# adr-arroyo/PointCloudComparator

Measured on NVIDIA B200. Metric: knn_queries_per_s_k16_10M, higher is better.
Workload: dtype f32

## Files before the change

### include/pcc/search.h

```cpp
#ifndef PCC_SEARCH_H_
#define PCC_SEARCH_H_

#include <stdint.h>

#ifdef __cplusplus
extern "C" {
#endif

#define PCC_HOST 0
#define PCC_DEVICE 1

#define PCC_OK 0
#define PCC_ERR_INVALID (-1)
#define PCC_ERR_CUDA (-2)
#define PCC_ERR_STATE (-3)

#define PCC_MAX_K 512

typedef struct pcc_index pcc_index;

const char *pcc_last_error(void);
int pcc_version(void);
int64_t pcc_launch_count(void);

int pcc_create(int device, pcc_index **out);
void pcc_destroy(pcc_index *idx);

int pcc_build(pcc_index *idx, const void *pts, int64_t n, int stride_bytes, const int32_t *indices, int64_t n_idx,
              float cell_hint, int k_hint, int mem, void *stream);
int64_t pcc_size(const pcc_index *idx);
int pcc_grid_info(const pcc_index *idx, double out[5]);

int pcc_knn(pcc_index *idx, const void *q, int64_t nq, int stride_bytes, int k, int32_t *out_idx, float *out_d2,
            int *k_eff, int mem, void *stream);

int pcc_radius_count(pcc_index *idx, const void *q, int64_t nq, int stride_bytes, double radius, unsigned max_nn,
                     int64_t *offsets, int64_t *total, int mem, void *stream);
int pcc_radius_fill(pcc_index *idx, const void *q, int64_t nq, int stride_bytes, double radius, unsigned max_nn, int sorted,
                    const int64_t *offsets, int32_t *out_idx, float *out_d2, int mem, void *stream);

int pcc_knn_mean_dist(pcc_index *idx, const void *q, int64_t nq, int stride_bytes, int mean_k, float *out_mean,
                      int mem, void *stream);
int pcc_sor_threshold(pcc_index *idx, const float *distances, int64_t n, int64_t n_valid, double std_mul, double stats[3],
                      uint8_t *keep, int64_t *kept, int mem, void *stream);

int pcc_normals_knn(pcc_index *idx, const void *q, int64_t nq, int stride_bytes, int k, const float viewpoint[3], float *out,
                    int mem, void *stream);
int pcc_normals_radius(pcc_index *idx, const void *q, int64_t nq, int stride_bytes, double radius, const float viewpoint[3],
                       float *out, int mem, void *stream);

int pcc_intensity_gradient(pcc_index *idx, const void *q, int64_t nq, int stride_bytes, double radius, const float *intensity,
                           const float *normals4, float *out, int mem, void *stream);
int pcc_rift(pcc_index *idx, const void *q, int64_t nq, int stride_bytes, double radius, const float *gradient4,
             int n_distance_bins, int n_gradient_bins, float *out, int mem, void *stream);

int pcc_sift_dog(pcc_index *idx, const float *values, const float *scales, int n_scales, float *out, int mem, void *stream);
int pcc_sift_extrema(pcc_index *idx, const float *dog, int n_cols, float min_contrast, int32_t *out_row, int32_t *out_col, int64_t cap,
                     int64_t *n_found, int mem, void *stream);
int pcc_sift_keypoints(pcc_index *idx, const void *pts, int64_t n, int stride_bytes, int rgb_offset_bytes, float min_scale, int nr_octaves,
                       int nr_scales_per_octave, float min_contrast, float *out4, int64_t cap, int64_t *n_keypoints, int mem, void *stream);

int pcc_icp_step(pcc_index *idx, void *src_inout, int64_t ns, int stride_bytes, const float *T_apply, double sums[16],
                 int64_t *count, int32_t *corr_idx, float *corr_d2, int mem, void *stream);
int pcc_icp_align(pcc_index *idx, const void *src, int64_t ns, int stride_bytes, int max_iter, float T16[16], int *converged,
                  double *fitness, int *iterations, int mem, void *stream);
int pcc_umeyama_from_sums(const double sums[16], int64_t count, float T16[16]);

int pcc_euclidean_labels(pcc_index *idx, double tolerance, int64_t min_size, int64_t max_size, int32_t *labels,
                         int64_t *n_clusters, int64_t *sizes, int64_t sizes_cap, int mem, void *stream);

int pcc_ece_init(pcc_index *idx, uint32_t *parent, void *stream);
int pcc_ece_link_range(pcc_index *idx, double tolerance, int64_t begin, int64_t end, uint32_t *parent, void *stream);
int pcc_ece_absorb(pcc_index *idx, const uint32_t *other, uint32_t *parent, void *stream);
int pcc_ece_finish(pcc_index *idx, uint32_t *parent, int64_t min_size, int64_t max_size, int32_t *labels, int64_t *n_clusters, int64_t *sizes,
                   int64_t sizes_cap, void *stream);

int pcc_first_within(pcc_index *idx, const void *q, int64_t nq, int stride_bytes, double thr, int32_t *out, int mem, void *stream);

int pcc_voxel_grid(pcc_index *idx, const void *pts, int64_t n, int stride_bytes, int rgb_offset_bytes, const float leaf[3],
                   int min_points_per_voxel, void *out, int64_t *n_out, int mem, void *stream);

int pcc_region_growing(const int32_t *neighbours, int64_t n, int k, const float *normals4, float smoothness_rad, float curvature_threshold,
                       int64_t min_size, int64_t max_size, int32_t *labels, int64_t *n_clusters);

int pcc_region_growing_rgb(const int32_t *neighbours, const float *sqr_distances, int64_t n, int k, const uint32_t *rgba, int rgba_stride_bytes,
                           float distance_threshold, float point_color_threshold, float region_color_threshold, int grow_neighbours,
                           int64_t min_size, int64_t max_size, int32_t *labels, int64_t *n_clusters);

int pcc_descriptor_nn(pcc_index *workspace, const float *ref, int64_t n_ref, const float *qry, int64_t n_qry, int dim, int stride_floats,
                      int32_t *out_idx, float *out_d2, int mem, void *stream);

int pcc_export(const pcc_index *idx, double meta[16], void *ptrs[2]);
int pcc_adopt(pcc_index *idx, const double meta[16], void *stream);

int pcc_comm_init(pcc_index *idx, void *nccl_comm, int rank, int world);
int pcc_comm_info(const pcc_index *idx, int *rank, int *world);
int pcc_broadcast_index(pcc_index *idx, int root, void *stream);
int pcc_gather(pcc_index *idx, const void *local, int64_t n_local, int row_bytes, const int32_t *local_rows, void *out, int64_t n_total, void *stream);
int pcc_allreduce_f64(pcc_index *idx, double *device_buf, int n, void *stream);

int pcc_set_timing(pcc_index *idx, int enable);
double pcc_last_kernel_ms(const pcc_index *idx);

#ifdef __cplusplus
}
#endif
#endif
```

### pointcloudcomparator_b200/_lib.py

```python
from __future__ import annotations

import ctypes as C
import os

_HERE = os.path.dirname(os.path.abspath(__file__))
SO_PATH = os.path.abspath(os.environ["PCC_SO"]) if os.environ.get("PCC_SO") else os.path.join(_HERE, "libpcc_search.so")

HOST, DEVICE = 0, 1
MAX_K = 512

_lib = None

SYMBOLS = [
    "pcc_last_error", "pcc_version", "pcc_launch_count", "pcc_create", "pcc_destroy", "pcc_build", "pcc_size", "pcc_grid_info",
    "pcc_knn", "pcc_radius_count", "pcc_radius_fill", "pcc_knn_mean_dist", "pcc_sor_threshold", "pcc_normals_knn",
    "pcc_normals_radius", "pcc_icp_step", "pcc_icp_align", "pcc_umeyama_from_sums", "pcc_euclidean_labels", "pcc_first_within",
    "pcc_export", "pcc_adopt", "pcc_set_timing", "pcc_last_kernel_ms", "pcc_ece_init", "pcc_ece_link_range", "pcc_ece_absorb", "pcc_ece_finish", "pcc_voxel_grid", "pcc_descriptor_nn", "pcc_region_growing",
    "pcc_region_growing_rgb", "pcc_intensity_gradient", "pcc_rift", "pcc_sift_dog", "pcc_sift_extrema", "pcc_sift_keypoints", "pcc_comm_init", "pcc_comm_info", "pcc_broadcast_index", "pcc_gather", "pcc_allreduce_f64",
]


class PccError(RuntimeError):
    pass


def lib():
    global _lib
    if _lib is not None:
        return _lib
    if not os.path.exists(SO_PATH):
        raise PccError(f"{SO_PATH} is missing: build it with `python -c 'import __graft_entry__ as g; g.build()'` "
                       "(make -C pointcloudcomparator_b200/csrc); there is no CPU fallback")
    L = C.CDLL(SO_PATH)
    vp, i64, i32, dbl, u32 = C.c_void_p, C.c_int64, C.c_int, C.c_double, C.c_uint
    L.pcc_last_error.restype = C.c_char_p
    L.pcc_launch_count.restype = i64
    L.pcc_create.argtypes = [i32, C.POINTER(vp)]
    L.pcc_destroy.argtypes = [vp]
    L.pcc_destroy.restype = None
    L.pcc_build.argtypes = [vp, vp, i64, i32, vp, i64, C.c_float, i32, i32, vp]
    L.pcc_size.argtypes = [vp]
    L.pcc_size.restype = i64
    L.pcc_grid_info.argtypes = [vp, C.POINTER(dbl)]
    L.pcc_knn.argtypes = [vp, vp, i64, i32, i32, vp, vp, C.POINTER(i32), i32, vp]
    L.pcc_radius_count.argtypes = [vp, vp, i64, i32, dbl, u32, vp, C.POINTER(i64), i32, vp]
    L.pcc_radius_fill.argtypes = [vp, vp, i64, i32, dbl, u32, i32, vp, vp, vp, i32, vp]
    L.pcc_knn_mean_dist.argtypes = [vp, vp, i64, i32, i32, vp, i32, vp]
    L.pcc_sor_threshold.argtypes = [vp, vp, i64, i64, dbl, C.POINTER(dbl), vp, C.POINTER(i64), i32, vp]
    L.pcc_normals_knn.argtypes = [vp, vp, i64, i32, i32, C.POINTER(C.c_float), vp, i32, vp]
    L.pcc_normals_radius.argtypes = [vp, vp, i64, i32, dbl, C.POINTER(C.c_float), vp, i32, vp]
    L.pcc_intensity_gradient.argtypes = [vp, vp, i64, i32, dbl, vp, vp, vp, i32, vp]
    L.pcc_rift.argtypes = [vp, vp, i64, i32, dbl, vp, i32, i32, vp, i32, vp]
    L.pcc_sift_dog.argtypes = [vp, vp, vp, i32, vp, i32, vp]
    L.pcc_sift_extrema.argtypes = [vp, vp, i32, C.c_float, vp, vp, i64, C.POINTER(i64), i32, vp]
    L.pcc_sift_keypoints.argtypes = [vp, vp, i64, i32, i32, C.c_float, i32, i32, C.c_float, vp, i64, C.POINTER(i64), i32, vp]
    L.pcc_icp_step.argtypes = [vp, vp, i64, i32, C.POINTER(C.c_float), C.POINTER(dbl), C.POINTER(i64), vp, vp, i32, vp]
    L.pcc_icp_align.argtypes = [vp, vp, i64, i32, i32, C.POINTER(C.c_float), C.POINTER(i32), C.POINTER(dbl), C.POINTER(i32), i32, vp]
    L.pcc_umeyama_from_sums.argtypes = [C.POINTER(dbl), i64, C.POINTER(C.c_float)]
    L.pcc_euclidean_labels.argtypes = [vp, dbl, i64, i64, vp, C.POINTER(i64), vp, i64, i32, vp]
    L.pcc_first_within.argtypes = [vp, vp, i64, i32, dbl, vp, i32, vp]
    L.pcc_ece_init.argtypes = [vp, vp, vp]
    L.pcc_ece_link_range.argtypes = [vp, dbl, i64, i64, vp, vp]
    L.pcc_ece_absorb.argtypes = [vp, vp, vp, vp]
    L.pcc_ece_finish.argtypes = [vp, vp, i64, i64, vp, C.POINTER(i64), vp, i64, vp]
    L.pcc_voxel_grid.argtypes = [vp, vp, i64, i32, i32, C.POINTER(C.c_float), i32, vp, C.POINTER(i64), i32, vp]
    L.pcc_descriptor_nn.argtypes = [vp, vp, i64, vp, i64, i32, i32, vp, vp, i32, vp]
    L.pcc_region_growing.argtypes = [vp, i64, i32, vp, C.c_float, C.c_float, i64, i64, vp, C.POINTER(i64)]
    L.pcc_export.argtypes = [vp, C.POINTER(dbl), C.POINTER(vp)]
    L.pcc_adopt.argtypes = [vp, C.POINTER(dbl), vp]
    L.pcc_region_growing_rgb.argtypes = [vp, vp, i64, i32, vp, i32, C.c_float, C.c_float, C.c_float, i32, i64, i64, vp, C.POINTER(i64)]
    L.pcc_comm_init.argtypes = [vp, vp, i32, i32]
    L.pcc_comm_info.argtypes = [vp, C.POINTER(i32), C.POINTER(i32)]
    L.pcc_broadcast_index.argtypes = [vp, i32, vp]
    L.pcc_gather.argtypes = [vp, vp, i64, i32, vp, vp, i64, vp]
    L.pcc_allreduce_f64.argtypes = [vp, vp, i32, vp]
    L.pcc_set_timing.argtypes = [vp, i32]
    L.pcc_last_kernel_ms.argtypes = [vp]
    L.pcc_last_kernel_ms.restype = dbl
    _lib = L
    return L


def check(rc: int):
    if rc != 0:
        raise PccError(f"libpcc_search error {rc}: {lib().pcc_last_error().decode(errors='replace')}")
```

### pointcloudcomparator_b200/csrc/pcc_build.cu

```cuda
#include <cub/cub.cuh>
#include <stdarg.h>
#include <algorithm>
#include <cmath>
#include <cstdlib>
#include <vector>

#include <cstring>
#include "pcc_internal.h"

namespace pcc {

thread_local std::string g_error;
std::atomic<int64_t> g_launches{0};

int fail(int code, const char *fmt, ...) {
    char buf[1024];
    va_list ap; va_start(ap, fmt); vsnprintf(buf, sizeof(buf), fmt, ap); va_end(ap);
    g_error = buf;
    return code;
}

static constexpr int kMaxDim = 2048;
static constexpr int64_t kMaxCellsDefault = 1ll << 28;

__device__ __forceinline__ int f2ord(float f) { int i = __float_as_int(f); return i >= 0 ? i : i ^ 0x7FFFFFFF; }
static inline float ord2f(int i) { int j = i >= 0 ? i : i ^ 0x7FFFFFFF; float f; memcpy(&f, &j, 4); return f; }

__global__ void extract_kernel(const uint8_t *__restrict__ raw, int stride, const int32_t *__restrict__ indices, int64_t m,
                               int64_t n_rows, float4 *__restrict__ stage, int *__restrict__ bbox, unsigned long long *__restrict__ n_finite) {
    int64_t i = (int64_t)blockIdx.x * blockDim.x + threadIdx.x;
    int lo[3] = {INT_MAX, INT_MAX, INT_MAX}, hi[3] = {INT_MIN, INT_MIN, INT_MIN};
    int fin = 0;
    if (i < m) {
        int64_t row = indices ? (int64_t)indices[i] : i;
        float x = CUDART_NAN_F, y = x, z = x;
        if (row >= 0 && row < n_rows) {
            const float *p = (const float *)(raw + row * (int64_t)stride);
            x = p[0]; y = p[1]; z = p[2];
        }
        fin = finite3(x, y, z);
        stage[i] = make_float4(x, y, z, fin ? __int_as_float((int)row) : CUDART_NAN_F);
        if (fin) { lo[0] = hi[0] = f2ord(x); lo[1] = hi[1] = f2ord(y); lo[2] = hi[2] = f2ord(z); }
    }
#pragma unroll
    for (int d = 0; d < 3; ++d) { lo[d] = __reduce_min_sync(0xffffffffu, lo[d]); hi[d] = __reduce_max_sync(0xffffffffu, hi[d]); }
    unsigned nf = __reduce_add_sync(0xffffffffu, (unsigned)fin);
    if ((threadIdx.x & 31) == 0 && nf) {
#pragma unroll
        for (int d = 0; d < 3; ++d) { atomicMin(bbox + d, lo[d]); atomicMax(bbox + 3 + d, hi[d]); }
        atomicAdd(n_finite, (unsigned long long)nf);
    }
}

struct BinParams { float ox, oy, oz, inv; int nx, ny, nz; };
constexpr int64_t kFillSamples = 1 << 17;
constexpr double kFillSurface = 15.0, kFillVolume = 21.0;
__device__ __forceinline__ uint32_t cell_of(const BinParams &b, float x, float y, float z) {
    int cx = grid_c(grid_u(x, b.ox, b.inv), b.nx), cy = grid_c(grid_u(y, b.oy, b.inv), b.ny), cz = grid_c(grid_u(z, b.oz, b.inv), b.nz);
    return (uint32_t)(((size_t)cz * b.ny + cy) * b.nx + cx);
}
__global__ void bin_kernel(const float4 *__restrict__ stage, int64_t m, BinParams b, uint32_t *__restrict__ counts, uint2 *__restrict__ cellrank) {
    int64_t i = (int64_t)blockIdx.x * blockDim.x + threadIdx.x;
    if (i >= m) return;
    float4 p = stage[i];
    if (p.w != p.w) { if (cellrank) cellrank[i] = make_uint2(0xFFFFFFFFu, 0u); return; }
    uint32_t c = cell_of(b, p.x, p.y, p.z);
    uint32_t r = atomicAdd(counts + c, 1u);
    if (cellrank) cellrank[i] = make_uint2(c, r);
}
__global__ void blockfill_kernel(const float4 *__restrict__ stage, int64_t m, int64_t stride, BinParams b, const uint32_t *__restrict__ counts, unsigned long long *__restrict__ out) {
    const int64_t i = ((int64_t)blockIdx.x * blockDim.x + threadIdx.x) * stride;
    unsigned filled = 0, sample = 0;
    if (i < m) {
        const float4 p = stage[i];
        if (p.w == p.w) {
            const int cx = grid_c(grid_u(p.x, b.ox, b.inv), b.nx), cy = grid_c(grid_u(p.y, b.oy, b.inv), b.ny), cz = grid_c(grid_u(p.z, b.oz, b.inv), b.nz);
            sample = 1;
            for (int z = max(cz - 1, 0); z <= min(cz + 1, b.nz - 1); ++z)
                for (int y = max(cy - 1, 0); y <= min(cy + 1, b.ny - 1); ++y)
                    for (int x = max(cx - 1, 0); x <= min(cx + 1, b.nx - 1); ++x)
                        filled += counts[((size_t)z * b.ny + y) * b.nx + x] > 0u ? 1u : 0u;
        }
    }
    filled = __reduce_add_sync(0xffffffffu, filled); sample = __reduce_add_sync(0xffffffffu, sample);
    if ((threadIdx.x & 31) == 0 && sample) { atomicAdd(out, (unsigned long long)filled); atomicAdd(out + 1, (unsigned long long)sample); }
}
__global__ void nonzero_kernel(const uint32_t *__restrict__ counts, int64_t n, unsigned long long *__restrict__ out) {
    unsigned local = 0;
    for (int64_t i = (int64_t)blockIdx.x * blockDim.x + threadIdx.x; i < n; i += (int64_t)gridDim.x * blockDim.x) local += counts[i] != 0;
    local = __reduce_add_sync(0xffffffffu, local);
    if ((threadIdx.x & 31) == 0 && local) atomicAdd(out, (unsigned long long)local);
}
__global__ void scatter_kernel(const float4 *__restrict__ stage, const uint2 *__restrict__ cellrank, int64_t m,
                               const uint32_t *__restrict__ cell_start, float4 *__restrict__ pts) {
    int64_t i = (int64_t)blockIdx.x * blockDim.x + threadIdx.x;
    if (i >= m) return;
    uint2 cr = cellrank[i];
    if (cr.x == 0xFFFFFFFFu) return;
    pts[cell_start[cr.x] + cr.y] = stage[i];
}
__global__ void inverse_kernel(const float4 *__restrict__ pts, int64_t n, uint32_t *__restrict__ inv_pos) {
    int64_t i = (int64_t)blockIdx.x * blockDim.x + threadIdx.x;
    if (i < n) inv_pos[__float_as_int(pts[i].w)] = (uint32_t)i;
}
__global__ void occupancy_kernel(const uint32_t *__restrict__ cell_start, int64_t n_cells, uint32_t *__restrict__ occ) {
    const int64_t words = (n_cells + 31) / 32 + 1;
    for (int64_t c = (int64_t)blockIdx.x * blockDim.x + threadIdx.x; c < words * 32; c += (int64_t)gridDim.x * blockDim.x) {
        const bool full = c < n_cells && cell_start[c + 1] > cell_start[c];
        const unsigned w = __ballot_sync(0xffffffffu, full);
        if ((threadIdx.x & 31) == 0) occ[c >> 5] = w;
    }
}
struct PopcOp { __device__ __forceinline__ uint32_t operator()(uint32_t w) const { return (uint32_t)__popc(w); } };
__global__ void compact_table_kernel(const uint32_t *__restrict__ occ, const uint32_t *__restrict__ wprefix, int64_t words, const uint32_t *__restrict__ cell_start,
                                     int64_t n_cells, uint2 *__restrict__ occ2, uint32_t *__restrict__ cstart) {
    const int64_t w = (int64_t)blockIdx.x * blockDim.x + threadIdx.x;
    if (w >= words) return;
    uint32_t bits = occ[w], r = wprefix[w];
    occ2[w] = make_uint2(bits, r);
    while (bits) { const int b = __ffs(bits) - 1; bits &= bits - 1; cstart[r++] = cell_start[w * 32 + b]; }
    if (w == words - 1) cstart[r] = cell_start[n_cells];
}
int rebuild_occupancy(pcc_index *idx, cudaStream_t s) {
    const int64_t n_cells = std::max<int64_t>(idx->gh.n_cells, 1);
    const int64_t words = (n_cells + 31) / 32 + 1;
    PCC_TRY(idx->occ.reserve((size_t)words * 4));
    const int64_t threads = words * 32;
    occupancy_kernel<<<(unsigned)std::min<int64_t>((threads + 255) / 256, 148 * 32), 256, 0, s>>>(idx->cell_start.as<uint32_t>(), idx->gh.n_cells, idx->occ.as<uint32_t>());
    PCC_LAUNCHED();
    PCC_CUDA(cudaGetLastError());
#if PCC_COMPACT_TABLE
    PCC_TRY(idx->occ2.reserve((size_t)(words + 1) * sizeof(uint2)));
    PCC_TRY(idx->cstart.reserve((size_t)(std::min<int64_t>(n_cells, std::max<int64_t>(idx->n_indexed, 0)) + 2) * 4));
    PCC_TRY(idx->qkeys2.reserve((size_t)words * 4));
    size_t tmp = 0;
    cub::TransformInputIterator<uint32_t, PopcOp, const uint32_t *> pc(idx->occ.as<uint32_t>(), PopcOp());
    cub::DeviceScan::ExclusiveSum(nullptr, tmp, pc, idx->qkeys2.as<uint32_t>(), (int)words, s);
    PCC_TRY(idx->cub_tmp.reserve(tmp));
    PCC_CUDA(cub::DeviceScan::ExclusiveSum(idx->cub_tmp.p, tmp, pc, idx->qkeys2.as<uint32_t>(), (int)words, s));
    g_launches += 2;
    PCC_CUDA(cudaMemsetAsync(idx->occ2.as<uint2>() + words, 0, sizeof(uint2), s));
    compact_table_kernel<<<(unsigned)((words + 255) / 256), 256, 0, s>>>(idx->occ.as<uint32_t>(), idx->qkeys2.as<uint32_t>(), words, idx->cell_start.as<uint32_t>(), idx->gh.n_cells,
                                                                 idx->occ2.as<uint2>(), idx->cstart.as<uint32_t>());
    PCC_LAUNCHED();
    PCC_CUDA(cudaGetLastError());
#endif
    idx->occ_valid = true;
    return PCC_OK;
}
int rebuild_inverse(pcc_index *idx, cudaStream_t s) {
    PCC_TRY(idx->inv_pos.reserve((size_t)std::max<int64_t>(idx->n_input, 1) * 4));
    PCC_CUDA(cudaMemsetAsync(idx->inv_pos.p, 0xFF, (size_t)std::max<int64_t>(idx->n_input, 1) * 4, s));
    if (idx->n_indexed > 0) {
        inverse_kernel<<<(unsigned)((idx->n_indexed + 255) / 256), 256, 0, s>>>(idx->pts.as<float4>(), idx->n_indexed, idx->inv_pos.as<uint32_t>());
        PCC_LAUNCHED();
        PCC_CUDA(cudaGetLastError());
    }
    idx->inv_valid = true;
    return PCC_OK;
}

__global__ void qprep_kernel(const uint8_t *__restrict__ raw, int stride, int64_t nq, BinParams b, uint32_t bad_key,
                             float4 *__restrict__ qbuf, uint32_t *__restrict__ keys, uint32_t *__restrict__ perm) {
    int64_t i = (int64_t)blockIdx.x * blockDim.x + threadIdx.x;
    if (i >= nq) return;
    const float *p = (const float *)(raw + i * (int64_t)stride);
    float x = p[0], y = p[1], z = p[2];
    qbuf[i] = make_float4(x, y, z, 0.f);
    if (keys) { keys[i] = finite3(x, y, z) ? cell_of(b, x, y, z) : bad_key; perm[i] = (uint32_t)i; }
}

static inline unsigned blocks_for(int64_t n, int threads) { return (unsigned)std::max<int64_t>(1, (n + threads - 1) / threads); }

static double occupancy_target(int k_hint) {
    int k = k_hint > 0 ? k_hint : 16;
    if (k == 1) return 12.0;
    return std::max(8.0, 0.5 * k);
}
static double occupancy_target_volume(int k_hint) {
    int k = k_hint > 0 ? k_hint : 16;
    if (k > 32) return 0.5 * k;
    return std::max(1.9, std::min(k / 3.5, 4.0 + (k - 16) / 10.0));
}
static bool occupancy_override(double *v) {
    const char *e = getenv("PCC_OCC");
    if (e && atof(e) > 0) { *v = atof(e); return true; }
    return false;
}

static void dims_for(const double ext[3], double cell, int dims[3]) {
    for (int d = 0; d < 3; ++d) dims[d] = (int)std::min<double>(kMaxDim, std::floor(ext[d] / cell) + 1);
}
static double clamp_cell(const double ext[3], double cell, int64_t max_cells) {
    double mx = std::max(ext[0], std::max(ext[1], ext[2]));
    if (!(cell > 0) || !std::isfinite(cell)) cell = mx > 0 ? mx : 1.0;
    cell = std::max(cell, mx / (kMaxDim - 1));
    for (int it = 0; it < 64; ++it) {
        int d[3]; dims_for(ext, cell, d);
        double total = (double)d[0] * d[1] * d[2];
        if (total <= (double)max_cells) break;
        cell *= std::max(1.02, std::cbrt(total / (double)max_cells));
    }
    return cell;
}

int prepare_queries(pcc_index *idx, const void *q, int64_t nq, int stride_bytes, int mem, cudaStream_t s, Queries *out) {
    if (!idx->built) return fail(PCC_ERR_STATE, "index not built (call pcc_build first)");
    if (q == nullptr) { out->self = true; out->nq = idx->n_indexed; out->rows = idx->n_input; out->q = nullptr; out->order = nullptr; return PCC_OK; }
    if (nq < 0 || nq >= (1ll << 31) - 1 || stride_bytes < 12 || (stride_bytes & 3)) return fail(PCC_ERR_INVALID, "bad query batch (nq=%lld stride=%d; nq must be below 2^31 - 1: row counts go to CUB as 32-bit ints)", (long long)nq, stride_bytes);
    out->self = false; out->nq = nq; out->rows = nq;
    if (nq == 0) return PCC_OK;
    const uint8_t *raw = (const uint8_t *)q;
    if (mem == PCC_HOST) {
        PCC_TRY(idx->raw.reserve((size_t)nq * stride_bytes));
        PCC_CUDA(cudaMemcpyAsync(idx->raw.p, q, (size_t)nq * stride_bytes, cudaMemcpyHostToDevice, s));
        raw = idx->raw.as<uint8_t>();
    }
    PCC_TRY(idx->qbuf.reserve((size_t)nq * sizeof(float4)));
    if (idx->reuse_order_n == nq && nq > 2048) {
        BinParams b0{idx->gh.ox, idx->gh.oy, idx->gh.oz, idx->gh.inv_cell, idx->gh.nx, idx->gh.ny, idx->gh.nz};
        qprep_kernel<<<blocks_for(nq, 256), 256, 0, s>>>(raw, stride_bytes, nq, b0, (uint32_t)idx->gh.n_cells, idx->qbuf.as<float4>(), nullptr, nullptr);
        PCC_LAUNCHED();
        PCC_CUDA(cudaGetLastError());
        out->q = idx->qbuf.as<float4>();
        out->order = idx->qperm2.as<uint32_t>();
        return PCC_OK;
    }
    const bool sort = nq > 2048;
    BinParams b{idx->gh.ox, idx->gh.oy, idx->gh.oz, idx->gh.inv_cell, idx->gh.nx, idx->gh.ny, idx->gh.nz};
    if (sort) {
        PCC_TRY(idx->qkeys.reserve((size_t)nq * 4)); PCC_TRY(idx->qkeys2.reserve((size_t)nq * 4));
        PCC_TRY(idx->qperm.reserve((size_t)nq * 4)); PCC_TRY(idx->qperm2.reserve((size_t)nq * 4));
    }
    qprep_kernel<<<blocks_for(nq, 256), 256, 0, s>>>(raw, stride_bytes, nq, b, (uint32_t)idx->gh.n_cells, idx->qbuf.as<float4>(),
                                                     sort ? idx->qkeys.as<uint32_t>() : nullptr, sort ? idx->qperm.as<uint32_t>() : nullptr);
    PCC_LAUNCHED();
    PCC_CUDA(cudaGetLastError());
    out->q = idx->qbuf.as<float4>();
    out->order = nullptr;
    if (sort) {
        int bits = 1; while ((1ll << bits) <= idx->gh.n_cells && bits < 32) ++bits;
        static const int low_env = getenv("PCC_SORT_LOW_BITS") ? atoi(getenv("PCC_SORT_LOW_BITS")) : 0;
        const int low = std::max(0, std::min(low_env, bits - 8));
        size_t tmp = idx->sort_tmp_bytes;
        if (idx->sort_tmp_nq != nq || idx->sort_tmp_bits != bits) {
            cub::DeviceRadixSort::SortPairs(nullptr, tmp, idx->qkeys.as<uint32_t>(), idx->qkeys2.as<uint32_t>(), idx->qperm.as<uint32_t>(), idx->qperm2.as<uint32_t>(), (int)nq, low, bits, s);
            idx->sort_tmp_nq = nq; idx->sort_tmp_bits = bits; idx->sort_tmp_bytes = tmp;
        }
        PCC_TRY(idx->cub_tmp.reserve(tmp));
        PCC_CUDA(cub::DeviceRadixSort::SortPairs(idx->cub_tmp.p, tmp, idx->qkeys.as<uint32_t>(), idx->qkeys2.as<uint32_t>(), idx->qperm.as<uint32_t>(), idx->qperm2.as<uint32_t>(), (int)nq, low, bits, s));
        g_launches += 4;
        out->order = idx->qperm2.as<uint32_t>();
    }
    return PCC_OK;
}

int copy_out(void *dst, const void *src_dev, size_t bytes, int mem, cudaStream_t s) {
    if (!bytes || dst == src_dev) return PCC_OK;
    PCC_CUDA(cudaMemcpyAsync(dst, src_dev, bytes, mem == PCC_HOST ? cudaMemcpyDeviceToHost : cudaMemcpyDeviceToDevice, s));
    return PCC_OK;
}

}

using namespace pcc;

extern "C" {

const char *pcc_last_error(void) { return g_error.c_str(); }
int pcc_version(void) { return 100; }
int64_t pcc_launch_count(void) { return g_launches.load(); }

int pcc_create(int device, pcc_index **out) {
    if (!out) return fail(PCC_ERR_INVALID, "out is NULL");
    int n = 0;
    cudaError_t e = cudaGetDeviceCount(&n);
    if (e != cudaSuccess || n == 0) return fail(PCC_ERR_CUDA, "no usable CUDA device (%s); this library has no CPU fallback", cudaGetErrorString(e));
    if (device < 0 || device >= n) return fail(PCC_ERR_INVALID, "device %d out of range (0..%d)", device, n - 1);
    PCC_CUDA(cudaSetDevice(device));
    cudaDeviceProp prop;
    PCC_CUDA(cudaGetDeviceProperties(&prop, device));
    if (prop.major < 10) return fail(PCC_ERR_CUDA, "device %d is sm_%d%d; libpcc_search is built for sm_100a only", device, prop.major, prop.minor);
    pcc_index *idx = new pcc_index();
    idx->device = device;
    PCC_CUDA(cudaMallocHost(&idx->h_pinned, 4096));
    memset(idx->h_pinned, 0, 4096);
    PCC_CUDA(cudaEventCreate(&idx->ev0));
    PCC_CUDA(cudaEventCreate(&idx->ev1));
    *out = idx;
    return PCC_OK;
}

void pcc_destroy(pcc_index *idx) {
    if (!idx) return;
    cudaSetDevice(idx->device);
    if (idx->shadow) { pcc_index *sh = idx->shadow; idx->shadow = nullptr; pcc_destroy(sh); }
    for (int i = 0; i < 2; ++i) if (idx->pipe_stream[i]) cudaStreamDestroy(idx->pipe_stream[i]);
    Buf *bufs[] = {&idx->pts, &idx->cell_start, &idx->occ, &idx->occ2, &idx->cstart, &idx->raw, &idx->stage4, &idx->cellrank, &idx->qbuf, &idx->qkeys, &idx->qkeys2, &idx->qperm, &idx->qperm2,
                   &idx->cub_tmp, &idx->out_i, &idx->out_f, &idx->out_l, &idx->keys64, &idx->keys64b, &idx->misc, &idx->parent, &idx->inv_pos, &idx->sel_params, &idx->icp_prior, &idx->calib,
                   &idx->sift_cloud[0], &idx->sift_cloud[1], &idx->sift_val, &idx->sift_dog, &idx->sift_in, &idx->sift_nbr, &idx->sift_d2, &idx->sift_flag, &idx->sift_pos,
                   &idx->sift_row, &idx->sift_col, &idx->sift_kp};
    for (Buf *b : bufs) b->release();
    if (idx->h_pinned) cudaFreeHost(idx->h_pinned);
    if (idx->aux_stream) cudaStreamDestroy(idx->aux_stream);
    if (idx->ev_fork) cudaEventDestroy(idx->ev_fork);
    if (idx->ev_join) cudaEventDestroy(idx->ev_join);
    if (idx->ev0) cudaEventDestroy(idx->ev0);
    if (idx->ev1) cudaEventDestroy(idx->ev1);
    delete idx;
}

int64_t pcc_size(const pcc_index *idx) { return idx ? idx->n_indexed : 0; }

int pcc_grid_info(const pcc_index *idx, double out[5]) {
    if (!idx || !idx->built) return fail(PCC_ERR_STATE, "index not built");
    out[0] = idx->gh.nx; out[1] = idx->gh.ny; out[2] = idx->gh.nz; out[3] = idx->gh.cell; out[4] = idx->gh.occupancy;
    return PCC_OK;
}

int pcc_set_timing(pcc_index *idx, int enable) { if (!idx) return fail(PCC_ERR_INVALID, "idx is NULL"); idx->timing = enable != 0; idx->last_ms = -1; return PCC_OK; }
double pcc_last_kernel_ms(const pcc_index *idx) { return idx ? idx->last_ms : -1; }

int pcc_build(pcc_index *idx, const void *pts, int64_t n, int stride_bytes, const int32_t *indices, int64_t n_idx,
              float cell_hint, int k_hint, int mem, void *stream) {
    if (!idx) return fail(PCC_ERR_INVALID, "idx is NULL");
    if (n < 0 || (n > 0 && !pts) || stride_bytes < 12 || (stride_bytes & 3)) return fail(PCC_ERR_INVALID, "bad cloud (n=%lld stride=%d)", (long long)n, stride_bytes);
    if (n >= (1ll << 31) - 1) return fail(PCC_ERR_INVALID, "n=%lld exceeds int32 indices", (long long)n);
    if (indices && (n_idx < 0 || n_idx >= (1ll << 31) - 1)) return fail(PCC_ERR_INVALID, "n_idx=%lld out of range", (long long)n_idx);
    cudaStream_t s = (cudaStream_t)stream;
    PCC_CUDA(cudaSetDevice(idx->device));
    idx->built = false;
    idx->inv_valid = false;
    idx->occ_valid = false;
    idx->icp_prior_n = -1;
    ++idx->grid_gen;
    const int64_t m = indices ? n_idx : n;
    idx->n_input = n;
    idx->n_indexed = 0;
    idx->gh = GridHost();

    const uint8_t *raw = (const uint8_t *)pts;
    const int32_t *d_indices = indices;
    if (mem == PCC_HOST && m > 0) {
        PCC_TRY(idx->raw.reserve((size_t)n * stride_bytes));
        PCC_CUDA(cudaMemcpyAsync(idx->raw.p, pts, (size_t)n * stride_bytes, cudaMemcpyHostToDevice, s));
        raw = idx->raw.as<uint8_t>();
        if (indices) {
            PCC_TRY(idx->misc.reserve((size_t)n_idx * 4));
            PCC_CUDA(cudaMemcpyAsync(idx->misc.p, indices, (size_t)n_idx * 4, cudaMemcpyHostToDevice, s));
            d_indices = idx->misc.as<int32_t>();
        }
    }
    int *h = (int *)idx->h_pinned;
    PCC_TRY(idx->stage4.reserve((size_t)std::max<int64_t>(m, 1) * sizeof(float4)));
    PCC_TRY(idx->keys64.reserve(256));
    int *d_scal = idx->keys64.as<int>();
    {
        int init[12] = {INT_MAX, INT_MAX, INT_MAX, INT_MIN, INT_MIN, INT_MIN, 0, 0, 0, 0, 0, 0};
        memcpy(h, init, sizeof(init));
        PCC_CUDA(cudaMemcpyAsync(d_scal, h, sizeof(init), cudaMemcpyHostToDevice, s));
        PCC_CUDA(cudaStreamSynchronize(s));
    }
    if (m > 0) {
        extract_kernel<<<blocks_for(m, 256), 256, 0, s>>>(raw, stride_bytes, d_indices, m, n, idx->stage4.as<float4>(), d_scal, (unsigned long long *)(d_scal + 8));
        PCC_LAUNCHED();
        PCC_CUDA(cudaGetLastError());
    }
    PCC_CUDA(cudaMemcpyAsync(h, d_scal, 48, cudaMemcpyDeviceToHost, s));
    PCC_CUDA(cudaStreamSynchronize(s));
    const int64_t nfin = (int64_t)(*(unsigned long long *)(h + 8));
    idx->n_indexed = nfin;
    idx->all_rows_indexed = !indices && nfin == n;
    if (nfin == 0) {
        PCC_TRY(idx->pts.reserve(sizeof(float4)));
        PCC_TRY(idx->cell_start.reserve(2 * sizeof(uint32_t)));
        PCC_CUDA(cudaMemsetAsync(idx->cell_start.p, 0, 2 * sizeof(uint32_t), s));
        idx->gh = GridHost();
        PCC_TRY(rebuild_occupancy(idx, s));
        idx->built = true;
        return PCC_OK;
    }
    double lo[3], ext[3];
    for (int d = 0; d < 3; ++d) { lo[d] = ord2f(h[d]); ext[d] = (double)ord2f(h[3 + d]) - lo[d]; }

    int64_t max_cells = kMaxCellsDefault;
    if (const char *e = getenv("PCC_MAX_CELLS")) { long long v = atoll(e); if (v >= 1) max_cells = std::min<long long>(v, kMaxCellsDefault); }
    const double mx = std::max(ext[0], std::max(ext[1], ext[2]));
    double cell;
    const bool autotune = !(cell_hint > 0);
    double target = occupancy_target(k_hint);
    const bool target_fixed = occupancy_override(&target);
    if (!autotune) cell = cell_hint;
    else {
        int live = 0; double vol = 1;
        for (int d = 0; d < 3; ++d) if (ext[d] > 1e-6 * mx && ext[d] > 0) { ++live; vol *= ext[d]; }
        cell = live ? std::pow(vol * target / (double)nfin, 1.0 / live) : 1.0;
    }
    cell = clamp_cell(ext, cell, max_cells);

    PCC_TRY(idx->cellrank.reserve((size_t)m * sizeof(uint2)));
    BinParams b{};
    int dims[3]; int64_t n_cells = 0; double occ = 0;
    double prev_cell = 0, prev_occ = 0, dim_first = 2.0;
    for (int it = 0; it < 5; ++it) {
        dims_for(ext, cell, dims);
        n_cells = (int64_t)dims[0] * dims[1] * dims[2];
        const float cellf = (float)cell;
        b = BinParams{(float)lo[0], (float)lo[1], (float)lo[2], 1.0f / cellf, dims[0], dims[1], dims[2]};
        PCC_TRY(idx->cell_start.reserve((size_t)(n_cells + 1) * sizeof(uint32_t)));
        PCC_CUDA(cudaMemsetAsync(idx->cell_start.p, 0, (size_t)(n_cells + 1) * sizeof(uint32_t), s));
        PCC_CUDA(cudaMemsetAsync(d_scal + 10, 0, 24, s));
        bin_kernel<<<blocks_for(m, 256), 256, 0, s>>>(idx->stage4.as<float4>(), m, b, idx->cell_start.as<uint32_t>(), idx->cellrank.as<uint2>());
        PCC_LAUNCHED();
        nonzero_kernel<<<(unsigned)std::min<int64_t>(blocks_for(n_cells, 256), 148 * 16), 256, 0, s>>>(idx->cell_start.as<uint32_t>(), n_cells, (unsigned long long *)(d_scal + 10));
        PCC_LAUNCHED();
        const bool probe_fill = autotune && !target_fixed && it == 0;
        if (probe_fill) {
            const int64_t stride = std::max<int64_t>(1, m / kFillSamples);
            blockfill_kernel<<<blocks_for((m + stride - 1) / stride, 256), 256, 0, s>>>(idx->stage4.as<float4>(), m, stride, b, idx->cell_start.as<uint32_t>(), (unsigned long long *)(d_scal + 12));
            PCC_LAUNCHED();
        }
        PCC_CUDA(cudaGetLastError());
        PCC_CUDA(cudaMemcpyAsync(h + 10, d_scal + 10, 24, cudaMemcpyDeviceToHost, s));
        PCC_CUDA(cudaStreamSynchronize(s));
        const int64_t nonempty = (int64_t)(*(unsigned long long *)(h + 10));
        occ = (double)nfin / (double)std::max<int64_t>(nonempty, 1);
        if (probe_fill) {
            const unsigned long long filled = *(unsigned long long *)(h + 12), samples = *(unsigned long long *)(h + 14);
            const double nb = samples ? (double)filled / (double)samples : 0.0;
            const double w = std::min(1.0, std::max(0.0, (nb - kFillSurface) / (kFillVolume - kFillSurface)));
            target = (1.0 - w) * target + w * occupancy_target_volume(k_hint);
            dim_first = 2.0 + w;
            idx->gh.block_fill = nb;
        }
        if (!autotune || it == 4) break;
        if (occ > 0.9 * target && occ < 1.4 * target) break;
        double dim_est = dim_first;
        if (prev_cell > 0 && prev_occ > 0 && std::fabs(std::log(cell / prev_cell)) > 1e-3) {
            dim_est = std::log(occ / prev_occ) / std::log(cell / prev_cell);
            dim_est = std::min(3.0, std::max(1.0, dim_est));
        }
        prev_cell = cell; prev_occ = occ;
        double next = clamp_cell(ext, cell * std::pow(target / occ, 1.0 / dim_est), max_cells);
        if (std::fabs(next / cell - 1.0) < 0.02) break;
        cell = next;
    }
    idx->gh.ox = b.ox; idx->gh.oy = b.oy; idx->gh.oz = b.oz;
    idx->gh.cell = (float)cell; idx->gh.inv_cell = b.inv;
    idx->gh.nx = dims[0]; idx->gh.ny = dims[1]; idx->gh.nz = dims[2];
    idx->gh.n_cells = n_cells; idx->gh.occupancy = occ;

    size_t tmp = 0;
    cub::DeviceScan::ExclusiveSum(nullptr, tmp, idx->cell_start.as<uint32_t>(), idx->cell_start.as<uint32_t>(), (int)(n_cells + 1), s);
    PCC_TRY(idx->cub_tmp.reserve(tmp));
    PCC_CUDA(cub::DeviceScan::ExclusiveSum(idx->cub_tmp.p, tmp, idx->cell_start.as<uint32_t>(), idx->cell_start.as<uint32_t>(), (int)(n_cells + 1), s));
    g_launches += 2;
    PCC_TRY(idx->pts.reserve((size_t)nfin * sizeof(float4)));
    scatter_kernel<<<blocks_for(m, 256), 256, 0, s>>>(idx->stage4.as<float4>(), idx->cellrank.as<uint2>(), m, idx->cell_start.as<uint32_t>(), idx->pts.as<float4>());
    PCC_LAUNCHED();
    PCC_CUDA(cudaGetLastError());
    PCC_TRY(rebuild_occupancy(idx, s));
    if (mem == PCC_HOST) PCC_CUDA(cudaStreamSynchronize(s));
    idx->built = true;
    return PCC_OK;
}

int pcc_export(const pcc_index *idx, double meta[16], void *ptrs[2]) {
    if (!idx || !idx->built) return fail(PCC_ERR_STATE, "index not built");
    meta[0] = (double)idx->n_indexed; meta[1] = (double)idx->n_input;
    meta[2] = idx->gh.nx; meta[3] = idx->gh.ny; meta[4] = idx->gh.nz;
    meta[5] = idx->gh.ox; meta[6] = idx->gh.oy; meta[7] = idx->gh.oz;
    meta[8] = idx->gh.cell; meta[9] = idx->gh.inv_cell; meta[10] = idx->gh.occupancy; meta[11] = (double)idx->gh.n_cells;
    meta[12] = idx->all_rows_indexed ? 1.0 : 0.0; meta[13] = meta[14] = meta[15] = 0;
    ptrs[0] = idx->pts.p; ptrs[1] = idx->cell_start.p;
    return PCC_OK;
}

int pcc_adopt(pcc_index *idx, const double meta[16], void *stream) {
    if (!idx) return fail(PCC_ERR_INVALID, "idx is NULL");
    (void)stream;
    PCC_CUDA(cudaSetDevice(idx->device));
    if (!(meta[0] >= 0 && meta[1] >= 0 && meta[0] < 2147483647.0 && meta[1] < 2147483647.0 && meta[2] >= 1 && meta[3] >= 1 && meta[4] >= 1 && meta[2] <= 2048 && meta[3] <= 2048 && meta[4] <= 2048 &&
          meta[11] >= 1 && meta[11] <= (double)kMaxCellsDefault && meta[11] == meta[2] * meta[3] * meta[4] && meta[8] > 0))
        return fail(PCC_ERR_INVALID, "pcc_adopt: grid description out of range (n=%g dims=%gx%gx%g cells=%g cell=%g)", meta[0], meta[2], meta[3], meta[4], meta[11], meta[8]);
    idx->n_indexed = (int64_t)meta[0]; idx->n_input = (int64_t)meta[1]; idx->all_rows_indexed = meta[12] == 1.0;
    idx->gh.nx = (int)meta[2]; idx->gh.ny = (int)meta[3]; idx->gh.nz = (int)meta[4];
    idx->gh.ox = (float)meta[5]; idx->gh.oy = (float)meta[6]; idx->gh.oz = (float)meta[7];
    idx->gh.cell = (float)meta[8]; idx->gh.inv_cell = (float)meta[9]; idx->gh.occupancy = meta[10]; idx->gh.n_cells = (int64_t)meta[11];
    PCC_TRY(idx->pts.reserve((size_t)std::max<int64_t>(idx->n_indexed, 1) * sizeof(float4)));
    PCC_TRY(idx->cell_start.reserve((size_t)(idx->gh.n_cells + 1) * sizeof(uint32_t)));
    idx->built = true;
    idx->inv_valid = false;
    idx->icp_prior_n = -1;
    ++idx->grid_gen;
    idx->occ_valid = false;
    return PCC_OK;
}

}
```

### pointcloudcomparator_b200/csrc/pcc_device.cuh

```cuda
#pragma once
#include <type_traits>
#include <cuda_runtime.h>
#include <stdint.h>
#include <math_constants.h>

namespace pcc {

struct Grid {
    const float4 *pts;
    const uint32_t *cell_start;
    const uint32_t *occ;
    const uint2 *occ2;
    const uint32_t *cstart;
    float ox, oy, oz;
    float inv_cell, cell;
    int nx, ny, nz;
    uint32_t n;
};

#ifndef PCC_COMPACT_TABLE
#define PCC_COMPACT_TABLE 0
#endif
__device__ __forceinline__ uint32_t cell_begin(const Grid &g, size_t c) {
#if PCC_COMPACT_TABLE
    const uint2 w = __ldg(g.occ2 + (c >> 5));
    return __ldg(g.cstart + w.y + __popc(w.x & ((1u << (c & 31)) - 1u)));
#else
    return __ldg(g.cell_start + c);
#endif
}

__device__ __forceinline__ float dist2(float qx, float qy, float qz, float px, float py, float pz) {
    float dx = __fsub_rn(qx, px), dy = __fsub_rn(qy, py), dz = __fsub_rn(qz, pz);
    return __fadd_rn(__fadd_rn(__fmul_rn(dx, dx), __fmul_rn(dy, dy)), __fmul_rn(dz, dz));
}
__device__ __forceinline__ float grid_u(float x, float o, float inv) { return __fmul_rn(__fsub_rn(x, o), inv); }
__device__ __forceinline__ int grid_c(float u, int n) { return (int)fminf(fmaxf(floorf(u), 0.f), (float)(n - 1)); }
__device__ __forceinline__ bool finite3(float x, float y, float z) { return isfinite(x) && isfinite(y) && isfinite(z); }

struct QueryCell {
    float ux, uy, uz;
    int cx, cy, cz;
};
__device__ __forceinline__ QueryCell locate(const Grid &g, float x, float y, float z) {
    QueryCell c;
    c.ux = grid_u(x, g.ox, g.inv_cell); c.uy = grid_u(y, g.oy, g.inv_cell); c.uz = grid_u(z, g.oz, g.inv_cell);
    c.cx = grid_c(c.ux, g.nx); c.cy = grid_c(c.uy, g.ny); c.cz = grid_c(c.uz, g.nz);
    return c;
}
__device__ __forceinline__ float covered_d2(const Grid &g, const QueryCell &c, int R) {
    float b = CUDART_INF_F;
    if (c.cx - R > 0) b = fminf(b, c.ux - (float)(c.cx - R));
    if (c.cx + R < g.nx - 1) b = fminf(b, (float)(c.cx + R + 1) - c.ux);
    if (c.cy - R > 0) b = fminf(b, c.uy - (float)(c.cy - R));
    if (c.cy + R < g.ny - 1) b = fminf(b, (float)(c.cy + R + 1) - c.uy);
    if (c.cz - R > 0) b = fminf(b, c.uz - (float)(c.cz - R));
    if (c.cz + R < g.nz - 1) b = fminf(b, (float)(c.cz + R + 1) - c.uz);
    if (b == CUDART_INF_F) return b;
    b = (b * (1.0f - 1e-5f) - 2e-3f) * g.cell;
    return b > 0.f ? b * b : 0.f;
}

template <class F>
__device__ __forceinline__ void scan_shell(const Grid &g, const QueryCell &c, int Rin, int Rout, F &&f) {
    const int z0 = max(c.cz - Rout, 0), z1 = min(c.cz + Rout, g.nz - 1);
    const int y0 = max(c.cy - Rout, 0), y1 = min(c.cy + Rout, g.ny - 1);
    const int xa = max(c.cx - Rout, 0), xb = min(c.cx + Rout, g.nx - 1);
    for (int z = z0; z <= z1; ++z) {
        for (int y = y0; y <= y1; ++y) {
            const uint32_t *row = g.cell_start + ((size_t)z * g.ny + y) * g.nx;
            const bool outer = max(abs(z - c.cz), abs(y - c.cy)) > Rin;
            if (outer) {
                uint32_t j = __ldg(row + xa), e = __ldg(row + xb + 1);
                for (; j < e; ++j) f(j, __ldg(g.pts + j));
            } else {
                int xl = c.cx - Rin - 1;
                if (xl >= xa) { uint32_t j = __ldg(row + xa), e = __ldg(row + xl + 1); for (; j < e; ++j) f(j, __ldg(g.pts + j)); }
                int xr = c.cx + Rin + 1;
                if (xr <= xb) { uint32_t j = __ldg(row + xr), e = __ldg(row + xb + 1); for (; j < e; ++j) f(j, __ldg(g.pts + j)); }
            }
        }
    }
}

__device__ __forceinline__ float to_cell_units(const Grid &g, float d2) { return d2 == CUDART_INF_F ? d2 : d2 * g.inv_cell * g.inv_cell * (1.0f + 4e-5f); }

__device__ __forceinline__ int next_ring(const Grid &g, int R, float kth_d2) {
    const int cap = max(g.nx, max(g.ny, g.nz));
    if (kth_d2 == CUDART_INF_F) return min(2 * R + 1, max(cap, R + 1));
    const float need = sqrtf(to_cell_units(g, kth_d2)) + 0.01f;
    return max(R + 1, (int)fminf(ceilf(need), (float)cap));
}

struct group_visitor {};
template <class F>
__device__ __forceinline__ void walk_run(const Grid &g, uint32_t j, uint32_t e, F &&f) {
    for (; j + 4 <= e; j += 4) {
        const float4 p0 = __ldg(g.pts + j), p1 = __ldg(g.pts + j + 1), p2 = __ldg(g.pts + j + 2), p3 = __ldg(g.pts + j + 3);
#ifndef PCC_GROUP_VISIT
#define PCC_GROUP_VISIT 1
#endif
        if constexpr (PCC_GROUP_VISIT && std::is_base_of<group_visitor, typename std::remove_reference<F>::type>::value) f.four(j, p0, p1, p2, p3);
        else { f(j, p0); f(j + 1, p1); f(j + 2, p2); f(j + 3, p3); }
    }
    if (j < e) {
        const float4 p0 = __ldg(g.pts + j);
        const float4 p1 = __ldg(g.pts + min(j + 1, e - 1)), p2 = __ldg(g.pts + min(j + 2, e - 1));
        f(j, p0);
        if (j + 1 < e) f(j + 1, p1);
        if (j + 2 < e) f(j + 2, p2);
    }
}

__device__ __forceinline__ int centre_out(int a) { return (a & 1) ? -((a + 1) >> 1) : (a >> 1); }
struct RowRuns { uint32_t j1, e1, j2, e2; };
__device__ __forceinline__ bool row_occupied(const Grid &g, size_t base, int xa, int xb) {
    if (xb - xa >= 32) return true;
    const size_t b = base + (size_t)xa;
#if PCC_COMPACT_TABLE
    const uint32_t w0 = __ldg(&g.occ2[b >> 5].x), w1 = __ldg(&g.occ2[(b >> 5) + 1].x);
#else
    const uint32_t w0 = __ldg(g.occ + (b >> 5)), w1 = __ldg(g.occ + (b >> 5) + 1);
#endif
    const uint32_t bits = __funnelshift_r(w0, w1, (uint32_t)(b & 31));
    const int len = xb - xa + 1;
    return (bits & (len == 32 ? 0xffffffffu : ((1u << len) - 1u))) != 0u;
}
__device__ __forceinline__ RowRuns row_runs(const Grid &g, const QueryCell &c, int Rin, int Rout, float tau_u, int az, int ay) {
    RowRuns r; r.j1 = r.e1 = r.j2 = r.e2 = 0;
    const int dz = centre_out(az), z = c.cz + dz, dy = centre_out(ay), y = c.cy + dy;
    if (z < 0 || z >= g.nz || y < 0 || y >= g.ny) return r;
    const float gz = fmaxf(fmaxf((float)z - c.uz, c.uz - (float)(z + 1)) - 2e-3f, 0.f);
    const float gy = fmaxf(fmaxf((float)y - c.uy, c.uy - (float)(y + 1)) - 2e-3f, 0.f);
    const float D = gy * gy + gz * gz;
    if (D > tau_u) return r;
    int xlo = c.cx - Rout, xhi = c.cx + Rout;
    if (tau_u < CUDART_INF_F) {
        const float w = sqrtf(tau_u - D) + 2e-3f;
        xlo = max(xlo, (int)floorf(c.ux - w)); xhi = min(xhi, (int)floorf(c.ux + w));
    }
    xlo = max(xlo, 0); xhi = min(xhi, g.nx - 1);
    const size_t base = ((size_t)z * g.ny + y) * g.nx;
    const bool probe = Rin >= 0;
    if (max(abs(dz), abs(dy)) > Rin) {
        if (xlo <= xhi && (!probe || row_occupied(g, base, xlo, xhi))) { r.j1 = cell_begin(g, base + xlo); r.e1 = cell_begin(g, base + xhi + 1); }
    } else {
        const int xl = min(xhi, c.cx - Rin - 1);
        if (xlo <= xl && row_occupied(g, base, xlo, xl)) { r.j1 = cell_begin(g, base + xlo); r.e1 = cell_begin(g, base + xl + 1); }
        const int xr = max(xlo, c.cx + Rin + 1);
        if (xr <= xhi && row_occupied(g, base, xr, xhi)) { r.j2 = cell_begin(g, base + xr); r.e2 = cell_begin(g, base + xhi + 1); }
    }
    return r;
}
template <class T, class F>
__device__ __forceinline__ void scan_progressive(const Grid &g, const QueryCell &c, int Rin, int Rout, T &&tau_now, F &&f) {
    const int n1 = 2 * Rout + 1;
    int az = 0, ay = 0;
    RowRuns nxt = row_runs(g, c, Rin, Rout, tau_now(), 0, 0);
    for (;;) {
        const RowRuns cur = nxt;
        if (++ay == n1) { ay = 0; ++az; }
        const bool more = az < n1;
        if (more) nxt = row_runs(g, c, Rin, Rout, tau_now(), az, ay);
        walk_run(g, cur.j1, cur.e1, f);
        walk_run(g, cur.j2, cur.e2, f);
        if (!more) break;
    }
}
template <class F>
__device__ __forceinline__ void scan_clipped(const Grid &g, const QueryCell &c, int Rin, int Rout, float tau_u, F &&f) {
    scan_progressive(g, c, Rin, Rout, [&]() { return tau_u; }, f);
}

struct Nearest1 : group_visitor {
    float x, y, z, bd; uint32_t bidx, bpos;
    __device__ __forceinline__ void init(float qx, float qy, float qz) { x = qx; y = qy; z = qz; bd = CUDART_INF_F; bidx = 0xFFFFFFFFu; bpos = 0; }
    __device__ __forceinline__ bool found() const { return bidx != 0xFFFFFFFFu; }
    __device__ __forceinline__ void take(uint32_t pos, const float4 &r, float d2) {
        const uint32_t ri = __float_as_uint(r.w);
        if (d2 < bd || ri < bidx) { bd = d2; bidx = ri; bpos = pos; }
    }
    __device__ __forceinline__ void operator()(uint32_t pos, const float4 &r) { const float d2 = dist2(x, y, z, r.x, r.y, r.z); if (d2 <= bd) take(pos, r, d2); }
    __device__ __forceinline__ void four(uint32_t j, const float4 &p0, const float4 &p1, const float4 &p2, const float4 &p3) {
        const float d0 = dist2(x, y, z, p0.x, p0.y, p0.z), d1 = dist2(x, y, z, p1.x, p1.y, p1.z), d2 = dist2(x, y, z, p2.x, p2.y, p2.z), d3 = dist2(x, y, z, p3.x, p3.y, p3.z);
        if (fminf(fminf(d0, d1), fminf(d2, d3)) <= bd) {
            if (d0 <= bd) take(j, p0, d0);
            if (d1 <= bd) take(j + 1, p1, d1);
            if (d2 <= bd) take(j + 2, p2, d2);
            if (d3 <= bd) take(j + 3, p3, d3);
        }
    }
// ... 311 lines not shown
```

### pointcloudcomparator_b200/csrc/pcc_internal.h

```cpp
#pragma once
#include <cuda_runtime.h>
#include <stdint.h>
#include <stdio.h>
#include <atomic>
#include <string>

#include "../../include/pcc/search.h"
#include "pcc_device.cuh"

namespace pcc {

extern thread_local std::string g_error;
extern std::atomic<int64_t> g_launches;
int fail(int code, const char *fmt, ...);

#define PCC_CUDA(expr)                                                                                   \
    do {                                                                                                 \
        cudaError_t e__ = (expr);                                                                        \
        if (e__ != cudaSuccess) return pcc::fail(PCC_ERR_CUDA, "%s:%d %s -> %s", __FILE__, __LINE__, #expr, cudaGetErrorString(e__)); \
    } while (0)
#define PCC_TRY(expr)                 \
    do {                              \
        int r__ = (expr);             \
        if (r__ != PCC_OK) return r__; \
    } while (0)
#define PCC_LAUNCHED() (++pcc::g_launches)

struct Buf {
    void *p = nullptr;
    size_t cap = 0;
    int reserve(size_t bytes) {
        if (bytes <= cap) return PCC_OK;
        if (p) cudaFree(p);
        p = nullptr; cap = 0;
        size_t want = bytes + bytes / 8 + 256;
        cudaError_t e = cudaMalloc(&p, want);
        if (e != cudaSuccess) { p = nullptr; return fail(PCC_ERR_CUDA, "cudaMalloc(%zu) -> %s", want, cudaGetErrorString(e)); }
        cap = want;
        return PCC_OK;
    }
    void release() { if (p) cudaFree(p); p = nullptr; cap = 0; }
    template <class T> T *as() const { return (T *)p; }
};

struct GridHost {
    float ox = 0, oy = 0, oz = 0, cell = 1, inv_cell = 1;
    int nx = 1, ny = 1, nz = 1;
    double occupancy = 0;
    double block_fill = 0;
    int64_t n_cells = 1;
};

}

struct pcc_index {
    int device = 0;
    bool built = false;
    int64_t n_input = 0;
    int64_t n_indexed = 0;
    bool all_rows_indexed = false;
    pcc::GridHost gh;
    pcc::Buf pts;
    pcc::Buf cell_start;
    pcc::Buf occ;
    pcc::Buf occ2, cstart;
    bool occ_valid = false;
    pcc::Buf raw, stage4, cellrank, qbuf, qkeys, qkeys2, qperm, qperm2, cub_tmp, out_i, out_f, out_l, keys64, keys64b, misc, parent, inv_pos, sel_params, icp_prior, calib;
    pcc::Buf sift_cloud[2], sift_val, sift_dog, sift_in, sift_nbr, sift_d2, sift_flag, sift_pos, sift_row, sift_col, sift_kp;
    uint64_t grid_gen = 0;
    void *comm = nullptr;
    int comm_rank = 0, comm_world = 1;
    int64_t sel_tmp_nq = -1; size_t sel_tmp_bytes = 0; int64_t sort_tmp_nq = -1; int sort_tmp_bits = 0; size_t sort_tmp_bytes = 0;
    bool icp_allreduce = false;
    int calib_k = -1;
    uint64_t calib_gen = 0;
    int64_t calib_nq = 0;
    int64_t reuse_order_n = -1;
    int64_t icp_prior_n = -1;
    bool inv_valid = false;
    void *h_pinned = nullptr;
    cudaEvent_t ev0 = nullptr, ev1 = nullptr;
    bool timing = false;
    double last_ms = -1;

    pcc_index *shadow = nullptr;
    const pcc_index *grid_owner = nullptr;
    cudaStream_t pipe_stream[2] = {nullptr, nullptr};
    cudaStream_t aux_stream = nullptr;
    cudaEvent_t ev_fork = nullptr, ev_join = nullptr;

    pcc::Grid grid() const {
        const pcc_index *o = grid_owner ? grid_owner : this;
        pcc::Grid g;
        g.pts = o->pts.as<float4>(); g.cell_start = o->cell_start.as<uint32_t>(); g.occ = o->occ.as<uint32_t>(); g.occ2 = o->occ2.as<uint2>(); g.cstart = o->cstart.as<uint32_t>();
        g.ox = o->gh.ox; g.oy = o->gh.oy; g.oz = o->gh.oz; g.inv_cell = o->gh.inv_cell; g.cell = o->gh.cell;
        g.nx = o->gh.nx; g.ny = o->gh.ny; g.nz = o->gh.nz; g.n = (uint32_t)o->n_indexed;
        return g;
    }
};

namespace pcc {
struct Queries {
    const float4 *q = nullptr;
    const uint32_t *order = nullptr;
    int64_t nq = 0;
    bool self = false;
    int64_t rows = 0;
};
int prepare_queries(pcc_index *idx, const void *q, int64_t nq, int stride_bytes, int mem, cudaStream_t s, Queries *out);
int copy_out(void *dst, const void *src_dev, size_t bytes, int mem, cudaStream_t s);
int rebuild_inverse(pcc_index *idx, cudaStream_t s);
int rebuild_occupancy(pcc_index *idx, cudaStream_t s);
int comm_allreduce_f64(pcc_index *idx, double *d_buf, int n, cudaStream_t s);
int knn_select(pcc_index *idx, const Queries &qs, int k, int32_t *oi, float *od, cudaStream_t s);
struct KernelTimer {
    pcc_index *idx; cudaStream_t s;
    KernelTimer(pcc_index *i, cudaStream_t st) : idx(i), s(st) { if (idx->timing) cudaEventRecord(idx->ev0, s); }
    void stop() { if (idx->timing) { cudaEventRecord(idx->ev1, s); cudaEventSynchronize(idx->ev1); float ms = 0; cudaEventElapsedTime(&ms, idx->ev0, idx->ev1); idx->last_ms = ms; } }
};
}
```

### pointcloudcomparator_b200/csrc/pcc_knn.cu

```cuda
#include <algorithm>
#include <cmath>
#include <cstring>

#include <cub/device/device_select.cuh>
#include <cub/iterator/counting_input_iterator.cuh>

#include "pcc_internal.h"
#include "pcc_fastknn.cuh"

namespace pcc {

struct QueryView {
    const float4 *q; const uint32_t *order; int64_t nq; bool self;
};
__device__ __forceinline__ bool load_query(const Grid &g, const QueryView &v, int64_t t, float &x, float &y, float &z, int64_t &row, bool &write_empty) {
    write_empty = false;
    if (t >= v.nq) return false;
    if (v.self) { float4 p = __ldg(g.pts + t); x = p.x; y = p.y; z = p.z; row = __float_as_int(p.w); return true; }
    uint32_t qi = v.order ? __ldg(v.order + t) : (uint32_t)t;
    float4 p = __ldg(v.q + qi); x = p.x; y = p.y; z = p.z; row = qi;
#ifdef PCC_EXP_SEQROWS
    row = t;
#endif
#ifdef PCC_EXP_SEQQ
    p = __ldg(v.q + t); x = p.x; y = p.y; z = p.z;
#endif
    if (!finite3(x, y, z) || g.n == 0) { write_empty = true; return false; }
    return true;
}

template <class List>
__device__ __forceinline__ void knn_search(const Grid &g, float x, float y, float z, int k, List &list) {
    const QueryCell c = locate(g, x, y, z);
    int Rin = -1, R = 1;
    for (;;) {
        scan_progressive(g, c, Rin, R, [&]() { return to_cell_units(g, key_d2(list.at(k - 1))); },
                         [&](uint32_t, float4 p) { list.offer(make_key(dist2(x, y, z, p.x, p.y, p.z), __float_as_uint(p.w))); });
        const float cov = covered_d2(g, c, R);
        if (cov == CUDART_INF_F) break;
        const nkey_t kth = list.at(k - 1);
        if (kth != PCC_EMPTY_KEY && key_d2(kth) < cov) break;
        Rin = R; R = next_ring(g, R, key_d2(kth));
    }
}

template <int K>
__device__ __forceinline__ void write_row(const nkey_t (&key)[K], int k, int32_t *__restrict__ oi, float *__restrict__ od, int vec4) {
    if (vec4 && K >= 4 && k == K) {
#pragma unroll
        for (int j = 0; j + 3 < K; j += 4) {
            reinterpret_cast<int4 *>(oi)[j >> 2] = make_int4(key_idx(key[j]), key_idx(key[j + 1]), key_idx(key[j + 2]), key_idx(key[j + 3]));
            reinterpret_cast<float4 *>(od)[j >> 2] = make_float4(key_d2(key[j]), key_d2(key[j + 1]), key_d2(key[j + 2]), key_d2(key[j + 3]));
        }
    } else {
#pragma unroll
        for (int j = 0; j < K; ++j) if (j < k) { oi[j] = key_idx(key[j]); od[j] = key_d2(key[j]); }
    }
}
template <int K>
__device__ __forceinline__ void knn_reg_body(const Grid &g, const QueryView &v, int64_t t, int k, int32_t *__restrict__ out_idx, float *__restrict__ out_d2, int vec4) {
    float x, y, z; int64_t row; bool empty;
    RegList<K> list; list.init();
    const bool live = load_query(g, v, t, x, y, z, row, empty);
    if (!live && !empty) return;
    if (live) knn_search(g, x, y, z, k, list);
    write_row<K>(list.key, k, out_idx + row * k, out_d2 + row * k, vec4);
}
template <int K>
__global__ void __launch_bounds__(128) knn_reg_kernel(Grid g, QueryView v, int k, int32_t *__restrict__ out_idx, float *__restrict__ out_d2, int vec4) {
    knn_reg_body<K>(g, v, (int64_t)blockIdx.x * blockDim.x + threadIdx.x, k, out_idx, out_d2, vec4);
}
constexpr unsigned kTiedToWide = 4096;
struct FixList { uint32_t *list; unsigned *count; unsigned long long *stats; uint32_t *ring_list; unsigned *ring_count; uint8_t *ring_flag; uint32_t *wide_list; unsigned *wide_count; uint32_t *late_list; unsigned *late_count; uint32_t *retry_list; unsigned *retry_count; };
__device__ __forceinline__ void push_list(uint32_t *list, unsigned *count, uint32_t value) {
    const unsigned mask = __activemask();
    const int leader = __ffs(mask) - 1, lane = threadIdx.x & 31;
    unsigned base = 0;
    if (lane == leader) base = atomicAdd(count, (unsigned)__popc(mask));
    base = __shfl_sync(mask, base, leader);
    list[base + __popc(mask & ((1u << lane) - 1))] = value;
}
template <int K>
__global__ void __launch_bounds__(128) knn_fixup_kernel(Grid g, QueryView v, int k, int32_t *__restrict__ out_idx, float *__restrict__ out_d2, int vec4, FixList fix) {
    const unsigned n = *fix.count;
    if (fix.wide_list && n <= kTiedToWide) return;
    for (unsigned i = blockIdx.x * blockDim.x + threadIdx.x; i < n; i += gridDim.x * blockDim.x) knn_reg_body<K>(g, v, (int64_t)fix.list[i], k, out_idx, out_d2, vec4);
}

#ifndef PCC_LOG16
#define PCC_LOG16 48
#endif
#ifndef PCC_MB16
#define PCC_MB16 9
#endif
#ifndef PCC_LOG32
#define PCC_LOG32 80
#endif
#ifndef PCC_MB32
#define PCC_MB32 5
#endif
constexpr int64_t kSmallBatch = 1024, kSmallBatchBigK = 64;
constexpr int kRingMaxR = 3;
template <int K> struct FastCfg { static constexpr int threads = 128, log_slots = K <= 16 ? PCC_LOG16 : PCC_LOG32, min_blocks = K <= 16 ? PCC_MB16 : PCC_MB32; };
}
#include "pcc_knn_thr.cuh"
namespace pcc {
template <int K>
__device__ __forceinline__ float kth_distance(const Grid &g, const QueryCell &c, float x, float y, float z, int k, RegDist<K> &list, bool &proved,
                                              uint32_t *__restrict__ slog, int &nlog, const int R0) {
    scan_progressive(g, c, -1, R0, [&]() { return to_cell_units(g, (k == K) ? list.d[K - 1] : list.at(k - 1)); }, [&](uint32_t pos, float4 p) {
        const float d2 = dist2(x, y, z, p.x, p.y, p.z);
        if (d2 <= list.d[K - 1]) {
            if (nlog < FastCfg<K>::log_slots) slog[nlog * FastCfg<K>::threads] = pos;
            ++nlog;
            list.insert(d2);
        }
    });
    const float kth = (k == K) ? list.d[K - 1] : list.at(k - 1);
    const float cov = covered_d2(g, c, R0);
    proved = cov == CUDART_INF_F || kth < cov;
    return kth;
}
template <int K>
__device__ __forceinline__ void knn_fast_body(const Grid &g, const QueryView &v, const int64_t t, int k, int32_t *__restrict__ out_idx, float *__restrict__ out_d2, int vec4,
                                              const FixList &fix, uint32_t *__restrict__ slog, const int R0) {
    constexpr int kFastThreads = FastCfg<K>::threads, kLogSlots = FastCfg<K>::log_slots;
    float x, y, z; int64_t row; bool empty;
    const bool live = load_query(g, v, t, x, y, z, row, empty);
    if (!live) {
        if (R0 == 1 && t < v.nq) fix.ring_flag[t] = 0;
        if (empty) { nkey_t e[K];
#pragma unroll
            for (int j = 0; j < K; ++j) e[j] = PCC_EMPTY_KEY;
            write_row<K>(e, k, out_idx + row * k, out_d2 + row * k, vec4); }
        return;
    }
    const QueryCell c = locate(g, x, y, z);
    RegDist<K> list; list.init();
    int nlog = 0; bool proved;
    const float tau = kth_distance<K>(g, c, x, y, z, k, list, proved, slog, nlog, R0);
    int m = 0;
    if (nlog <= kLogSlots) {
        for (int i = 0; i < nlog; ++i) {
            const uint32_t pos = slog[i * kFastThreads];
            const float4 p = __ldg(g.pts + pos);
            if (dist2(x, y, z, p.x, p.y, p.z) <= tau) { slog[m * kFastThreads] = pos; ++m; }
        }
    } else {
        scan_clipped(g, c, -1, R0, to_cell_units(g, tau), [&](uint32_t pos, float4 p) {
            if (dist2(x, y, z, p.x, p.y, p.z) <= tau) { if (m < kLogSlots) slog[m * kFastThreads] = pos; ++m; }
        });
    }
    if (fix.stats && R0 == 1) { atomicAdd(fix.stats + 0, 1ull); atomicAdd(fix.stats + 1, (unsigned long long)nlog); atomicAdd(fix.stats + 4, proved ? 0ull : 1ull); atomicAdd(fix.stats + 5, m > K ? 1ull : 0ull); atomicAdd(fix.stats + 6, (unsigned long long)m); atomicAdd(fix.stats + 3, nlog > kLogSlots ? 1ull : 0ull); }
    const bool tied = m > K;
    const bool wide = !tied && !proved && (tau == CUDART_INF_F || next_ring(g, 1, tau) > kRingMaxR);
    if (R0 == 1) fix.ring_flag[t] = (!tied && !proved && !wide) ? 1 : 0;
    if (tied) { push_list(fix.list, fix.count, (uint32_t)t); return; }
    if (wide) { push_list(fix.wide_list, fix.wide_count, (uint32_t)t); return; }
    nkey_t e[K];
#pragma unroll
    for (int j = 0; j < K; ++j) {
        e[j] = PCC_EMPTY_KEY;
        if (j < m) { const float4 p = __ldg(g.pts + slog[j * kFastThreads]); e[j] = make_key(dist2(x, y, z, p.x, p.y, p.z), __float_as_uint(p.w)); }
    }
    bitonic_sort_key<K>(e);
    write_row<K>(e, k, out_idx + row * k, out_d2 + row * k, vec4);
}
template <int K>
__global__ void __launch_bounds__(FastCfg<K>::threads, FastCfg<K>::min_blocks) knn_fast_kernel(Grid g, QueryView v, int k, int32_t *__restrict__ out_idx, float *__restrict__ out_d2, int vec4, FixList fix) {
    __shared__ uint32_t slog_all[FastCfg<K>::log_slots * FastCfg<K>::threads];
    knn_fast_body<K>(g, v, (int64_t)blockIdx.x * blockDim.x + threadIdx.x, k, out_idx, out_d2, vec4, fix, slog_all + threadIdx.x, 1);
}
__device__ __forceinline__ nkey_t warp_sort_keys(nkey_t v, int lane) {
#pragma unroll
    for (int size = 2; size <= 32; size <<= 1) {
#pragma unroll
        for (int j = size >> 1; j > 0; j >>= 1) {
            const nkey_t o = __shfl_xor_sync(0xffffffffu, v, j);
// ... 410 lines not shown
__global__ void mean_dist_heap_kernel(Grid g, QueryView v, int mean_k, float *__restrict__ out) {
    extern __shared__ nkey_t smem_keys[];
    const int64_t t = (int64_t)blockIdx.x * blockDim.x + threadIdx.x;
    float x, y, z; int64_t row; bool empty;
    const bool live = load_query(g, v, t, x, y, z, row, empty);
    if (!live) { if (empty) out[row] = 0.f; return; }
    HeapList list; list.init(smem_keys + threadIdx.x, blockDim.x, mean_k + 1);
    const QueryCell c = locate(g, x, y, z);
    int Rin = -1, R = 1;
    for (;;) {
        scan_progressive(g, c, Rin, R, [&]() { return list.full() ? to_cell_units(g, key_d2(list.worst())) : CUDART_INF_F; },
                             [&](uint32_t, float4 p) { list.offer(make_key(dist2(x, y, z, p.x, p.y, p.z), __float_as_uint(p.w))); });
        const float cov = covered_d2(g, c, R);
        if (cov == CUDART_INF_F) break;
        if (list.full() && key_d2(list.worst()) < cov) break;
        Rin = R; R = next_ring(g, R, list.full() ? key_d2(list.worst()) : CUDART_INF_F);
    }
    list.finish();
    double s = 0.0;
    for (int j = 1; j <= mean_k; ++j) s += sqrt((double)key_d2(list.at(j)));
    out[row] = (float)(s / (double)mean_k);
}

template <int K>
__global__ void __launch_bounds__(128) normals_knn_reg_kernel(Grid g, QueryView v, int k, const uint32_t *__restrict__ inv_pos, float vx, float vy, float vz, float4 *__restrict__ out) {
    const int64_t t = (int64_t)blockIdx.x * blockDim.x + threadIdx.x;
    float x, y, z; int64_t row; bool empty;
    const bool live = load_query(g, v, t, x, y, z, row, empty);
    if (!live) { if (empty) out[row] = make_float4(CUDART_NAN_F, CUDART_NAN_F, CUDART_NAN_F, CUDART_NAN_F); return; }
    RegList<K> list; list.init();
    knn_search(g, x, y, z, k, list);
    float a[9] = {0, 0, 0, 0, 0, 0, 0, 0, 0}; int cnt = 0;
#pragma unroll
    for (int j = 0; j < K; ++j) if (j < k && list.key[j] != PCC_EMPTY_KEY) { float4 p = __ldg(g.pts + __ldg(inv_pos + (uint32_t)list.key[j])); accu_add(a, p.x, p.y, p.z); ++cnt; }
    out[row] = normal_from_accu(a, cnt, x, y, z, vx, vy, vz);
}
__global__ void normals_knn_heap_kernel(Grid g, QueryView v, int k, const uint32_t *__restrict__ inv_pos, float vx, float vy, float vz, float4 *__restrict__ out) {
    extern __shared__ nkey_t smem_keys[];
    const int64_t t = (int64_t)blockIdx.x * blockDim.x + threadIdx.x;
    float x, y, z; int64_t row; bool empty;
    const bool live = load_query(g, v, t, x, y, z, row, empty);
    if (!live) { if (empty) out[row] = make_float4(CUDART_NAN_F, CUDART_NAN_F, CUDART_NAN_F, CUDART_NAN_F); return; }
    HeapList list; list.init(smem_keys + threadIdx.x, blockDim.x, k);
    const QueryCell c = locate(g, x, y, z);
    int Rin = -1, R = 1;
    for (;;) {
        scan_progressive(g, c, Rin, R, [&]() { return list.full() ? to_cell_units(g, key_d2(list.worst())) : CUDART_INF_F; },
                             [&](uint32_t, float4 p) { list.offer(make_key(dist2(x, y, z, p.x, p.y, p.z), __float_as_uint(p.w))); });
        const float cov = covered_d2(g, c, R);
        if (cov == CUDART_INF_F) break;
        if (list.full() && key_d2(list.worst()) < cov) break;
        Rin = R; R = next_ring(g, R, list.full() ? key_d2(list.worst()) : CUDART_INF_F);
    }
    list.finish();
    float a[9] = {0, 0, 0, 0, 0, 0, 0, 0, 0}; int cnt = 0;
    for (int j = 0; j < list.cnt; ++j) { float4 p = __ldg(g.pts + __ldg(inv_pos + (uint32_t)list.at(j))); accu_add(a, p.x, p.y, p.z); ++cnt; }
    out[row] = normal_from_accu(a, cnt, x, y, z, vx, vy, vz);
}

struct Mat34 { float m[12]; };
static constexpr int kIcpThreads = 128, kIcpMaxPriorR = 16;
__global__ void __launch_bounds__(kIcpThreads) icp_step_kernel(Grid g, float4 *__restrict__ src, const uint32_t *__restrict__ order, int64_t ns, Mat34 T, int apply,
                                                               double *__restrict__ partials, int32_t *__restrict__ corr_idx, float *__restrict__ corr_d2,
                                                               uint32_t *__restrict__ prior) {
    const int64_t t = (int64_t)blockIdx.x * blockDim.x + threadIdx.x;
    double acc[17];
#pragma unroll
    for (int i = 0; i < 17; ++i) acc[i] = 0.0;
    if (t < ns) {
        const uint32_t qi = order ? __ldg(order + t) : (uint32_t)t;
        float4 p = src[qi];
        int32_t bi = -1; float bd = CUDART_INF_F;
        uint32_t acc_pos = 0xFFFFFFFFu;
        if (finite3(p.x, p.y, p.z)) {
            if (apply) {
                float nx = ((T.m[0] * p.x + T.m[1] * p.y) + T.m[2] * p.z) + T.m[3];
                float ny = ((T.m[4] * p.x + T.m[5] * p.y) + T.m[6] * p.z) + T.m[7];
                float nz = ((T.m[8] * p.x + T.m[9] * p.y) + T.m[10] * p.z) + T.m[11];
                p.x = nx; p.y = ny; p.z = nz;
                src[qi] = p;
            }
            if (g.n > 0 && finite3(p.x, p.y, p.z)) {
                Nearest1 nn; nn.init(p.x, p.y, p.z);
                const QueryCell c = locate(g, p.x, p.y, p.z);
                int R = 1;
                const uint32_t pv = prior ? prior[qi] : 0xFFFFFFFFu;
                if (pv < g.n) {
                    const float4 m = __ldg(g.pts + pv);
                    nn.bd = dist2(p.x, p.y, p.z, m.x, m.y, m.z); nn.bidx = __float_as_uint(m.w); nn.bpos = pv;
                    R = next_ring(g, 0, nn.bd);
                    if (R > kIcpMaxPriorR) { nn.init(p.x, p.y, p.z); R = 1; }
                }
                nearest1_search(g, c, R, nn);
                bi = nn.found() ? (int32_t)nn.bidx : -1; bd = nn.bd;
                const uint32_t bpos = nn.bpos;
                if (bi >= 0) {
                    acc_pos = bpos;
                    const float4 m = __ldg(g.pts + bpos);
                    const double sx = p.x, sy = p.y, sz = p.z, tx = m.x, ty = m.y, tz = m.z;
                    acc[0] = sx; acc[1] = sy; acc[2] = sz; acc[3] = tx; acc[4] = ty; acc[5] = tz;
                    acc[6] = tx * sx; acc[7] = tx * sy; acc[8] = tx * sz;
                    acc[9] = ty * sx; acc[10] = ty * sy; acc[11] = ty * sz;
                    acc[12] = tz * sx; acc[13] = tz * sy; acc[14] = tz * sz;
                    acc[15] = (double)bd; acc[16] = 1.0;
                }
            }
        }
        if (corr_idx) corr_idx[qi] = bi;
        if (corr_d2) corr_d2[qi] = bd;
        if (prior) prior[qi] = bi >= 0 ? acc_pos : 0xFFFFFFFFu;
    }
    __shared__ double red[kIcpThreads / 32][17];
#pragma unroll
    for (int i = 0; i < 17; ++i) {
        double v = acc[i];
#pragma unroll
        for (int o = 16; o > 0; o >>= 1) v += __shfl_xor_sync(0xffffffffu, v, o);
        if ((threadIdx.x & 31) == 0) red[threadIdx.x >> 5][i] = v;
    }
    __syncthreads();
    if (threadIdx.x < 17) {
        double v = 0.0;
#pragma unroll
        for (int w = 0; w < kIcpThreads / 32; ++w) v += red[w][threadIdx.x];
        partials[(size_t)blockIdx.x * 17 + threadIdx.x] = v;
    }
}
__global__ void icp_reduce_kernel(const double *__restrict__ partials, int64_t n_blocks, double *__restrict__ out) {
    __shared__ double red[256];
    const int comp = blockIdx.x;
    double v = 0.0;
    for (int64_t b = threadIdx.x; b < n_blocks; b += blockDim.x) v += partials[(size_t)b * 17 + comp];
    red[threadIdx.x] = v;
    __syncthreads();
    for (int o = 128; o > 0; o >>= 1) { if ((int)threadIdx.x < o) red[threadIdx.x] += red[threadIdx.x + o]; __syncthreads(); }
    if (threadIdx.x == 0) out[comp] = red[0];
}
__global__ void icp_load_kernel(const uint8_t *__restrict__ raw, int stride, int64_t ns, float4 *__restrict__ dst) {
    int64_t i = (int64_t)blockIdx.x * blockDim.x + threadIdx.x;
    if (i >= ns) return;
    const float *p = (const float *)(raw + i * (int64_t)stride);
    dst[i] = make_float4(p[0], p[1], p[2], 1.0f);
}
__global__ void icp_store_kernel(const float4 *__restrict__ srcw, int64_t ns, uint8_t *__restrict__ raw, int stride) {
    int64_t i = (int64_t)blockIdx.x * blockDim.x + threadIdx.x;
    if (i >= ns) return;
    float *p = (float *)(raw + i * (int64_t)stride);
    float4 v = srcw[i];
    p[0] = v.x; p[1] = v.y; p[2] = v.z;
}

__global__ void fill_f32_kernel(float *p, int64_t n, float v) { int64_t i = (int64_t)blockIdx.x * blockDim.x + threadIdx.x; if (i < n) p[i] = v; }
static inline unsigned nblocks(int64_t n, int threads) { return (unsigned)std::max<int64_t>(1, (n + threads - 1) / threads); }
static inline QueryView view_of(const Queries &q) { return QueryView{q.q, q.order, q.nq, q.self}; }
static int heap_threads(int k) {
    int t = (int)((96 * 1024) / ((size_t)k * sizeof(nkey_t)));
    t = std::min(128, (t / 32) * 32);
    return std::max(32, t);
}
template <class Kern>
static int set_heap_smem(Kern kern) {
    PCC_CUDA(cudaFuncSetAttribute(kern, cudaFuncAttributeMaxDynamicSharedMemorySize, 160 * 1024));
    return PCC_OK;
}

template <int K>
static void launch_knn_reg(const Grid &g, const QueryView &v, int k, int32_t *oi, float *od, int vec4, cudaStream_t s) {
    knn_reg_kernel<K><<<nblocks(v.nq, 128), 128, 0, s>>>(g, v, k, oi, od, vec4);
    PCC_LAUNCHED();
}
template <int K>
static void launch_knn_cell(const Grid &g, const QueryView &v, int k, int32_t *oi, float *od, int vec4, FixList fix, cudaStream_t s) {
    fix.wide_list = nullptr;
    cudaMemsetAsync(fix.count, 0, sizeof(unsigned), s);
    knn_cell_kernel<K><<<nblocks(v.nq, kCellWarps * 32), kCellWarps * 32, 0, s>>>(g, v, k, oi, od, vec4, fix);
    PCC_LAUNCHED();
    knn_fixup_kernel<K><<<148 * 4, 128, 0, s>>>(g, v, k, oi, od, vec4, fix);
    PCC_LAUNCHED();
}
constexpr int64_t kCalibSample = 1 << 15;
constexpr float kCalibQuantile = 0.99f;
template <int K>
static int calibrate_thr(pcc_index *idx, const Grid &g, const QueryView &v, int k, cudaStream_t s) {
    PCC_TRY(idx->calib.reserve((size_t)kCalibBuckets * kCalibBins * 4 + kCalibBuckets * 4));
    unsigned *hist = idx->calib.as<unsigned>();
    float *ratio = (float *)(hist + kCalibBuckets * kCalibBins);
    PCC_CUDA(cudaMemsetAsync(hist, 0, (size_t)kCalibBuckets * kCalibBins * 4, s));
    const int64_t stride = std::max<int64_t>(1, v.nq / kCalibSample), ns = (v.nq + stride - 1) / stride;
    knn_calib_kernel<K><<<nblocks(ns, 128), 128, 0, s>>>(g, v, k, stride, hist);
    PCC_LAUNCHED();
    static const float quantile = getenv("PCC_THR_QUANTILE") ? (float)atof(getenv("PCC_THR_QUANTILE")) : kCalibQuantile;
    knn_calib_finish_kernel<<<1, kCalibBuckets, 0, s>>>(hist, ratio, quantile);
    PCC_LAUNCHED();
    return PCC_OK;
}
template <int K>
static int launch_knn_fast(pcc_index *idx, const Grid &g, const QueryView &v, int k, int32_t *oi, float *od, int vec4, FixList fix, cudaStream_t s) {
    size_t tmp = idx->sel_tmp_bytes;
    if (idx->sel_tmp_nq != v.nq) {
        cub::DeviceSelect::Flagged(nullptr, tmp, cub::CountingInputIterator<uint32_t>(0), fix.ring_flag, fix.ring_list, fix.ring_count, (int)v.nq, s);
        idx->sel_tmp_nq = v.nq; idx->sel_tmp_bytes = tmp;
    }
    PCC_TRY(idx->cub_tmp.reserve(tmp));
    if (!idx->aux_stream) {
        PCC_CUDA(cudaStreamCreateWithFlags(&idx->aux_stream, cudaStreamNonBlocking));
        PCC_CUDA(cudaEventCreateWithFlags(&idx->ev_fork, cudaEventDisableTiming));
        PCC_CUDA(cudaEventCreateWithFlags(&idx->ev_join, cudaEventDisableTiming));
    }
    if (fix.stats) { cudaMemsetAsync(fix.count, 0, sizeof(unsigned), s); cudaMemsetAsync(fix.wide_count, 0, 3 * sizeof(unsigned), s); }
    else cudaMemsetAsync(fix.count, 0, 33 * sizeof(unsigned), s);
    static const bool old_fast_env = getenv("PCC_OLD_FAST") != nullptr;
    static const bool thr_all = getenv("PCC_THR_ALL") != nullptr;
    const bool old_fast = old_fast_env || (K != 16 && !thr_all) || v.nq >= (1ll << 31);
    if (old_fast) {
        knn_fast_kernel<K><<<nblocks(v.nq, FastCfg<K>::threads), FastCfg<K>::threads, 0, s>>>(g, v, k, oi, od, vec4, fix);
        PCC_LAUNCHED();
    } else {
        const pcc_index *owner = idx->grid_owner ? idx->grid_owner : idx;
        unsigned *h_fb = (unsigned *)((char *)idx->h_pinned + 2048);
        if (idx->calib_k == k && idx->calib_gen == owner->grid_gen && idx->calib_nq > 0 && (double)h_fb[0] > 0.04 * (double)idx->calib_nq) idx->calib_k = -1;
        if (idx->calib_k != k || idx->calib_gen != owner->grid_gen) {
            PCC_TRY(calibrate_thr<K>(idx, g, v, k, s));
            idx->calib_k = k; idx->calib_gen = owner->grid_gen;
        }
        const float *ratio = (const float *)(idx->calib.as<unsigned>() + kCalibBuckets * kCalibBins);
        static std::atomic<unsigned long long> attr_done{0};
        if (!((attr_done.load() >> (idx->device & 63)) & 1ull)) {
            PCC_CUDA(cudaFuncSetAttribute(knn_thr_kernel<K, true>, cudaFuncAttributeMaxDynamicSharedMemorySize, (int)ThrCfg<K>::smem));
            PCC_CUDA(cudaFuncSetAttribute(knn_thr_kernel<K, false>, cudaFuncAttributeMaxDynamicSharedMemorySize, (int)ThrCfg<K>::smem));
            PCC_CUDA(cudaFuncSetAttribute(knn_thr_retry_kernel<K, true>, cudaFuncAttributeMaxDynamicSharedMemorySize, (int)ThrCfg<K>::smem));
            PCC_CUDA(cudaFuncSetAttribute(knn_thr_retry_kernel<K, false>, cudaFuncAttributeMaxDynamicSharedMemorySize, (int)ThrCfg<K>::smem));
            attr_done.fetch_or(1ull << (idx->device & 63));
        }
        const char *staged_env = getenv("PCC_THR_STAGED");
        const bool staged = staged_env && atoi(staged_env) != 0;
        if (staged && k == K) {
            static std::atomic<unsigned long long> sattr_done{0};
            if (!((sattr_done.load() >> (idx->device & 63)) & 1ull)) {
                PCC_CUDA(cudaFuncSetAttribute(knn_thr_staged_kernel<K, true>, cudaFuncAttributeMaxDynamicSharedMemorySize, (int)ThrStagedCfg<K>::smem));
                sattr_done.fetch_or(1ull << (idx->device & 63));
            }
            knn_thr_staged_kernel<K, true><<<nblocks(v.nq, ThrCfg<K>::threads), ThrCfg<K>::threads, ThrStagedCfg<K>::smem, s>>>(g, v, k, oi, od, vec4, fix, ratio);
            PCC_LAUNCHED();
            knn_thr_retry_kernel<K, true><<<148 * 4, ThrCfg<K>::threads, ThrCfg<K>::smem, s>>>(g, v, k, oi, od, vec4, fix, ratio);
            PCC_LAUNCHED();
        } else if (k == K) {
            knn_thr_kernel<K, true><<<nblocks(v.nq, ThrCfg<K>::threads), ThrCfg<K>::threads, ThrCfg<K>::smem, s>>>(g, v, k, oi, od, vec4, fix, ratio);
            PCC_LAUNCHED();
            knn_thr_retry_kernel<K, true><<<148 * 4, ThrCfg<K>::threads, ThrCfg<K>::smem, s>>>(g, v, k, oi, od, vec4, fix, ratio);
            PCC_LAUNCHED();
        } else {
            knn_thr_kernel<K, false><<<nblocks(v.nq, ThrCfg<K>::threads), ThrCfg<K>::threads, ThrCfg<K>::smem, s>>>(g, v, k, oi, od, vec4, fix, ratio);
            PCC_LAUNCHED();
            knn_thr_retry_kernel<K, false><<<148 * 4, ThrCfg<K>::threads, ThrCfg<K>::smem, s>>>(g, v, k, oi, od, vec4, fix, ratio);
            PCC_LAUNCHED();
        }
        h_fb[0] = 0; idx->calib_nq = v.nq;
        PCC_CUDA(cudaMemcpyAsync(h_fb, fix.retry_count, sizeof(unsigned), cudaMemcpyDeviceToHost, s));
    }
    PCC_CUDA(cudaEventRecord(idx->ev_fork, s));
    PCC_CUDA(cudaStreamWaitEvent(idx->aux_stream, idx->ev_fork, 0));
    knn_wide_kernel<<<148 * 6, 128, 0, idx->aux_stream>>>(g, v, k, oi, od, fix, fix.wide_list, fix.wide_count, old_fast ? 1 : 0);
    PCC_LAUNCHED();
    PCC_CUDA(cudaEventRecord(idx->ev_join, idx->aux_stream));
    PCC_CUDA(cub::DeviceSelect::Flagged(idx->cub_tmp.p, tmp, cub::CountingInputIterator<uint32_t>(0), fix.ring_flag, fix.ring_list, fix.ring_count, (int)v.nq, s));
    PCC_LAUNCHED();
    knn_rings_kernel<K><<<148 * 16, 128, 0, s>>>(g, v, k, oi, od, vec4, fix);
    PCC_LAUNCHED();
    PCC_CUDA(cudaStreamWaitEvent(s, idx->ev_join, 0));
    knn_wide_kernel<<<148 * 2, 128, 0, s>>>(g, v, k, oi, od, fix, fix.late_list, fix.late_count, 0);
    PCC_LAUNCHED();
    if (old_fast) {
        knn_fixup_kernel<K><<<148 * 4, 128, 0, s>>>(g, v, k, oi, od, vec4, fix);
        PCC_LAUNCHED();
    }
    return PCC_OK;
}

}

using namespace pcc;

static int check_common(pcc_index *idx, void *stream) {
    if (!idx) return fail(PCC_ERR_INVALID, "idx is NULL");
    if (!idx->built) return fail(PCC_ERR_STATE, "index not built (call pcc_build first)");
    PCC_CUDA(cudaSetDevice(idx->device));
    if (!idx->occ_valid) PCC_TRY(rebuild_occupancy(idx, (cudaStream_t)stream));
    return PCC_OK;
}

extern "C" {

}

static int knn_impl(pcc_index *idx, const void *q, int64_t nq, int stride_bytes, int k, int32_t *out_idx, float *out_d2, int *k_eff, int mem, cudaStream_t s, bool sync) {
    Queries qs;
    PCC_TRY(prepare_queries(idx, q, nq, stride_bytes, mem, s, &qs));
    if (k_eff) *k_eff = (int)std::min<int64_t>(k, idx->n_indexed);
    if (qs.rows == 0) return PCC_OK;
    if (!out_idx || !out_d2) return fail(PCC_ERR_INVALID, "output pointers are NULL");
    int32_t *oi = out_idx; float *od = out_d2;
    const size_t cells = (size_t)qs.rows * k;
    if (mem == PCC_HOST) {
        PCC_TRY(idx->out_i.reserve(cells * 4)); PCC_TRY(idx->out_f.reserve(cells * 4));
        oi = idx->out_i.as<int32_t>(); od = idx->out_f.as<float>();
    }
    if (qs.self && !idx->all_rows_indexed) {
// ... 24 lines not shown
        else if (exact_only && k <= 8) launch_knn_reg<8>(g, v, k, oi, od, vec4, s);
        else if (exact_only && k <= 16) launch_knn_reg<16>(g, v, k, oi, od, vec4, s);
        else if (exact_only && k <= 32) launch_knn_reg<32>(g, v, k, oi, od, vec4, s);
        else if (use_cell && k <= 8) launch_knn_cell<8>(g, v, k, oi, od, vec4, fix, s);
        else if (use_cell && k <= 16) launch_knn_cell<16>(g, v, k, oi, od, vec4, fix, s);
        else if (use_cell && k <= 32) launch_knn_cell<32>(g, v, k, oi, od, vec4, fix, s);
        else if (k <= 4) PCC_TRY(launch_knn_fast<4>(idx, g, v, k, oi, od, vec4, fix, s));
        else if (k <= 8) PCC_TRY(launch_knn_fast<8>(idx, g, v, k, oi, od, vec4, fix, s));
        else if (k <= 16) PCC_TRY(launch_knn_fast<16>(idx, g, v, k, oi, od, vec4, fix, s));
        else if (k <= 32) PCC_TRY(launch_knn_fast<32>(idx, g, v, k, oi, od, vec4, fix, s));
        else if (!exact_only) PCC_TRY(knn_select(idx, qs, k, oi, od, s));
        else {
            const int th = heap_threads(k);
            PCC_TRY(set_heap_smem(knn_heap_kernel));
            knn_heap_kernel<<<nblocks(v.nq, th), th, (size_t)k * th * sizeof(nkey_t), s>>>(g, v, k, oi, od);
            PCC_LAUNCHED();
        }
        PCC_CUDA(cudaGetLastError());
    }
    timer.stop();
    if (getenv("PCC_STATS") && k > 1 && k <= 32) {
        unsigned long long h[14];
        cudaMemcpyAsync(h, idx->misc.as<uint32_t>() + 2, 112, cudaMemcpyDeviceToHost, s); cudaStreamSynchronize(s);
        const double q = (double)std::max<unsigned long long>(h[0], 1);
        fprintf(stderr, "[pcc stats] queries=%llu logged/q=%.1f log_overflow=%.5f need_ring2=%.3f fixup=%.5f members/q=%.2f\n",
                h[0], h[1] / q, h[3] / q, h[4] / q, h[5] / q, h[6] / q);
        fprintf(stderr, "[pcc stats] wide queries=%llu steps/q=%.1f final R: <=1 %llu, 2 %llu, 3 %llu, 4-7 %llu, 8-15 %llu, 16+ %llu\n", h[2], h[7] / (double)std::max<unsigned long long>(h[2], 1), h[8], h[9], h[10], h[11], h[12], h[13]);
    }
    if (mem == PCC_HOST) {
        PCC_TRY(copy_out(out_idx, oi, cells * 4, mem, s));
        PCC_TRY(copy_out(out_d2, od, cells * 4, mem, s));
        if (sync) PCC_CUDA(cudaStreamSynchronize(s));
    }
    return PCC_OK;
}

extern "C" {

int pcc_knn(pcc_index *idx, const void *q, int64_t nq, int stride_bytes, int k, int32_t *out_idx, float *out_d2, int *k_eff, int mem, void *stream) {
    PCC_TRY(check_common(idx, stream));
    if (k < 1 || k > PCC_MAX_K) return fail(PCC_ERR_INVALID, "k=%d outside 1..%d", k, PCC_MAX_K);
    cudaStream_t s = (cudaStream_t)stream;
    static const int64_t kChunk = getenv("PCC_PIPE_CHUNK_LOG2") ? (1ll << std::max(16, std::min(24, atoi(getenv("PCC_PIPE_CHUNK_LOG2"))))) : (1ll << 20);
    if (mem == PCC_HOST && q && nq >= 2 * kChunk && !idx->timing && stride_bytes >= 12 && !(stride_bytes & 3)) {
        if (!out_idx || !out_d2) return fail(PCC_ERR_INVALID, "output pointers are NULL");
        if (!idx->shadow) {
            idx->shadow = new pcc_index();
            idx->shadow->device = idx->device;
            idx->shadow->grid_owner = idx;
            PCC_CUDA(cudaMallocHost(&idx->shadow->h_pinned, 4096));
            for (int i = 0; i < 2; ++i) PCC_CUDA(cudaStreamCreateWithFlags(&idx->pipe_stream[i], cudaStreamNonBlocking));
        }
        pcc_index *sh = idx->shadow;
        sh->built = true; sh->n_input = idx->n_input; sh->n_indexed = idx->n_indexed; sh->gh = idx->gh;
        PCC_CUDA(cudaStreamSynchronize(s));
        int rc = PCC_OK;
        int64_t c0 = 0;
        for (int i = 0; c0 < nq && rc == PCC_OK; ++i, c0 += kChunk) {
            const int64_t n = std::min(kChunk, nq - c0);
            rc = knn_impl((i & 1) ? sh : idx, (const uint8_t *)q + c0 * stride_bytes, n, stride_bytes, k, out_idx + c0 * k, out_d2 + c0 * k, k_eff, PCC_HOST, idx->pipe_stream[i & 1], false);
        }
        cudaStreamSynchronize(idx->pipe_stream[0]);
        cudaStreamSynchronize(idx->pipe_stream[1]);
        return rc;
    }
    return knn_impl(idx, q, nq, stride_bytes, k, out_idx, out_d2, k_eff, mem, s, true);
}

int pcc_knn_mean_dist(pcc_index *idx, const void *q, int64_t nq, int stride_bytes, int mean_k, float *out_mean, int mem, void *stream) {
    PCC_TRY(check_common(idx, stream));
    if (mean_k < 1 || mean_k + 1 > PCC_MAX_K) return fail(PCC_ERR_INVALID, "mean_k=%d outside 1..%d", mean_k, PCC_MAX_K - 1);
    cudaStream_t s = (cudaStream_t)stream;
    Queries qs;
    PCC_TRY(prepare_queries(idx, q, nq, stride_bytes, mem, s, &qs));
    if (qs.rows == 0) return PCC_OK;
    if (!out_mean) return fail(PCC_ERR_INVALID, "output pointer is NULL");
    float *od = out_mean;
    if (mem == PCC_HOST) { PCC_TRY(idx->out_f.reserve((size_t)qs.rows * 4)); od = idx->out_f.as<float>(); }
    if (qs.self && !idx->all_rows_indexed) PCC_CUDA(cudaMemsetAsync(od, 0, (size_t)qs.rows * 4, s));
    const Grid g = idx->grid();
    const QueryView v = view_of(qs);
    const int need = mean_k + 1;
    KernelTimer timer(idx, s);
    if (qs.nq > 0) {
        const unsigned nb = nblocks(v.nq, 128);
#define PCC_MD(KK)                                                                            \
    if (need == KK) mean_dist_reg_kernel<KK, true><<<nb, 128, 0, s>>>(g, v, mean_k, od);          \
    else mean_dist_reg_kernel<KK, false><<<nb, 128, 0, s>>>(g, v, mean_k, od)
        if (need <= 2) { PCC_MD(2); }
        else if (need <= 5) { PCC_MD(5); }
        else if (need <= 9) { PCC_MD(9); }
        else if (need <= 17) { PCC_MD(17); }
        else if (need <= 33) { PCC_MD(33); }
        else if (need <= 51) { PCC_MD(51); }
#undef PCC_MD
        else {
            const int th = heap_threads(need);
            PCC_TRY(set_heap_smem(mean_dist_heap_kernel));
            mean_dist_heap_kernel<<<nblocks(v.nq, th), th, (size_t)need * th * sizeof(nkey_t), s>>>(g, v, mean_k, od);
        }
        PCC_LAUNCHED();
        PCC_CUDA(cudaGetLastError());
    }
    timer.stop();
    if (mem == PCC_HOST) { PCC_TRY(copy_out(out_mean, od, (size_t)qs.rows * 4, mem, s)); PCC_CUDA(cudaStreamSynchronize(s)); }
    return PCC_OK;
}

int pcc_normals_knn(pcc_index *idx, const void *q, int64_t nq, int stride_bytes, int k, const float viewpoint[3], float *out, int mem, void *stream) {
    PCC_TRY(check_common(idx, stream));
    if (k < 1 || k > PCC_MAX_K) return fail(PCC_ERR_INVALID, "k=%d outside 1..%d", k, PCC_MAX_K);
    cudaStream_t s = (cudaStream_t)stream;
    Queries qs;
    PCC_TRY(prepare_queries(idx, q, nq, stride_bytes, mem, s, &qs));
    if (qs.rows == 0) return PCC_OK;
    if (!out) return fail(PCC_ERR_INVALID, "output pointer is NULL");
    if (!idx->inv_valid) PCC_TRY(rebuild_inverse(idx, s));
    float4 *od = (float4 *)out;
    if (mem == PCC_HOST) { PCC_TRY(idx->out_f.reserve((size_t)qs.rows * 16)); od = idx->out_f.as<float4>(); }
    if (qs.self && !idx->all_rows_indexed) PCC_CUDA(cudaMemsetAsync(od, 0xFF, (size_t)qs.rows * 16, s));
    const float vx = viewpoint ? viewpoint[0] : 0.f, vy = viewpoint ? viewpoint[1] : 0.f, vz = viewpoint ? viewpoint[2] : 0.f;
    const Grid g = idx->grid();
    const QueryView v = view_of(qs);
    const uint32_t *inv = idx->inv_pos.as<uint32_t>();
    KernelTimer timer(idx, s);
    if (qs.nq > 0) {
        const unsigned nb = nblocks(v.nq, 128);
        if (k <= 8) normals_knn_reg_kernel<8><<<nb, 128, 0, s>>>(g, v, k, inv, vx, vy, vz, od);
        else if (k <= 16) normals_knn_reg_kernel<16><<<nb, 128, 0, s>>>(g, v, k, inv, vx, vy, vz, od);
        else if (k <= 32) normals_knn_reg_kernel<32><<<nb, 128, 0, s>>>(g, v, k, inv, vx, vy, vz, od);
        else {
            const int th = heap_threads(k);
            PCC_TRY(set_heap_smem(normals_knn_heap_kernel));
            normals_knn_heap_kernel<<<nblocks(v.nq, th), th, (size_t)k * th * sizeof(nkey_t), s>>>(g, v, k, inv, vx, vy, vz, od);
        }
        PCC_LAUNCHED();
        PCC_CUDA(cudaGetLastError());
    }
    timer.stop();
    if (mem == PCC_HOST) { PCC_TRY(copy_out(out, od, (size_t)qs.rows * 16, mem, s)); PCC_CUDA(cudaStreamSynchronize(s)); }
    return PCC_OK;
}

int pcc_icp_step(pcc_index *idx, void *src_inout, int64_t ns, int stride_bytes, const float *T_apply, double sums[16], int64_t *count,
                 int32_t *corr_idx, float *corr_d2, int mem, void *stream) {
    PCC_TRY(check_common(idx, stream));
    if (ns < 0 || stride_bytes < 12 || (stride_bytes & 3)) return fail(PCC_ERR_INVALID, "bad source cloud (ns=%lld stride=%d)", (long long)ns, stride_bytes);
    if (!sums || !count) return fail(PCC_ERR_INVALID, "sums / count are NULL");
    cudaStream_t s = (cudaStream_t)stream;
    for (int i = 0; i < 16; ++i) sums[i] = 0;
    *count = 0;
    if (ns == 0) return PCC_OK;
    Queries qs;
    PCC_TRY(prepare_queries(idx, src_inout, ns, stride_bytes, mem, s, &qs));
    float4 *work = idx->qbuf.as<float4>();
    Mat34 T; int apply = 0;
    if (T_apply) { memcpy(T.m, T_apply, sizeof(T.m)); apply = 1; } else memset(&T, 0, sizeof(T));
    const unsigned nb = nblocks(ns, kIcpThreads);
    PCC_TRY(idx->keys64b.reserve(((size_t)nb * 17 + 32) * sizeof(double)));
    double *partials = idx->keys64b.as<double>();
    double *d_out = partials + (size_t)nb * 17;
    int32_t *ci = corr_idx; float *cd = corr_d2;
    if (mem == PCC_HOST) {
        if (corr_idx) { PCC_TRY(idx->out_i.reserve((size_t)ns * 4)); ci = idx->out_i.as<int32_t>(); }
        if (corr_d2) { PCC_TRY(idx->out_f.reserve((size_t)ns * 4)); cd = idx->out_f.as<float>(); }
    }
    KernelTimer timer(idx, s);
    static const bool no_prior = getenv("PCC_ICP_NO_PRIOR") != nullptr;
    uint32_t *prior = nullptr;
    if (!no_prior) {
        const bool fresh = idx->icp_prior_n != ns;
        if (fresh) {
            PCC_TRY(idx->icp_prior.reserve((size_t)std::max<int64_t>(ns, 1) * 4));
            PCC_CUDA(cudaMemsetAsync(idx->icp_prior.p, 0xFF, (size_t)std::max<int64_t>(ns, 1) * 4, s));
            idx->icp_prior_n = ns;
        }
        prior = idx->icp_prior.as<uint32_t>();
    }
    icp_step_kernel<<<nb, kIcpThreads, 0, s>>>(idx->grid(), work, qs.order, ns, T, apply, partials, ci, cd, prior);
    PCC_LAUNCHED();
    icp_reduce_kernel<<<17, 256, 0, s>>>(partials, nb, d_out);
    PCC_LAUNCHED();
    if (idx->icp_allreduce) PCC_TRY(comm_allreduce_f64(idx, d_out, 17, s));
    PCC_CUDA(cudaGetLastError());
    timer.stop();
    double *h = (double *)idx->h_pinned;
    PCC_CUDA(cudaMemcpyAsync(h, d_out, 17 * sizeof(double), cudaMemcpyDeviceToHost, s));
    if (apply) {
        if (mem == PCC_DEVICE) {
            icp_store_kernel<<<nblocks(ns, 256), 256, 0, s>>>(work, ns, (uint8_t *)src_inout, stride_bytes);
            PCC_LAUNCHED();
        } else {
            icp_store_kernel<<<nblocks(ns, 256), 256, 0, s>>>(work, ns, idx->raw.as<uint8_t>(), stride_bytes);
            PCC_LAUNCHED();
            PCC_CUDA(cudaMemcpyAsync(src_inout, idx->raw.p, (size_t)ns * stride_bytes, cudaMemcpyDeviceToHost, s));
        }
    }
    if (mem == PCC_HOST) {
        if (corr_idx) PCC_TRY(copy_out(corr_idx, ci, (size_t)ns * 4, mem, s));
        if (corr_d2) PCC_TRY(copy_out(corr_d2, cd, (size_t)ns * 4, mem, s));
    }
    PCC_CUDA(cudaStreamSynchronize(s));
    for (int i = 0; i < 16; ++i) sums[i] = h[i];
    *count = (int64_t)llround(h[16]);
    return PCC_OK;
}

}
```

### pointcloudcomparator_b200/csrc/pcc_knn_thr.cuh

```cuda
#pragma once
#include <utility>

#include "pcc_device.cuh"

namespace pcc {

#ifndef PCC_THR_QAHEAD
#define PCC_THR_QAHEAD 0
#endif
#ifndef PCC_THR_EARLY
#define PCC_THR_EARLY 16
#endif
#ifndef PCC_THR_JOINT
#define PCC_THR_JOINT 1
#endif
#ifndef PCC_THR_SLOTS8
#define PCC_THR_SLOTS8 36
#endif
#ifndef PCC_THR_SLOTS16
#define PCC_THR_SLOTS16 48
#endif
#ifndef PCC_THR_SLOTS32
#define PCC_THR_SLOTS32 100
#endif
#ifndef PCC_THR_MB8
#define PCC_THR_MB8 6
#endif
#ifndef PCC_THR_MB16
#define PCC_THR_MB16 4
#endif
#ifndef PCC_THR_MB32
#define PCC_THR_MB32 4
#endif
template <int K> struct ThrCfg {
    static constexpr int B = K <= 16 ? 16 : 32;
    static constexpr int slots = K <= 8 ? PCC_THR_SLOTS8 : (K <= 16 ? PCC_THR_SLOTS16 : PCC_THR_SLOTS32);
    static constexpr int slot_bits = slots <= 64 ? 6 : 7;
    static constexpr int threads = K <= 16 ? 128 : 64;
    static constexpr int min_blocks = K <= 8 ? PCC_THR_MB8 : (K <= 16 ? PCC_THR_MB16 : PCC_THR_MB32);
    static constexpr size_t smem = (size_t)slots * threads * sizeof(uint2);
    static_assert(slots <= (1 << slot_bits) && slots % 4 == 0, "log slots must fit the key's slot field");
};
constexpr int kCalibBuckets = 64, kCalibBins = 64;
constexpr float kCalibBinsPerOctave = 8.f;

template <class F, int... I> __device__ __forceinline__ void static_for_impl(F &&f, std::integer_sequence<int, I...>) { (f(std::integral_constant<int, I>{}), ...); }
template <int N, class F> __device__ __forceinline__ void static_for(F &&f) { static_for_impl(f, std::make_integer_sequence<int, N>{}); }
__device__ __forceinline__ void ce_u32(uint32_t &a, uint32_t &b) { const uint32_t lo = min(a, b), hi = max(a, b); a = lo; b = hi; }
template <int N> struct OemNet {
    int a[N * 8], b[N * 8], n;
    constexpr OemNet() : a(), b(), n(0) {
        for (int p = 1; p < N; p <<= 1)
            for (int k = p; k >= 1; k >>= 1)
                for (int j = k % p; j <= N - 1 - k; j += 2 * k)
                    for (int i = 0; i < k; ++i)
                        if (i + j + k < N && (i + j) / (2 * p) == (i + j + k) / (2 * p)) { a[n] = i + j; b[n] = i + j + k; ++n; }
    }
};
template <int N, int... I>
__device__ __forceinline__ void oem_apply_u32(uint32_t (&v)[N], std::integer_sequence<int, I...>) {
    constexpr OemNet<N> net{};
    (ce_u32(v[net.a[I]], v[net.b[I]]), ...);
}
template <int N>
__device__ __forceinline__ void oem_sort_u32(uint32_t (&v)[N]) {
    constexpr OemNet<N> net{};
    oem_apply_u32<N>(v, std::make_integer_sequence<int, net.n>{});
}
template <int N> struct BitonicMergeNet {
    int a[N * 8], b[N * 8], n;
    constexpr BitonicMergeNet() : a(), b(), n(0) {
        for (int j = N >> 1; j > 0; j >>= 1)
            for (int i = 0; i < N; ++i)
                if ((i ^ j) > i) { a[n] = i; b[n] = i ^ j; ++n; }
    }
};
template <int N, int... I>
__device__ __forceinline__ void bitonic_merge_apply_u32(uint32_t (&v)[N], std::integer_sequence<int, I...>) {
    constexpr BitonicMergeNet<N> net{};
    (ce_u32(v[net.a[I]], v[net.b[I]]), ...);
}
template <int N>
__device__ __forceinline__ void merge_prune_u32(uint32_t (&best)[N], const uint32_t (&blk)[N], uint32_t &dropmin) {
    static_for<N>([&](auto I) {
        constexpr int i = decltype(I)::value;
        const uint32_t a = best[i], b = blk[N - 1 - i];
        best[i] = min(a, b);
        dropmin = min(dropmin, max(a, b));
    });
    constexpr BitonicMergeNet<N> net{};
    bitonic_merge_apply_u32<N>(best, std::make_integer_sequence<int, net.n>{});
}

template <int K>
__global__ void __launch_bounds__(128) knn_calib_kernel(Grid g, QueryView v, int k, int64_t stride, unsigned *__restrict__ hist) {
    const int64_t t = ((int64_t)blockIdx.x * blockDim.x + threadIdx.x) * stride;
    float x, y, z; int64_t row; bool empty;
    if (!load_query(g, v, t, x, y, z, row, empty)) return;
    const QueryCell c = locate(g, x, y, z);
    RegDist<K> list; list.init();
    uint32_t M = 0;
    scan_shell(g, c, -1, 1, [&](uint32_t, float4 p) { list.offer(dist2(x, y, z, p.x, p.y, p.z)); ++M; });
    const float kth = (k == K) ? list.d[K - 1] : list.at(k - 1);
    if (kth == CUDART_INF_F) return;
    const float ratio = (kth - list.d[0]) * g.inv_cell * g.inv_cell * (float)M / (float)k;
    const int bin = min(max((int)floorf(log2f(fmaxf(ratio, 1e-6f)) * kCalibBinsPerOctave) + kCalibBins / 2, 0), kCalibBins - 1);
    atomicAdd(hist + min(M >> 2, (uint32_t)kCalibBuckets - 1u) * kCalibBins + bin, 1u);
}
__global__ void knn_calib_finish_kernel(const unsigned *__restrict__ hist, float *__restrict__ ratio, float quant) {
    __shared__ unsigned all[kCalibBins];
    __shared__ float all_r;
    const int b = threadIdx.x;
    unsigned s = 0;
    for (int i = 0; i < kCalibBuckets; ++i) s += hist[i * kCalibBins + b];
    all[b] = s;
    __syncthreads();
    if (b == 0) {
        unsigned tot = 0; for (int j = 0; j < kCalibBins; ++j) tot += all[j];
        float r = 8.f;
        if (tot) { unsigned cum = 0; int j = 0; for (; j < kCalibBins; ++j) { cum += all[j]; if ((float)cum >= quant * (float)tot) break; } r = exp2f((float)(min(j, kCalibBins - 1) + 1 - kCalibBins / 2) / kCalibBinsPerOctave); }
        all_r = r;
    }
    __syncthreads();
    unsigned tot = 0; for (int j = 0; j < kCalibBins; ++j) tot += hist[b * kCalibBins + j];
    float r = all_r;
    if (tot >= 64) { unsigned cum = 0; int j = 0; for (; j < kCalibBins; ++j) { cum += hist[b * kCalibBins + j]; if ((float)cum >= quant * (float)tot) break; } r = exp2f((float)(min(j, kCalibBins - 1) + 1 - kCalibBins / 2) / kCalibBinsPerOctave); }
    ratio[b] = r;
}

__device__ __forceinline__ void sts_v2(uint32_t addr, uint32_t a, uint32_t b) { asm volatile("st.shared.v2.u32 [%0], {%1, %2};" ::"r"(addr), "r"(a), "r"(b) : "memory"); }
template <uint32_t STRIDE> __device__ __forceinline__ void advance_if_le(uint32_t &wa, float d, float tau) {
    asm("{\n\t.reg .pred p;\n\tsetp.le.f32 p, %1, %2;\n\t@p add.u32 %0, %0, %3;\n\t}" : "+r"(wa) : "f"(d), "f"(tau), "n"(STRIDE));
}
template <uint32_t STRIDE> __device__ __forceinline__ void advance_if_le_and(uint32_t &wa, float d, float tau, bool ok) {
    asm("{\n\t.reg .pred p, q;\n\tsetp.ne.u32 q, %4, 0;\n\tsetp.le.and.f32 p, %1, %2, q;\n\t@p add.u32 %0, %0, %3;\n\t}" : "+r"(wa) : "f"(d), "f"(tau), "n"(STRIDE), "r"((uint32_t)ok));
}
#ifndef PCC_THR_PREFETCH
#define PCC_THR_PREFETCH 3
#endif
__device__ __forceinline__ void prefetch_l2(const void *p) { asm volatile("prefetch.global.L2 [%0];" ::"l"(p)); }
__device__ __forceinline__ void prefetch_l1(const void *p) { asm volatile("prefetch.global.L1 [%0];" ::"l"(p)); }
template <int LINES, bool L1>
__device__ __forceinline__ void prefetch_run(const float4 *pts, uint32_t j, uint32_t e) {
    if (j >= e) return;
    const char *a = (const char *)(pts + j), *last = (const char *)(pts + (e - 1));
#pragma unroll
    for (int i = 0; i < LINES; ++i) {
        const char *q = a + 128 * i;
        if (q <= last || i == 0) { if (L1) prefetch_l1(q); else prefetch_l2(q); }
    }
    if (L1) prefetch_l1(last); else prefetch_l2(last);
}
#ifndef PCC_THR_PIPE
#define PCC_THR_PIPE 0
#endif
struct Quad { float4 p0, p1, p2, p3; };
template <bool GEN> __device__ __forceinline__ float4 load_pt(const float4 *pts, uint32_t j) { if (GEN) return pts[j]; return __ldg(pts + j); }
template <bool GEN> __device__ __forceinline__ Quad load_quad(const float4 *pts, uint32_t j) { Quad q; q.p0 = load_pt<GEN>(pts, j); q.p1 = load_pt<GEN>(pts, j + 1); q.p2 = load_pt<GEN>(pts, j + 2); q.p3 = load_pt<GEN>(pts, j + 3); return q; }
template <uint32_t STRIDE, bool COMPRESS, class F>
__device__ __forceinline__ void thr_quad(const Quad &q, const uint32_t j, const float x, const float y, const float z, float &T, float &dmin, float &tau, uint32_t &wa, const uint32_t cap, F &&on_full) {
    const float d0 = dist2(x, y, z, q.p0.x, q.p0.y, q.p0.z), d1 = dist2(x, y, z, q.p1.x, q.p1.y, q.p1.z), d2 = dist2(x, y, z, q.p2.x, q.p2.y, q.p2.z), d3 = dist2(x, y, z, q.p3.x, q.p3.y, q.p3.z);
    sts_v2(wa, __float_as_uint(d0), j); advance_if_le<STRIDE>(wa, d0, tau);
    sts_v2(wa, __float_as_uint(d1), j + 1); advance_if_le<STRIDE>(wa, d1, tau);
    sts_v2(wa, __float_as_uint(d2), j + 2); advance_if_le<STRIDE>(wa, d2, tau);
    sts_v2(wa, __float_as_uint(d3), j + 3); advance_if_le<STRIDE>(wa, d3, tau);
    dmin = fminf(fminf(dmin, fminf(d0, d1)), fminf(d2, d3)); tau = dmin + T;
    if (!COMPRESS) wa = min(wa, cap);
    else if (PCC_THR_JOINT ? __any_sync(__activemask(), wa >= cap) : (wa >= cap)) on_full();
}
template <uint32_t STRIDE, bool COMPRESS, bool GEN, class F>
__device__ __forceinline__ void thr_walk_run(const float4 *pts, uint32_t j, const uint32_t e, const float x, const float y, const float z, float &T,
                                             float &dmin, float &tau, uint32_t &wa, const uint32_t cap, F &&on_full) {
#if PCC_THR_PIPE
    bool have_a = j + 4 <= e;
    Quad a, b;
    if (have_a) a = load_quad<GEN>(pts, j);
    while (have_a) {
        const bool have_b = j + 8 <= e;
        if (have_b) b = load_quad<GEN>(pts, j + 4);
        thr_quad<STRIDE, COMPRESS>(a, j, x, y, z, T, dmin, tau, wa, cap, on_full);
        j += 4;
        if (!have_b) break;
        have_a = j + 8 <= e;
        if (have_a) a = load_quad<GEN>(pts, j + 4);
        thr_quad<STRIDE, COMPRESS>(b, j, x, y, z, T, dmin, tau, wa, cap, on_full);
        j += 4;
    }
#else
#ifndef PCC_THR_EXP
#define PCC_THR_EXP 0
#endif
    const uint32_t j0 = j;
    for (; j + 4 <= e; j += 4) {
        const Quad a = load_quad<GEN>(pts, PCC_THR_EXP == 1 ? j0 : (PCC_THR_EXP == 2 ? 0u : j));
        thr_quad<STRIDE, COMPRESS>(a, j, x, y, z, T, dmin, tau, wa, cap, on_full);
    }
#endif
    if (j < e) {
        const float4 p0 = load_pt<GEN>(pts, j), p1 = load_pt<GEN>(pts, min(j + 1, e - 1)), p2 = load_pt<GEN>(pts, min(j + 2, e - 1));
        const float d0 = dist2(x, y, z, p0.x, p0.y, p0.z), d1 = dist2(x, y, z, p1.x, p1.y, p1.z), d2 = dist2(x, y, z, p2.x, p2.y, p2.z);
        sts_v2(wa, __float_as_uint(d0), j); advance_if_le<STRIDE>(wa, d0, tau);
        sts_v2(wa, __float_as_uint(d1), j + 1); advance_if_le_and<STRIDE>(wa, d1, tau, j + 1 < e);
        sts_v2(wa, __float_as_uint(d2), j + 2); advance_if_le_and<STRIDE>(wa, d2, tau, j + 2 < e);
        dmin = fminf(fminf(dmin, d0), fminf(d1, d2)); tau = dmin + T;
        if (!COMPRESS) wa = min(wa, cap);
        else if (PCC_THR_JOINT ? __any_sync(__activemask(), wa >= cap) : (wa >= cap)) on_full();
    }
}

constexpr float kRetryScale = 4.f;
#ifndef PCC_THR_TILE
#define PCC_THR_TILE 384
#endif
namespace thr_tma {
__device__ __forceinline__ uint32_t smem_u32(const void *p) { return (uint32_t)__cvta_generic_to_shared(p); }
__device__ __forceinline__ void mbar_init(unsigned long long *bar, unsigned count) {
    asm volatile("mbarrier.init.shared::cta.b64 [%0], %1;" ::"r"(smem_u32(bar)), "r"(count) : "memory");
    asm volatile("fence.mbarrier_init.release.cluster;" ::: "memory");
}
__device__ __forceinline__ void mbar_expect_tx(unsigned long long *bar, unsigned bytes) {
    asm volatile("mbarrier.arrive.expect_tx.shared::cta.b64 _, [%0], %1;" ::"r"(smem_u32(bar)), "r"(bytes) : "memory");
}
__device__ __forceinline__ void bulk_g2s(void *dst, const void *src, unsigned bytes, unsigned long long *bar) {
    asm volatile("cp.async.bulk.shared::cluster.global.mbarrier::complete_tx::bytes [%0], [%1], %2, [%3];"
                 ::"r"(smem_u32(dst)), "l"(src), "r"(bytes), "r"(smem_u32(bar)) : "memory");
}
__device__ __forceinline__ void mbar_wait(unsigned long long *bar, unsigned parity) {
    asm volatile("{\n\t.reg .pred p;\n\tWAIT_%=:\n\tmbarrier.try_wait.parity.shared::cta.b64 p, [%0], %1;\n\t@p bra DONE_%=;\n\tbra WAIT_%=;\n\tDONE_%=:\n\t}"
                 ::"r"(smem_u32(bar)), "r"(parity) : "memory");
}
}
#ifndef PCC_THR_MAIN_COMPRESS
#define PCC_THR_MAIN_COMPRESS 0
#endif
template <int K, bool FULLK, bool RETRY, bool STAGED = false, bool COMPRESS = RETRY>
__device__ __forceinline__ void knn_thr_body(const Grid &g, const QueryView &v, const int64_t t, const int k_rt, int32_t *__restrict__ out_idx, float *__restrict__ out_d2, int vec4,
                                             const FixList &fix, const float *__restrict__ ratio, uint2 *__restrict__ slog, const bool loose = false,
                                             float4 *tile = nullptr, unsigned long long *bar = nullptr) {
    constexpr int TH = ThrCfg<K>::threads, SLOTS = ThrCfg<K>::slots, B = ThrCfg<K>::B;
    constexpr uint32_t SMASK = (1u << ThrCfg<K>::slot_bits) - 1u;
    const int k = FULLK ? K : k_rt;
    float x = 0.f, y = 0.f, z = 0.f; int64_t row = 0; bool empty = false;
#if PCC_THR_QAHEAD
    uint32_t qi_ahead = 0xFFFFFFFFu;
    if (!RETRY && !STAGED && v.order) {
        constexpr int64_t AHEAD = (int64_t)PCC_THR_QAHEAD * ThrCfg<K>::threads;
        if ((threadIdx.x & 31) == 0 && t + 2 * AHEAD < v.nq) prefetch_l2(v.order + t + 2 * AHEAD);
        if (t + AHEAD < v.nq) qi_ahead = __ldg(v.order + t + AHEAD);
    }
#endif
    const bool live = load_query(g, v, t, x, y, z, row, empty);
    auto leave_dead = [&]() {
        if (t < v.nq) fix.ring_flag[t] = 0;
        if (empty) { nkey_t e[K];
#pragma unroll
            for (int j = 0; j < K; ++j) e[j] = PCC_EMPTY_KEY;
            write_row<K>(e, k, out_idx + row * k, out_d2 + row * k, vec4); }
    };
    if (!STAGED && !live) { leave_dead(); return; }
    QueryCell c; c.cx = c.cy = c.cz = 0; c.ux = c.uy = c.uz = 0.f;
    if (live) c = locate(g, x, y, z);
    uint32_t M = 0, s0 = 0, e0 = 0, rowmask = 0;
    if (live) {
        const int xa = max(c.cx - 1, 0), xb = min(c.cx + 1, g.nx - 1);
        uint32_t rs[9], re[9];
#pragma unroll
        for (int r = 0; r < 9; ++r) {
            const int zz = c.cz + centre_out(r / 3), yy = c.cy + centre_out(r % 3);
            rs[r] = re[r] = 0;
            if (zz >= 0 && zz < g.nz && yy >= 0 && yy < g.ny) {
                const size_t rowb = ((size_t)zz * g.ny + yy) * g.nx;
                rs[r] = cell_begin(g, rowb + xa); re[r] = cell_begin(g, rowb + xb + 1);
            }
        }
#pragma unroll
        for (int r = 0; r < 9; ++r) { M += re[r] - rs[r]; rowmask |= (re[r] > rs[r] ? 1u : 0u) << r; if (!STAGED && (PCC_THR_PREFETCH & 1)) prefetch_run<3, false>(g.pts, rs[r], re[r]); }
        s0 = rs[0]; e0 = re[0];
    }
#if PCC_THR_QAHEAD
    if (!RETRY && !STAGED && qi_ahead != 0xFFFFFFFFu) prefetch_l2(v.q + qi_ahead);
#endif
    auto leave_wide = [&]() {
        fix.ring_flag[t] = 0;
        if (fix.stats) { atomicAdd(fix.stats + 0, 1ull); atomicAdd(fix.stats + 4, 1ull); }
        push_list(fix.wide_list, fix.wide_count, (uint32_t)t);
    };
    const bool walker = live && M >= (uint32_t)k;
    if (!STAGED && !walker) { leave_wide(); return; }
    bool lane_staged = false;
    uint32_t my_start = 0, my_off = 0;
    if (STAGED) {
        const unsigned full = 0xffffffffu;
        const int lane = threadIdx.x & 31;
        const unsigned wmask = __ballot_sync(full, walker);
        if (wmask) {
            const int leader = __ffs(wmask) - 1;
            const int lcy = __shfl_sync(full, c.cy, leader), lcz = __shfl_sync(full, c.cz, leader);
            bool inrow = walker && c.cy == lcy && c.cz == lcz;
            const int xmin = __reduce_min_sync(full, inrow ? c.cx : 0x7fffffff);
            inrow = inrow && c.cx <= xmin + 9;
            const int xmax = __reduce_max_sync(full, inrow ? c.cx : xmin);
            uint32_t len = 0;
            if (lane < 9) {
                const int zz = lcz + centre_out(lane / 3), yy = lcy + centre_out(lane % 3);
                if (zz >= 0 && zz < g.nz && yy >= 0 && yy < g.ny) {
                    const uint32_t *rowp = g.cell_start + ((size_t)zz * g.ny + yy) * g.nx;
                    my_start = __ldg(rowp + max(xmin - 1, 0)); len = __ldg(rowp + min(xmax + 1, g.nx - 1) + 1) - my_start;
                }
            }
            uint32_t inc = len;
#pragma unroll
            for (int o = 1; o < 16; o <<= 1) { const uint32_t w = __shfl_up_sync(full, inc, o); if (lane >= o) inc += w; }
            my_off = inc - len;
            const uint32_t total = __shfl_sync(full, inc, 8);
            if (total <= (uint32_t)PCC_THR_TILE && total > 0) {
                if (lane == 0) thr_tma::mbar_expect_tx(bar, total * 16u);
                __syncwarp();
                if (lane < 9 && len) thr_tma::bulk_g2s(tile + my_off, g.pts + my_start, len * 16u, bar);
                lane_staged = inrow;
                thr_tma::mbar_wait(bar, 0);
            }
        }
    }
    float T = __ldg(ratio + min(M >> 2, (uint32_t)kCalibBuckets - 1u)) * (float)k / (float)max(M, 1u) * (g.cell * g.cell) * ((RETRY && loose) ? kRetryScale : 1.f);
    float dmin = CUDART_INF_F;
    if (walker && e0 > s0) { const float4 p = __ldg(g.pts + ((s0 + e0) >> 1)); dmin = dist2(x, y, z, p.x, p.y, p.z); }
    float tau = dmin + T;
    constexpr uint32_t STRIDE = (uint32_t)TH * (uint32_t)sizeof(uint2);
    constexpr int LOGCAP = SLOTS - 4;
    const uint32_t wa0 = (uint32_t)__cvta_generic_to_shared(slog), cap = wa0 + (uint32_t)LOGCAP * STRIDE;
    uint32_t wa = wa0;
    uint32_t best[B], dropmin;
    auto select_log = [&](const int n) {
        auto load_keys = [&](uint32_t (&key)[B], const int b0) {
            static_for<B>([&](auto I) {
                constexpr int i = decltype(I)::value;
                key[i] = b0 + i < n ? (((slog[(b0 + i) * TH].x << 1) & ~SMASK) | (uint32_t)(b0 + i)) : 0xFFFFFFFFu;
            });
        };
        dropmin = 0xFFFFFFFFu;
        load_keys(best, 0);
        oem_sort_u32<B>(best);
        for (int b0 = B; b0 < n; b0 += B) {
            uint32_t blk[B];
            load_keys(blk, b0);
            oem_sort_u32<B>(blk);
            merge_prune_u32<B>(best, blk, dropmin);
        }
    };
    auto kth_key = [&]() {
        uint32_t kth = best[K - 1];
        if (!FULLK) {
            kth = 0u;
            static_for<K - 1>([&](auto I) { constexpr int i = decltype(I)::value; kth = max(kth, i < k ? best[i] : 0u); });
        }
        return kth;
    };
    bool give_up = false;
    auto compress_if = [&](const int min_n) {
        const int nf = (int)((wa - wa0) / STRIDE);
        if (nf < min_n) return;
        select_log(nf);
        const float tau_new = __uint_as_float(slog[(kth_key() & SMASK) * TH].x) * (1.f + 1.f / 32768.f);
        if (tau_new < tau) { dmin = 0.f; T = tau_new; tau = tau_new; }
        int m = 0;
        for (int i = 0; i < nf; ++i) { const uint2 e = slog[i * TH]; if (__uint_as_float(e.x) <= tau) { slog[m * TH] = e; ++m; } }
        if (m >= LOGCAP - 4) { give_up = true; m = 0; }
        wa = wa0 + (uint32_t)m * STRIDE;
    };
    auto on_full = [&]() { compress_if(wa >= cap ? 0 : K + 13); };
    {
        const RowRuns none = {0u, 0u, 0u, 0u};
        int az = 0, ay = 0;
        if (!walker) rowmask = 0;
        RowRuns nxt = (rowmask & 1u) ? row_runs(g, c, -1, 1, to_cell_units(g, tau), 0, 0) : none;
        for (;;) {
            const RowRuns cur = nxt;
            const int r = az * 3 + ay;
            if (++ay == 3) { ay = 0; ++az; }
            const bool more = az < 3;
            nxt = none;
            if (more && ((rowmask >> (az * 3 + ay)) & 1u)) { nxt = row_runs(g, c, -1, 1, to_cell_units(g, tau), az, ay); if (!STAGED && (PCC_THR_PREFETCH & 2)) prefetch_run<3, true>(g.pts, nxt.j1, nxt.e1); }
            if (STAGED) {
                const uint32_t st = __shfl_sync(0xffffffffu, my_start, r), of = __shfl_sync(0xffffffffu, my_off, r);
                const float4 *src = lane_staged ? (const float4 *)tile + of - st : g.pts;
                thr_walk_run<STRIDE, COMPRESS, true>(src, cur.j1, cur.e1, x, y, z, T, dmin, tau, wa, cap, on_full);
            } else thr_walk_run<STRIDE, COMPRESS, false>(g.pts, cur.j1, cur.e1, x, y, z, T, dmin, tau, wa, cap, on_full);
            (void)r;
            if (!more) break;
            if (COMPRESS && PCC_THR_EARLY > 0) {
                const int nl = (int)((wa - wa0) / STRIDE);
                if (__any_sync(__activemask(), nl >= LOGCAP - PCC_THR_EARLY)) compress_if(K + 5);
            }
        }
    }
    if (STAGED && !live) { leave_dead(); return; }
    if (STAGED && !walker) { leave_wide(); return; }
    if (RETRY && give_up) { fix.ring_flag[t] = 0; knn_reg_body<K>(g, v, t, k, out_idx, out_d2, vec4); return; }
    if (!RETRY && COMPRESS && give_up) { fix.ring_flag[t] = 0; push_list(fix.retry_list, fix.retry_count, (uint32_t)t); return; }
    const int n = (int)((wa - wa0) / STRIDE);
    select_log(n);
    const uint32_t kth = kth_key();
    uint32_t gap = 0xFFFFFFFFu;
    static_for<K>([&](auto I) {
        constexpr int i = decltype(I)::value;
        const uint32_t nxt = i + 1 < B ? best[i + 1] : dropmin;
        const uint32_t d = nxt - best[i];
        gap = min(gap, (FULLK || i < k) ? d : 0xFFFFFFFFu);
    });
    const bool overflow = n >= LOGCAP;
    const bool tie = kth == 0xFFFFFFFFu || gap <= SMASK;
    float tau_k = CUDART_INF_F;
    if (kth != 0xFFFFFFFFu) tau_k = __uint_as_float(slog[(kth & SMASK) * TH].x);
    const bool under = !(tau_k <= tau);
    if (fix.stats && !RETRY) { atomicAdd(fix.stats + 0, 1ull); atomicAdd(fix.stats + 1, (unsigned long long)n); atomicAdd(fix.stats + 3, overflow ? 1ull : 0ull); atomicAdd(fix.stats + 5, (overflow || tie || under) ? 1ull : 0ull); atomicAdd(fix.stats + 6, (unsigned long long)M); }
    if (!RETRY && (overflow || tie || under)) {
        fix.ring_flag[t] = 0;
        push_list(fix.retry_list, fix.retry_count, (uint32_t)t | ((under && !overflow) ? 0x80000000u : 0u));
        return;
    }
    int32_t *oi = out_idx + row * k; float *od = out_d2 + row * k;
    if (RETRY && (overflow || tie || under)) {
        RegList<K> list; list.init();
        if (!overflow) for (int i = 0; i < n; ++i) { const uint2 e = slog[i * TH]; list.offer(((nkey_t)e.x << 32) | __float_as_uint(__ldg(&g.pts[e.y].w))); }
        const nkey_t kk = FULLK ? list.key[K - 1] : list.at(k - 1);
        tau_k = key_d2(kk);
        if (overflow || kk == PCC_EMPTY_KEY || !(tau_k <= tau)) { fix.ring_flag[t] = 0; knn_reg_body<K>(g, v, t, k, out_idx, out_d2, vec4); return; }
        const float cov = covered_d2(g, c, 1);
        const bool proved = cov == CUDART_INF_F || tau_k < cov;
        const bool wide = !proved && next_ring(g, 1, tau_k) > kRingMaxR;
        fix.ring_flag[t] = (!proved && !wide) ? 1 : 0;
        if (wide) { push_list(fix.wide_list, fix.wide_count, (uint32_t)t); return; }
        write_row<K>(list.key, k, oi, od, vec4);
        return;
// ... 57 lines not shown
```

### pointcloudcomparator_b200/csrc/pcc_radius.cu

```cuda
#include <cub/cub.cuh>
#include <algorithm>
#include <cmath>
#include <cstring>

#include "pcc_internal.h"

namespace pcc {

struct QueryView { const float4 *q; const uint32_t *order; int64_t nq; bool self; };
static inline QueryView view_of(const Queries &q) { return QueryView{q.q, q.order, q.nq, q.self}; }
static inline unsigned nblocks(int64_t n, int threads) { return (unsigned)std::max<int64_t>(1, (n + threads - 1) / threads); }

__device__ __forceinline__ bool load_query(const Grid &g, const QueryView &v, int64_t t, float &x, float &y, float &z, int64_t &row) {
    if (t >= v.nq) return false;
    if (v.self) { float4 p = __ldg(g.pts + t); x = p.x; y = p.y; z = p.z; row = __float_as_int(p.w); return true; }
    uint32_t qi = v.order ? __ldg(v.order + t) : (uint32_t)t;
    float4 p = __ldg(v.q + qi); x = p.x; y = p.y; z = p.z; row = qi;
    return finite3(x, y, z) && g.n > 0;
}

template <class F>
__device__ __forceinline__ void radius_visit(const Grid &g, float x, float y, float z, float r2, int R0, F &&f) {
    const QueryCell c = locate(g, x, y, z);
    int Rin = -1, R = R0;
    for (;;) {
        scan_shell(g, c, Rin, R, [&](uint32_t pos, float4 p) { const float d2 = dist2(x, y, z, p.x, p.y, p.z); if (d2 < r2) f(pos, p, d2); });
        if (covered_d2(g, c, R) >= r2) break;
        Rin = R; ++R;
    }
}

__global__ void __launch_bounds__(128) radius_count_kernel(Grid g, QueryView v, float r2, int R0, unsigned max_nn, int64_t *__restrict__ counts) {
    const int64_t t = (int64_t)blockIdx.x * blockDim.x + threadIdx.x;
    float x, y, z; int64_t row;
    if (!load_query(g, v, t, x, y, z, row)) return;
    unsigned n = 0;
    radius_visit(g, x, y, z, r2, R0, [&](uint32_t, float4, float) { ++n; });
    if (max_nn && n > max_nn) n = max_nn;
    counts[row] = n;
}
__global__ void __launch_bounds__(128) radius_fill_kernel(Grid g, QueryView v, float r2, int R0, const int64_t *__restrict__ offsets, nkey_t *__restrict__ keys) {
    const int64_t t = (int64_t)blockIdx.x * blockDim.x + threadIdx.x;
    float x, y, z; int64_t row;
    if (!load_query(g, v, t, x, y, z, row)) return;
    nkey_t *o = keys + offsets[row];
    int lead = (int)((4u - (unsigned)(((uintptr_t)o >> 3) & 3u)) & 3u);
    nkey_t p0 = 0, p1 = 0, p2 = 0, p3 = 0;
    int n = 0;
    radius_visit(g, x, y, z, r2, R0, [&](uint32_t, float4 p, float d2) {
        const nkey_t key = make_key(d2, __float_as_uint(p.w));
        if (lead > 0) { *o++ = key; --lead; return; }
        const int slot = n & 3;
        if (slot == 0) p0 = key; else if (slot == 1) p1 = key; else if (slot == 2) p2 = key; else p3 = key;
        ++n;
        if (slot == 3) { reinterpret_cast<ulonglong2 *>(o)[0] = make_ulonglong2(p0, p1); reinterpret_cast<ulonglong2 *>(o)[1] = make_ulonglong2(p2, p3); o += 4; }
    });
    const int rest = n & 3;
    if (rest > 0) o[0] = p0;
    if (rest > 1) o[1] = p1;
    if (rest > 2) o[2] = p2;
}
__global__ void radius_capped_kernel(Grid g, QueryView v, float r2, int R0, int max_nn, const int64_t *__restrict__ offsets, nkey_t *__restrict__ keys) {
    extern __shared__ nkey_t smem_keys[];
    const int64_t t = (int64_t)blockIdx.x * blockDim.x + threadIdx.x;
    float x, y, z; int64_t row;
    if (!load_query(g, v, t, x, y, z, row)) return;
    HeapList list; list.init(smem_keys + threadIdx.x, blockDim.x, max_nn);
    radius_visit(g, x, y, z, r2, R0, [&](uint32_t, float4 p, float d2) { list.offer(make_key(d2, __float_as_uint(p.w))); });
    list.finish();
    nkey_t *o = keys + offsets[row];
    for (int j = 0; j < list.cnt; ++j) o[j] = list.at(j);
}
template <int KPL>
__device__ __forceinline__ void warp_sort_regs(nkey_t (&v)[KPL], int lane) {
    constexpr int N = 32 * KPL;
#pragma unroll
    for (int kk = 2; kk <= N; kk <<= 1) {
#pragma unroll
        for (int j = kk >> 1; j > 0; j >>= 1) {
            if (j >= 32) {
                const int jj = j >> 5;
#pragma unroll
                for (int r = 0; r < KPL; ++r) {
                    if ((r & jj) == 0) {
                        const nkey_t a = v[r], b = v[r | jj];
                        const bool up = (((r << 5) | lane) & kk) == 0;
                        const bool sw = (b < a) == up;
                        v[r] = sw ? b : a; v[r | jj] = sw ? a : b;
                    }
                }
            } else {
#pragma unroll
                for (int r = 0; r < KPL; ++r) {
                    const nkey_t o = __shfl_xor_sync(0xffffffffu, v[r], j);
                    const bool up = (((r << 5) | lane) & kk) == 0, lower = (lane & j) == 0;
                    v[r] = ((lower == up) == (o < v[r])) ? o : v[r];
                }
            }
        }
    }
}
template <int KPL>
__device__ __forceinline__ void sort_row_in_place(nkey_t *__restrict__ k, int n, int lane) {
    nkey_t v[KPL];
#pragma unroll
    for (int r = 0; r < KPL; ++r) v[r] = (r * 32 + lane) < n ? k[r * 32 + lane] : PCC_EMPTY_KEY;
    warp_sort_regs<KPL>(v, lane);
#pragma unroll
    for (int r = 0; r < KPL; ++r) if ((r * 32 + lane) < n) k[r * 32 + lane] = v[r];
}
static constexpr int kRowSortWarps = 4, kRowSortCap = 1024;
__global__ void __launch_bounds__(kRowSortWarps * 32) sort_rows_kernel(const int64_t *__restrict__ offsets, int64_t rows, nkey_t *__restrict__ keys,
                                                                       uint32_t *__restrict__ big_rows, unsigned *__restrict__ n_big) {
    __shared__ nkey_t sm_all[kRowSortWarps][kRowSortCap];
    const int warp = threadIdx.x >> 5, lane = threadIdx.x & 31;
    const int64_t row = (int64_t)blockIdx.x * kRowSortWarps + warp;
    if (row >= rows) return;
    const int64_t b = offsets[row];
    const int64_t n64 = offsets[row + 1] - b;
    if (n64 <= 1) return;
    if (n64 > kRowSortCap) { if (lane == 0) big_rows[atomicAdd(n_big, 1u)] = (uint32_t)row; return; }
    const int n = (int)n64;
    nkey_t *k = keys + b;
    if (n <= 32) {
        nkey_t v = lane < n ? k[lane] : PCC_EMPTY_KEY;
#pragma unroll
        for (int kk = 2; kk <= 32; kk <<= 1) {
#pragma unroll
            for (int j = kk >> 1; j > 0; j >>= 1) {
                const nkey_t o = __shfl_xor_sync(0xffffffffu, v, j);
                const bool up = (lane & kk) == 0, lower = (lane & j) == 0;
                const nkey_t mn = v < o ? v : o, mx = v < o ? o : v;
                v = (lower == up) ? mn : mx;
            }
        }
        if (lane < n) k[lane] = v;
        return;
    }
    if (n <= 64) { sort_row_in_place<2>(k, n, lane); return; }
    if (n <= 128) { sort_row_in_place<4>(k, n, lane); return; }
    if (n <= 256) { sort_row_in_place<8>(k, n, lane); return; }
    nkey_t *sm = sm_all[warp];
    int P = 64; while (P < n) P <<= 1;
    for (int i = lane; i < P; i += 32) sm[i] = i < n ? k[i] : PCC_EMPTY_KEY;
    __syncwarp();
    for (int kk = 2; kk <= P; kk <<= 1) {
        for (int j = kk >> 1; j > 0; j >>= 1) {
            for (int t = lane; t < (P >> 1); t += 32) {
                const int i = ((t & ~(j - 1)) << 1) | (t & (j - 1));
                const nkey_t a = sm[i], c = sm[i + j];
                const bool up = (i & kk) == 0;
                if ((c < a) == up) { sm[i] = c; sm[i + j] = a; }
            }
            __syncwarp();
        }
    }
    for (int i = lane; i < n; i += 32) k[i] = sm[i];
}
constexpr int kSelBuckets = 64;
struct SelParam { float scale; int bucket; int R; int pad; };
#ifndef PCC_SELB
#define PCC_SELB 6
#endif
__global__ void __launch_bounds__(128, PCC_SELB) select_bound_kernel(Grid g, QueryView v, int k, int64_t *__restrict__ counts, SelParam *__restrict__ params) {
    __shared__ uint32_t hist_all[kSelBuckets * 128];
    uint32_t *hist = hist_all + threadIdx.x;
    const int64_t t = (int64_t)blockIdx.x * blockDim.x + threadIdx.x;
    float x, y, z; int64_t row;
    if (!load_query(g, v, t, x, y, z, row)) return;
    const QueryCell c = locate(g, x, y, z);
    int R = 1, B = -1;
    unsigned m = 0;
    float scale = 0.f;
    for (;;) {
        const float cov = covered_d2(g, c, R);
        float hi = cov;
        if (cov == CUDART_INF_F) {
            float mx = 0.f;
            scan_shell(g, c, -1, R, [&](uint32_t, float4 p) { mx = fmaxf(mx, dist2(x, y, z, p.x, p.y, p.z)); });
            hi = fmaxf(mx * 1.0001f, 1e-30f);
            if (!(hi < CUDART_INF_F)) hi = 3.0e38f;
        }
        unsigned seen = 0;
        if (hi > 0.f) {
            scale = (float)kSelBuckets / hi;
#pragma unroll 8
            for (int b = 0; b < kSelBuckets; ++b) hist[b * 128] = 0u;
            scan_shell(g, c, -1, R, [&](uint32_t, float4 p) {
                const float fb = __fmul_rn(dist2(x, y, z, p.x, p.y, p.z), scale);
                if (fb < (float)kSelBuckets) hist[(int)fb * 128] += 1u;
            });
            for (int b = 0; b < kSelBuckets; ++b) { seen += hist[b * 128]; if (seen >= (unsigned)k) { B = b; break; } }
        }
        if (B >= 0) { m = seen; break; }
        if (cov == CUDART_INF_F) { B = kSelBuckets - 1; m = seen; break; }
        R = seen > 0 ? R + 1 : next_ring(g, R, CUDART_INF_F);
    }
    counts[row] = (m + 3u) & ~3u;
    SelParam sp; sp.scale = scale; sp.bucket = B; sp.R = R; sp.pad = 0;
    params[row] = sp;
}
__global__ void __launch_bounds__(128) select_fill_kernel(Grid g, QueryView v, const int64_t *__restrict__ offsets, const SelParam *__restrict__ params, nkey_t *__restrict__ keys) {
    const int64_t t = (int64_t)blockIdx.x * blockDim.x + threadIdx.x;
    float x, y, z; int64_t row;
    if (!load_query(g, v, t, x, y, z, row)) return;
    if (offsets[row + 1] == offsets[row]) return;
    const SelParam sp = params[row];
    const QueryCell c = locate(g, x, y, z);
    ulonglong2 *o = reinterpret_cast<ulonglong2 *>(keys + offsets[row]);
    const float edge = (float)(sp.bucket + 1) / sp.scale;
    const float limit = (float)(sp.bucket + 1);
    nkey_t p0 = PCC_EMPTY_KEY, p1 = PCC_EMPTY_KEY, p2 = PCC_EMPTY_KEY, p3 = PCC_EMPTY_KEY;
    int n = 0;
    scan_clipped(g, c, -1, sp.R, to_cell_units(g, edge * 1.00001f), [&](uint32_t, float4 p) {
        const float d2 = dist2(x, y, z, p.x, p.y, p.z);
        const float fb = __fmul_rn(d2, sp.scale);
        if (fb < (float)kSelBuckets && (float)(int)fb < limit) {
            const nkey_t key = make_key(d2, __float_as_uint(p.w));
            const int slot = n & 3;
            if (slot == 0) p0 = key; else if (slot == 1) p1 = key; else if (slot == 2) p2 = key; else p3 = key;
            ++n;
            if (slot == 3) { o[0] = make_ulonglong2(p0, p1); o[1] = make_ulonglong2(p2, p3); o += 2; p0 = p1 = p2 = p3 = PCC_EMPTY_KEY; }
        }
    });
    if (n & 3) { o[0] = make_ulonglong2(p0, p1); o[1] = make_ulonglong2(p2, p3); }
}
__global__ void select_unpack_kernel(const int64_t *__restrict__ offsets, const nkey_t *__restrict__ keys, int64_t rows, int k, int32_t *__restrict__ idx, float *__restrict__ d2) {
    const int64_t i = (int64_t)blockIdx.x * blockDim.x + threadIdx.x;
    if (i >= rows * k) return;
    const int64_t row = i / k; const int j = (int)(i - row * k);
    const int64_t b = offsets[row], e = offsets[row + 1];
    const nkey_t key = b + j < e ? keys[b + j] : PCC_EMPTY_KEY;
    idx[i] = key_idx(key); d2[i] = key_d2(key);
}
template <int KPL>
__device__ __forceinline__ void sort_unpack_row(const nkey_t *__restrict__ k_in, int n, int k, int lane, int32_t *__restrict__ oi, float *__restrict__ od) {
    nkey_t v[KPL];
#pragma unroll
    for (int r = 0; r < KPL; ++r) v[r] = (r * 32 + lane) < n ? k_in[r * 32 + lane] : PCC_EMPTY_KEY;
    warp_sort_regs<KPL>(v, lane);
#pragma unroll
    for (int r = 0; r < KPL; ++r) { const int e = r * 32 + lane; if (e < k) { oi[e] = key_idx(v[r]); od[e] = key_d2(v[r]); } }
}
__global__ void __launch_bounds__(128) select_sort_unpack_kernel(const int64_t *__restrict__ offsets, const nkey_t *__restrict__ keys, int64_t rows, int k,
                                                                 int32_t *__restrict__ idx, float *__restrict__ d2, unsigned *__restrict__ n_long) {
    const int lane = threadIdx.x & 31;
    const int64_t row = (int64_t)blockIdx.x * 4 + (threadIdx.x >> 5);
    if (row >= rows) return;
    const int64_t b = offsets[row], n64 = offsets[row + 1] - b;
    int32_t *oi = idx + row * k; float *od = d2 + row * k;
    if (n64 > 256) { if (lane == 0) atomicAdd(n_long, 1u); return; }
    const int n = (int)n64;
    if (n <= 32) {
        nkey_t v[1] = {lane < n ? keys[b + lane] : PCC_EMPTY_KEY};
        warp_sort_regs<1>(v, lane);
        for (int e = lane; e < k; e += 32) { oi[e] = e < 32 ? key_idx(v[0]) : -1; od[e] = e < 32 ? key_d2(v[0]) : CUDART_INF_F; }
    } else if (n <= 64) {
        sort_unpack_row<2>(keys + b, n, k, lane, oi, od);
        for (int e = 64 + lane; e < k; e += 32) { oi[e] = -1; od[e] = CUDART_INF_F; }
    } else if (n <= 128) {
        sort_unpack_row<4>(keys + b, n, k, lane, oi, od);
        for (int e = 128 + lane; e < k; e += 32) { oi[e] = -1; od[e] = CUDART_INF_F; }
    } else {
        sort_unpack_row<8>(keys + b, n, k, lane, oi, od);
        for (int e = 256 + lane; e < k; e += 32) { oi[e] = -1; od[e] = CUDART_INF_F; }
    }
}
__global__ void big_row_bounds_kernel(const int64_t *__restrict__ offsets, const uint32_t *__restrict__ big_rows, unsigned n_big, int64_t *__restrict__ begin, int64_t *__restrict__ end) {
    const unsigned i = blockIdx.x * blockDim.x + threadIdx.x;
    if (i < n_big) { begin[i] = offsets[big_rows[i]]; end[i] = offsets[big_rows[i] + 1]; }
}
__global__ void big_row_copy_kernel(const int64_t *__restrict__ begin, const int64_t *__restrict__ end, const nkey_t *__restrict__ src, nkey_t *__restrict__ dst) {
    for (int64_t i = begin[blockIdx.x] + threadIdx.x; i < end[blockIdx.x]; i += blockDim.x) dst[i] = src[i];
}
__global__ void unpack_kernel(const nkey_t *__restrict__ keys, int64_t n, int32_t *__restrict__ idx, float *__restrict__ d2) {
    int64_t i = (int64_t)blockIdx.x * blockDim.x + threadIdx.x;
    if (i >= n) return;
    nkey_t k = keys[i];
    idx[i] = (int32_t)(uint32_t)k; d2[i] = __uint_as_float((uint32_t)(k >> 32));
}

__global__ void __launch_bounds__(128) normals_rows_kernel(Grid g, QueryView v, const int64_t *__restrict__ offsets, const nkey_t *__restrict__ keys,
                                                           const uint32_t *__restrict__ inv_pos, float vx, float vy, float vz, float4 *__restrict__ out) {
    const int64_t t = (int64_t)blockIdx.x * blockDim.x + threadIdx.x;
    if (t >= v.nq) return;
    float x, y, z; int64_t row;
    if (v.self) { float4 p = __ldg(g.pts + t); x = p.x; y = p.y; z = p.z; row = __float_as_int(p.w); }
    else { uint32_t qi = v.order ? __ldg(v.order + t) : (uint32_t)t; float4 p = __ldg(v.q + qi); x = p.x; y = p.y; z = p.z; row = qi; }
    const int64_t b = offsets[row], e = offsets[row + 1];
    float a[9] = {0, 0, 0, 0, 0, 0, 0, 0, 0};
    for (int64_t j = b; j < e; ++j) { float4 p = __ldg(g.pts + __ldg(inv_pos + (uint32_t)keys[j])); accu_add(a, p.x, p.y, p.z); }
    out[row] = normal_from_accu(a, (int)min((int64_t)INT_MAX, e - b), x, y, z, vx, vy, vz);
}

__device__ __forceinline__ int64_t rows_query(const Grid &g, const QueryView &v, int64_t t, float &x, float &y, float &z) {
    if (v.self) { float4 p = __ldg(g.pts + t); x = p.x; y = p.y; z = p.z; return __float_as_int(p.w); }
    uint32_t qi = v.order ? __ldg(v.order + t) : (uint32_t)t; float4 p = __ldg(v.q + qi); x = p.x; y = p.y; z = p.z; return qi;
}

__global__ void __launch_bounds__(128) gradient_rows_kernel(Grid g, QueryView v, const int64_t *__restrict__ offsets, const nkey_t *__restrict__ keys,
                                                            const uint32_t *__restrict__ inv_pos, const float *__restrict__ intensity,
                                                            const float4 *__restrict__ normals, float4 *__restrict__ out) {
    const int64_t t = (int64_t)blockIdx.x * blockDim.x + threadIdx.x;
    if (t >= v.nq) return;
    float qx, qy, qz;
    const int64_t row = rows_query(g, v, t, qx, qy, qz);
    const int64_t b = offsets[row], e = offsets[row + 1];
    const float qnan = CUDART_NAN_F;
    if (e - b < 3) { out[row] = make_float4(qnan, qnan, qnan, 0.f); return; }
    float cx = 0.f, cy = 0.f, cz = 0.f, mi = 0.f;
    for (int64_t j = b; j < e; ++j) {
        const uint32_t id = (uint32_t)keys[j];
        const float4 p = __ldg(g.pts + __ldg(inv_pos + id));
        cx += p.x; cy += p.y; cz += p.z;
        mi += __ldg(intensity + id);
    }
    const float fn = (float)(e - b);
    cx = __fdiv_rn(cx, fn); cy = __fdiv_rn(cy, fn); cz = __fdiv_rn(cz, fn); mi = __fdiv_rn(mi, fn);
    float a00 = 0.f, a01 = 0.f, a02 = 0.f, a11 = 0.f, a12 = 0.f, a22 = 0.f, b0 = 0.f, b1 = 0.f, b2 = 0.f;
    for (int64_t j = b; j < e; ++j) {
        const uint32_t id = (uint32_t)keys[j];
        const float4 p = __ldg(g.pts + __ldg(inv_pos + id));
        const float in = __ldg(intensity + id);
        if (!isfinite(in)) continue;
        const float x = p.x - cx, y = p.y - cy, z = p.z - cz, w = in - mi;
        a00 += x * x; a01 += x * y; a02 += x * z;
        a11 += y * y; a12 += y * z;
        a22 += z * z;
        b0 += x * w; b1 += y * w; b2 += z * w;
    }
    float A[9] = {a00, a01, a02, a01, a11, a12, a02, a12, a22};
    const float rhs[3] = {b0, b1, b2};
    float xs[3];
    colpiv_qr_solve(A, rhs, xs);
    const float4 n = __ldg(normals + row);
    const float nn[3] = {n.x, n.y, n.z};
    float gr[3];
#pragma unroll
    for (int r = 0; r < 3; ++r) {
        const float m0 = (r == 0 ? 1.f : 0.f) - nn[r] * nn[0];
        const float m1 = (r == 1 ? 1.f : 0.f) - nn[r] * nn[1];
        const float m2 = (r == 2 ? 1.f : 0.f) - nn[r] * nn[2];
        gr[r] = sum3(m0 * xs[0], m1 * xs[1], m2 * xs[2]);
    }
    out[row] = make_float4(gr[0], gr[1], gr[2], 0.f);
}

__device__ __forceinline__ float rift_sq_norm(const float (&h)[32], int nb) {
    if (nb < 4) {
        float s = h[0] * h[0];
#pragma unroll
        for (int i = 1; i < 3; ++i) if (i < nb) s = s + h[i] * h[i];
        return s;
    }
    const int aligned = nb & ~3, aligned2 = nb & ~7;
    float r0[4], r1[4];
#pragma unroll
    for (int l = 0; l < 4; ++l) r0[l] = h[l] * h[l];
    if (aligned > 4) {
#pragma unroll
        for (int l = 0; l < 4; ++l) r1[l] = h[4 + l] * h[4 + l];
#pragma unroll
        for (int idx = 8; idx < 32; idx += 8) {
            if (idx < aligned2) {
#pragma unroll
                for (int l = 0; l < 4; ++l) { r0[l] = r0[l] + h[idx + l] * h[idx + l]; r1[l] = r1[l] + h[idx + 4 + l] * h[idx + 4 + l]; }
            }
        }
#pragma unroll
        for (int l = 0; l < 4; ++l) r0[l] = r0[l] + r1[l];
        if (aligned > aligned2) {
#pragma unroll
            for (int idx = 0; idx < 32; idx += 8) {
                if (idx == aligned2) {
#pragma unroll
                    for (int l = 0; l < 4; ++l) r0[l] = r0[l] + h[idx + l] * h[idx + l];
                }
            }
        }
    }
    float s = (r0[0] + r0[2]) + (r0[1] + r0[3]);
#pragma unroll
    for (int i = 4; i < 32; ++i) if (i >= aligned && i < nb) s = s + h[i] * h[i];
    return s;
}

__global__ void __launch_bounds__(128) rift_rows_kernel(Grid g, QueryView v, const int64_t *__restrict__ offsets, const nkey_t *__restrict__ keys,
                                                        const uint32_t *__restrict__ inv_pos, const float4 *__restrict__ gradient, float radius,
                                                        int nd, int ng, float *__restrict__ out) {
    const int64_t t = (int64_t)blockIdx.x * blockDim.x + threadIdx.x;
    if (t >= v.nq) return;
    float qx, qy, qz;
    const int64_t row = rows_query(g, v, t, qx, qy, qz);
    const int nb = nd * ng;
    float *o = out + row * nb;
    const int64_t b = offsets[row], e = offsets[row + 1];
    if (e == b) { for (int k = 0; k < nb; ++k) o[k] = CUDART_NAN_F; return; }
    float h[32];
#pragma unroll
    for (int k = 0; k < 32; ++k) h[k] = 0.f;
    const float rden = radius + 1.1920929e-07f, gden = 3.14159274f + 1.1920929e-07f;
    const float fnd = (float)nd, fng = (float)ng;
    for (int64_t j = b; j < e; ++j) {
        const nkey_t key = keys[j];
        const uint32_t id = (uint32_t)key;
        const float4 p = __ldg(g.pts + __ldg(inv_pos + id));
        const float4 gv = __ldg(gradient + id);
        const float mag = sqrtf(sum3(gv.x * gv.x, gv.y * gv.y, gv.z * gv.z));
        float ux = p.x - qx, uy = p.y - qy, uz = p.z - qz;
        const float z = sum3(ux * ux, uy * uy, uz * uz);
        if (z > 0.f) { const float s = sqrtf(z); ux = __fdiv_rn(ux, s); uy = __fdiv_rn(uy, s); uz = __fdiv_rn(uz, s); }
        float ang = acosf(__fdiv_rn(sum3(gv.x * ux, gv.y * uy, gv.z * uz), mag));
        if (!isfinite(ang)) ang = 0.f;
        const float dist = __fdiv_rn(fnd * sqrtf(__uint_as_float((uint32_t)(key >> 32))), rden);
        const float grad = __fdiv_rn(fng * ang, gden);
        const int dmin = max((int)ceilf(dist - 1.f), 0), dmax = min((int)floorf(dist + 1.f), nd - 1);
        const int gmin = (int)ceilf(grad - 1.f), gmax = (int)floorf(grad + 1.f);
        for (int gi = gmin; gi <= gmax; ++gi) {
            const int gw = (gi + ng) % ng;
            const float wg = 1.0f - fabsf(grad - (float)gi);
            for (int di = dmin; di <= dmax; ++di) {
                const float w = (1.0f - fabsf(dist - (float)di)) * wg;
                const float add = w * mag;
                const int bin = gw * nd + di;
#pragma unroll
                for (int k = 0; k < 32; ++k) if (k == bin) h[k] += add;
            }
        }
    }
    const float z = rift_sq_norm(h, nb);
    if (z > 0.f) {
        const float s = sqrtf(z);
#pragma unroll
        for (int k = 0; k < 32; ++k) h[k] = __fdiv_rn(h[k], s);
    }
#pragma unroll
    for (int k = 0; k < 32; ++k) if (k < nb) o[k] = h[k];
}

struct SiftScales { float sigma_sqr[16]; float cutoff[16]; };

__global__ void __launch_bounds__(128) sift_dog_rows_kernel(Grid g, QueryView v, const int64_t *__restrict__ offsets, const nkey_t *__restrict__ keys,
                                                            const float *__restrict__ values, SiftScales sc, int ns, float *__restrict__ out) {
    const int64_t t = (int64_t)blockIdx.x * blockDim.x + threadIdx.x;
    if (t >= v.nq) return;
    float qx, qy, qz;
    const int64_t row = rows_query(g, v, t, qx, qy, qz);
    const int64_t b = offsets[row], e = offsets[row + 1];
    float num[16], den[16];
#pragma unroll
    for (int s = 0; s < 16; ++s) { num[s] = 0.f; den[s] = 0.f; }
    for (int64_t j = b; j < e; ++j) {
        const nkey_t key = keys[j];
        const float d2 = __uint_as_float((uint32_t)(key >> 32));
        const float val = __ldg(values + (uint32_t)key);
#pragma unroll
        for (int s = 0; s < 16; ++s) {
            if (s < ns && d2 <= sc.cutoff[s]) {
                const float w = sift_expf(__fdiv_rn(__fmul_rn(-0.5f, d2), sc.sigma_sqr[s]));
                num[s] = __fadd_rn(num[s], __fmul_rn(val, w));
                den[s] = __fadd_rn(den[s], w);
            }
        }
    }
    float *o = out + row * (ns - 1);
    float prev = 0.f;
#pragma unroll
    for (int s = 0; s < 16; ++s) {
        if (s < ns) {
            const float resp = __fdiv_rn(num[s], den[s]);
            if (s > 0) o[s - 1] = __fsub_rn(resp, prev);
            prev = resp;
        }
    }
}

__global__ void __launch_bounds__(128) first_within_kernel(Grid g, QueryView v, double thr, float r2_cover, int R0, int32_t *__restrict__ out) {
    const int64_t t = (int64_t)blockIdx.x * blockDim.x + threadIdx.x;
    if (t >= v.nq) return;
    const uint32_t qi = v.order ? __ldg(v.order + t) : (uint32_t)t;
    const float4 q = __ldg(v.q + qi);
    int32_t best = INT_MAX;
    if (finite3(q.x, q.y, q.z) && g.n > 0) {
        const QueryCell c = locate(g, q.x, q.y, q.z);
        int Rin = -1, R = R0;
        for (;;) {
            scan_shell(g, c, Rin, R, [&](uint32_t, float4 p) {
                const double dx = (double)(q.x - p.x), dy = (double)(q.y - p.y), dz = (double)(q.z - p.z);
                if (sqrt(dx * dx + dy * dy + dz * dz) < thr) best = min(best, __float_as_int(p.w));
            });
            if (covered_d2(g, c, R) >= r2_cover) break;
            Rin = R; ++R;
        }
    }
    out[qi] = best == INT_MAX ? -1 : best;
}

__device__ __forceinline__ uint32_t uf_find(uint32_t *parent, uint32_t x) {
    uint32_t p = __ldcg(parent + x);
    while (p != x) { uint32_t gp = __ldcg(parent + p); if (gp != p) parent[x] = gp; x = p; p = gp; }
    return x;
}
__device__ __forceinline__ void uf_union(uint32_t *parent, uint32_t a, uint32_t b) {
    for (;;) {
        a = uf_find(parent, a); b = uf_find(parent, b);
        if (a == b) return;
        if (a < b) { uint32_t t = a; a = b; b = t; }
        const uint32_t old = atomicCAS(parent + a, a, b);
        if (old == a) return;
        a = old;
    }
}
__global__ void iota_kernel(uint32_t *p, int64_t n) { int64_t i = (int64_t)blockIdx.x * blockDim.x + threadIdx.x; if (i < n) p[i] = (uint32_t)i; }
__global__ void __launch_bounds__(128) ece_link_kernel(Grid g, float r2, int R0, uint32_t *__restrict__ parent) {
    const int64_t t = (int64_t)blockIdx.x * blockDim.x + threadIdx.x;
    if (t >= g.n) return;
    const float4 q = __ldg(g.pts + t);
    uint32_t ra = uf_find(parent, (uint32_t)t);
    radius_visit(g, q.x, q.y, q.z, r2, R0, [&](uint32_t pos, float4, float) {
        if (pos >= (uint32_t)t) return;
        if (pos == ra || __ldcg(parent + pos) == ra) return;
        uf_union(parent, ra, pos);
        ra = uf_find(parent, ra);
    });
}
__global__ void __launch_bounds__(128) ece_link_range_kernel(Grid g, float r2, int R0, uint32_t begin, uint32_t end, uint32_t *__restrict__ parent) {
    const int64_t t = (int64_t)begin + (int64_t)blockIdx.x * blockDim.x + threadIdx.x;
    if (t >= end) return;
    const float4 q = __ldg(g.pts + t);
    uint32_t ra = uf_find(parent, (uint32_t)t);
    radius_visit(g, q.x, q.y, q.z, r2, R0, [&](uint32_t pos, float4, float) {
        if (pos == (uint32_t)t || pos == ra || __ldcg(parent + pos) == ra) return;
        uf_union(parent, ra, pos);
        ra = uf_find(parent, ra);
    });
}
__global__ void ece_absorb_kernel(uint32_t n, const uint32_t *__restrict__ other, uint32_t *__restrict__ parent) {
    const int64_t t = (int64_t)blockIdx.x * blockDim.x + threadIdx.x;
    if (t >= n) return;
    const uint32_t o = other[t];
    if (o != (uint32_t)t && o < n) uf_union(parent, (uint32_t)t, o);
}
__global__ void ece_compress_kernel(uint32_t n, uint32_t *__restrict__ parent) {
    const int64_t t = (int64_t)blockIdx.x * blockDim.x + threadIdx.x;
    if (t < n) parent[t] = uf_find(parent, (uint32_t)t);
}
__global__ void ece_flatten_kernel(Grid g, uint32_t *__restrict__ parent, uint32_t *__restrict__ size, uint32_t *__restrict__ min_orig) {
    const int64_t t = (int64_t)blockIdx.x * blockDim.x + threadIdx.x;
    if (t >= g.n) return;
    const uint32_t r = uf_find(parent, (uint32_t)t);
    parent[t] = r;
    atomicAdd(size + r, 1u);
    atomicMin(min_orig + r, (uint32_t)__float_as_int(__ldg(g.pts + t).w));
}
__global__ void ece_select_kernel(uint32_t n, const uint32_t *__restrict__ parent, const uint32_t *__restrict__ size, const uint32_t *__restrict__ min_orig,
                                  uint32_t min_size, uint32_t max_size, nkey_t *__restrict__ keys, uint32_t *__restrict__ roots, unsigned long long *__restrict__ n_kept) {
    const int64_t t = (int64_t)blockIdx.x * blockDim.x + threadIdx.x;
    if (t >= n || parent[t] != (uint32_t)t) return;
    const uint32_t s = size[t];
    if (s < min_size || s > max_size) return;
    const unsigned long long slot = atomicAdd(n_kept, 1ull);
    keys[slot] = ((nkey_t)(0xFFFFFFFFu - s) << 32) | min_orig[t];
    roots[slot] = (uint32_t)t;
}
__global__ void ece_rank_kernel(const nkey_t *__restrict__ keys_sorted, const uint32_t *__restrict__ roots_sorted, int64_t n_kept, uint32_t *__restrict__ rank_of_root, int64_t *__restrict__ sizes, int64_t sizes_cap) {
    const int64_t i = (int64_t)blockIdx.x * blockDim.x + threadIdx.x;
    if (i >= n_kept) return;
    rank_of_root[roots_sorted[i]] = (uint32_t)i;
    if (sizes && i < sizes_cap) sizes[i] = (int64_t)(0xFFFFFFFFu - (uint32_t)(keys_sorted[i] >> 32));
}
__global__ void ece_label_kernel(Grid g, const uint32_t *__restrict__ parent, const uint32_t *__restrict__ rank_of_root, int32_t *__restrict__ labels) {
    const int64_t t = (int64_t)blockIdx.x * blockDim.x + threadIdx.x;
    if (t >= g.n) return;
    labels[__float_as_int(__ldg(g.pts + t).w)] = (int32_t)rank_of_root[parent[t]];
}
__global__ void fill_u32_kernel(uint32_t *p, int64_t n, uint32_t v) { int64_t i = (int64_t)blockIdx.x * blockDim.x + threadIdx.x; if (i < n) p[i] = v; }
__global__ void fill_f4_kernel(float4 *p, int64_t n, float4 v) { int64_t i = (int64_t)blockIdx.x * blockDim.x + threadIdx.x; if (i < n) p[i] = v; }

static int heap_threads(int k) {
    int t = (int)((96 * 1024) / ((size_t)k * sizeof(nkey_t)));
    t = std::min(128, (t / 32) * 32);
    return std::max(32, t);
}
static inline int ring0(const pcc_index *idx, double radius) { return std::max(1, (int)std::ceil(radius / (double)idx->gh.cell)); }

static int radius_offsets(pcc_index *idx, const Queries &qs, double radius, unsigned max_nn, int64_t *d_offsets, cudaStream_t s) {
    const float r2 = (float)(radius * radius);
    PCC_CUDA(cudaMemsetAsync(d_offsets, 0, (size_t)(qs.rows + 1) * sizeof(int64_t), s));
    if (qs.nq > 0) {
        radius_count_kernel<<<nblocks(qs.nq, 128), 128, 0, s>>>(idx->grid(), view_of(qs), r2, ring0(idx, radius), max_nn, d_offsets);
        PCC_LAUNCHED();
        PCC_CUDA(cudaGetLastError());
    }
    size_t tmp = 0;
    cub::DeviceScan::ExclusiveSum(nullptr, tmp, d_offsets, d_offsets, (int)(qs.rows + 1), s);
    PCC_TRY(idx->cub_tmp.reserve(tmp));
    PCC_CUDA(cub::DeviceScan::ExclusiveSum(idx->cub_tmp.p, tmp, d_offsets, d_offsets, (int)(qs.rows + 1), s));
    g_launches += 2;
    return PCC_OK;
}
static int sort_csr_rows(pcc_index *idx, int64_t rows, const int64_t *d_offsets, int64_t total, nkey_t *keys, cudaStream_t s) {
    Queries qs; qs.rows = rows;
    {
        PCC_TRY(idx->misc.reserve((size_t)qs.rows * 4 + 64));
        unsigned *n_big = idx->misc.as<unsigned>();
        uint32_t *big_rows = idx->misc.as<uint32_t>() + 16;
        PCC_CUDA(cudaMemsetAsync(n_big, 0, 4, s));
        sort_rows_kernel<<<nblocks(qs.rows, kRowSortWarps), kRowSortWarps * 32, 0, s>>>(d_offsets, qs.rows, keys, big_rows, n_big);
        PCC_LAUNCHED();
        PCC_CUDA(cudaGetLastError());
        unsigned *h = (unsigned *)idx->h_pinned;
        PCC_CUDA(cudaMemcpyAsync(h, n_big, 4, cudaMemcpyDeviceToHost, s));
        PCC_CUDA(cudaStreamSynchronize(s));
        const unsigned nb = h[0];
        if (nb > 0) {
            if (total >= (1ll << 31)) return fail(PCC_ERR_INVALID, "radius result of %lld neighbours exceeds the segmented-sort limit", (long long)total);
            PCC_TRY(idx->keys64b.reserve((size_t)total * sizeof(nkey_t)));
            PCC_TRY(idx->parent.reserve((size_t)nb * 16));
            int64_t *bb = idx->parent.as<int64_t>(), *be = bb + nb;
            big_row_bounds_kernel<<<nblocks(nb, 256), 256, 0, s>>>(d_offsets, big_rows, nb, bb, be); PCC_LAUNCHED();
            size_t tmp = 0;
            cub::DeviceSegmentedSort::SortKeys(nullptr, tmp, keys, idx->keys64b.as<nkey_t>(), (int)total, (int)nb, bb, be, s);
            PCC_TRY(idx->cub_tmp.reserve(tmp));
            PCC_CUDA(cub::DeviceSegmentedSort::SortKeys(idx->cub_tmp.p, tmp, keys, idx->keys64b.as<nkey_t>(), (int)total, (int)nb, bb, be, s));
            g_launches += 3;
            big_row_copy_kernel<<<nb, 256, 0, s>>>(bb, be, idx->keys64b.as<nkey_t>(), keys); PCC_LAUNCHED();
            PCC_CUDA(cudaGetLastError());
        }
    }
    return PCC_OK;
}
static int radius_rows(pcc_index *idx, const Queries &qs, double radius, unsigned max_nn, int sorted, const int64_t *d_offsets, int64_t total, nkey_t **keys_out, cudaStream_t s) {
    const float r2 = (float)(radius * radius);
    PCC_TRY(idx->keys64.reserve((size_t)std::max<int64_t>(total, 1) * sizeof(nkey_t)));
// ... 416 lines not shown
```

Before: 2.650 billion.

## Sort queries by cell and scatter them into a sorted buffer

Replaces the full CUB radix sort over all key bits with a CUB sort on the low bits plus a custom top-digit count/scan/scatter pass. The scatter writes both the order and a query array already in sorted order, so search kernels read queries contiguously instead of gathering through the permutation. It also adds a pcc_query_order API and drops an experimental query-prefetch path. The cost is more kernels and extra buffers, and the scatter writes memory in a strided pattern.

```diff
diff --git a/include/pcc/search.h b/include/pcc/search.h
--- a/include/pcc/search.h
+++ b/include/pcc/search.h
@@ -33,6 +33,8 @@
 
 int pcc_knn(pcc_index *idx, const void *q, int64_t nq, int stride_bytes, int k, int32_t *out_idx, float *out_d2,
             int *k_eff, int mem, void *stream);
+
+int pcc_query_order(pcc_index *idx, const void *q, int64_t nq, int stride_bytes, int mem, uint32_t *out_order, uint32_t *out_keys, void *stream);
 
 int pcc_radius_count(pcc_index *idx, const void *q, int64_t nq, int stride_bytes, double radius, unsigned max_nn,
                      int64_t *offsets, int64_t *total, int mem, void *stream);
diff --git a/pointcloudcomparator_b200/_lib.py b/pointcloudcomparator_b200/_lib.py
--- a/pointcloudcomparator_b200/_lib.py
+++ b/pointcloudcomparator_b200/_lib.py
@@ -13,7 +13,7 @@
 
 SYMBOLS = [
     "pcc_last_error", "pcc_version", "pcc_launch_count", "pcc_create", "pcc_destroy", "pcc_build", "pcc_size", "pcc_grid_info",
-    "pcc_knn", "pcc_radius_count", "pcc_radius_fill", "pcc_knn_mean_dist", "pcc_sor_threshold", "pcc_normals_knn",
+    "pcc_knn", "pcc_query_order", "pcc_radius_count", "pcc_radius_fill", "pcc_knn_mean_dist", "pcc_sor_threshold", "pcc_normals_knn",
     "pcc_normals_radius", "pcc_icp_step", "pcc_icp_align", "pcc_umeyama_from_sums", "pcc_euclidean_labels", "pcc_first_within",
     "pcc_export", "pcc_adopt", "pcc_set_timing", "pcc_last_kernel_ms", "pcc_ece_init", "pcc_ece_link_range", "pcc_ece_absorb", "pcc_ece_finish", "pcc_voxel_grid", "pcc_descriptor_nn", "pcc_region_growing",
     "pcc_region_growing_rgb", "pcc_intensity_gradient", "pcc_rift", "pcc_sift_dog", "pcc_sift_extrema", "pcc_sift_keypoints", "pcc_comm_init", "pcc_comm_info", "pcc_broadcast_index", "pcc_gather", "pcc_allreduce_f64",
@@ -43,6 +43,7 @@
     L.pcc_size.restype = i64
     L.pcc_grid_info.argtypes = [vp, C.POINTER(dbl)]
     L.pcc_knn.argtypes = [vp, vp, i64, i32, i32, vp, vp, C.POINTER(i32), i32, vp]
+    L.pcc_query_order.argtypes = [vp, vp, i64, i32, i32, vp, vp, vp]
     L.pcc_radius_count.argtypes = [vp, vp, i64, i32, dbl, u32, vp, C.POINTER(i64), i32, vp]
     L.pcc_radius_fill.argtypes = [vp, vp, i64, i32, dbl, u32, i32, vp, vp, vp, i32, vp]
     L.pcc_knn_mean_dist.argtypes = [vp, vp, i64, i32, i32, vp, i32, vp]
diff --git a/pointcloudcomparator_b200/csrc/pcc_build.cu b/pointcloudcomparator_b200/csrc/pcc_build.cu
--- a/pointcloudcomparator_b200/csrc/pcc_build.cu
+++ b/pointcloudcomparator_b200/csrc/pcc_build.cu
@@ -160,14 +160,76 @@
     return PCC_OK;
 }
 
+__device__ __forceinline__ uint32_t query_key(const BinParams &b, uint32_t bad_key, float x, float y, float z) {
+    return finite3(x, y, z) ? cell_of(b, x, y, z) : bad_key;
+}
 __global__ void qprep_kernel(const uint8_t *__restrict__ raw, int stride, int64_t nq, BinParams b, uint32_t bad_key,
                              float4 *__restrict__ qbuf, uint32_t *__restrict__ keys, uint32_t *__restrict__ perm) {
     int64_t i = (int64_t)blockIdx.x * blockDim.x + threadIdx.x;
     if (i >= nq) return;
     const float *p = (const float *)(raw + i * (int64_t)stride);
     float x = p[0], y = p[1], z = p[2];
-    qbuf[i] = make_float4(x, y, z, 0.f);
-    if (keys) { keys[i] = finite3(x, y, z) ? cell_of(b, x, y, z) : bad_key; perm[i] = (uint32_t)i; }
+    if (qbuf) qbuf[i] = make_float4(x, y, z, 0.f);
+    if (keys) { keys[i] = query_key(b, bad_key, x, y, z); perm[i] = (uint32_t)i; }
+}
+constexpr int kTopBits = 5, kTopBins = 1 << kTopBits, kTopThreads = 256, kTopRounds = 16, kTopTile = kTopThreads * kTopRounds;
+__global__ void __launch_bounds__(kTopThreads) topdigit_count_kernel(const uint32_t *__restrict__ keys, int64_t nq, int low, uint32_t *__restrict__ tile_counts, int64_t ntiles) {
+    __shared__ uint32_t h[kTopBins];
+    if (threadIdx.x < kTopBins) h[threadIdx.x] = 0;
+    __syncthreads();
+    const int64_t base = (int64_t)blockIdx.x * kTopTile;
+    for (int r = 0; r < kTopRounds; ++r) {
+        const int64_t i = base + r * kTopThreads + threadIdx.x;
+        if (i < nq) atomicAdd(h + (__ldg(keys + i) >> low), 1u);
+    }
+    __syncthreads();
+    if (threadIdx.x < kTopBins) tile_counts[threadIdx.x * ntiles + blockIdx.x] = h[threadIdx.x];
+}
+__global__ void __launch_bounds__(kTopThreads) topdigit_scatter_kernel(const uint32_t *__restrict__ keys, const uint32_t *__restrict__ perm, int64_t nq, int low,
+                                                                       const uint32_t *__restrict__ tile_offsets, int64_t ntiles, const uint8_t *__restrict__ raw, int stride,
+                                                                       uint32_t *__restrict__ order, float4 *__restrict__ qsorted) {
+    constexpr int W = kTopThreads / 32;
+    __shared__ uint32_t next[kTopBins];
+    __shared__ uint32_t wpos[W][kTopBins];
+    const int lane = threadIdx.x & 31, warp = threadIdx.x >> 5;
+    if (threadIdx.x < kTopBins) next[threadIdx.x] = tile_offsets[threadIdx.x * ntiles + blockIdx.x];
+    const int64_t base = (int64_t)blockIdx.x * kTopTile;
+    for (int r = 0; r < kTopRounds; ++r) {
+        const int64_t i = base + r * kTopThreads + threadIdx.x;
+        const bool valid = i < nq;
+        const uint32_t d = valid ? __ldg(keys + i) >> low : kTopBins;
+        const uint32_t peers = __match_any_sync(0xffffffffu, d);
+        const int rank = __popc(peers & ((1u << lane) - 1u));
+        wpos[warp][lane] = 0;
+        __syncwarp();
+        if (valid && rank == 0) wpos[warp][d] = __popc(peers);
+        __syncthreads();
+        if (threadIdx.x < kTopBins) {
+            uint32_t run = next[threadIdx.x];
+#pragma unroll
+            for (int w = 0; w < W; ++w) { const uint32_t c = wpos[w][threadIdx.x]; wpos[w][threadIdx.x] = run; run += c; }
+            next[threadIdx.x] = run;
+        }
+        __syncthreads();
+        if (valid) {
+            const uint32_t pos = wpos[warp][d] + rank, row = __ldg(perm + i);
+            const float *p = (const float *)(raw + (int64_t)row * stride);
+            order[pos] = row;
+            qsorted[pos] = make_float4(p[0], p[1], p[2], 0.f);
+        }
+        __syncthreads();
+    }
+}
+__global__ void qgather_kernel(const float4 *__restrict__ qbuf, const uint32_t *__restrict__ order, int64_t nq, float4 *__restrict__ qsorted) {
+    int64_t t = (int64_t)blockIdx.x * blockDim.x + threadIdx.x;
+    if (t < nq) qsorted[t] = qbuf[order[t]];
+}
+__global__ void qkeys_identity_kernel(const float4 *__restrict__ q, int64_t nq, BinParams b, uint32_t bad_key, uint32_t *__restrict__ keys, uint32_t *__restrict__ order) {
+    int64_t i = (int64_t)blockIdx.x * blockDim.x + threadIdx.x;
+    if (i >= nq) return;
+    const float4 p = q[i];
+    keys[i] = query_key(b, bad_key, p.x, p.y, p.z);
+    order[i] = (uint32_t)i;
 }
 
 static inline unsigned blocks_for(int64_t n, int threads) { return (unsigned)std::max<int64_t>(1, (n + threads - 1) / threads); }
@@ -204,9 +266,11 @@
     return cell;
 }
 
-int prepare_queries(pcc_index *idx, const void *q, int64_t nq, int stride_bytes, int mem, cudaStream_t s, Queries *out) {
+constexpr int64_t kSortMinQueries = 2048;
+
+int prepare_queries(pcc_index *idx, const void *q, int64_t nq, int stride_bytes, int mem, cudaStream_t s, Queries *out, bool row_copy) {
     if (!idx->built) return fail(PCC_ERR_STATE, "index not built (call pcc_build first)");
-    if (q == nullptr) { out->self = true; out->nq = idx->n_indexed; out->rows = idx->n_input; out->q = nullptr; out->order = nullptr; return PCC_OK; }
+    if (q == nullptr) { out->self = true; out->nq = idx->n_indexed; out->rows = idx->n_input; out->qsorted = nullptr; out->order = nullptr; return PCC_OK; }
     if (nq < 0 || nq >= (1ll << 31) - 1 || stride_bytes < 12 || (stride_bytes & 3)) return fail(PCC_ERR_INVALID, "bad query batch (nq=%lld stride=%d; nq must be below 2^31 - 1: row counts go to CUB as 32-bit ints)", (long long)nq, stride_bytes);
     out->self = false; out->nq = nq; out->rows = nq;
     if (nq == 0) return PCC_OK;
@@ -216,42 +280,58 @@
         PCC_CUDA(cudaMemcpyAsync(idx->raw.p, q, (size_t)nq * stride_bytes, cudaMemcpyHostToDevice, s));
         raw = idx->raw.as<uint8_t>();
     }
-    PCC_TRY(idx->qbuf.reserve((size_t)nq * sizeof(float4)));
-    if (idx->reuse_order_n == nq && nq > 2048) {
-        BinParams b0{idx->gh.ox, idx->gh.oy, idx->gh.oz, idx->gh.inv_cell, idx->gh.nx, idx->gh.ny, idx->gh.nz};
-        qprep_kernel<<<blocks_for(nq, 256), 256, 0, s>>>(raw, stride_bytes, nq, b0, (uint32_t)idx->gh.n_cells, idx->qbuf.as<float4>(), nullptr, nullptr);
-        PCC_LAUNCHED();
-        PCC_CUDA(cudaGetLastError());
-        out->q = idx->qbuf.as<float4>();
-        out->order = idx->qperm2.as<uint32_t>();
-        return PCC_OK;
-    }
-    const bool sort = nq > 2048;
-    BinParams b{idx->gh.ox, idx->gh.oy, idx->gh.oz, idx->gh.inv_cell, idx->gh.nx, idx->gh.ny, idx->gh.nz};
+    const BinParams b{idx->gh.ox, idx->gh.oy, idx->gh.oz, idx->gh.inv_cell, idx->gh.nx, idx->gh.ny, idx->gh.nz};
+    const bool reuse = idx->reuse_order_n == nq && nq > kSortMinQueries;
+    const bool sort = nq > kSortMinQueries && !reuse;
+    const bool rows = !sort || row_copy;
+    if (rows) PCC_TRY(idx->qbuf.reserve((size_t)nq * sizeof(float4)));
     if (sort) {
         PCC_TRY(idx->qkeys.reserve((size_t)nq * 4)); PCC_TRY(idx->qkeys2.reserve((size_t)nq * 4));
         PCC_TRY(idx->qperm.reserve((size_t)nq * 4)); PCC_TRY(idx->qperm2.reserve((size_t)nq * 4));
     }
-    qprep_kernel<<<blocks_for(nq, 256), 256, 0, s>>>(raw, stride_bytes, nq, b, (uint32_t)idx->gh.n_cells, idx->qbuf.as<float4>(),
+    qprep_kernel<<<blocks_for(nq, 256), 256, 0, s>>>(raw, stride_bytes, nq, b, (uint32_t)idx->gh.n_cells, rows ? idx->qbuf.as<float4>() : nullptr,
                                                      sort ? idx->qkeys.as<uint32_t>() : nullptr, sort ? idx->qperm.as<uint32_t>() : nullptr);
     PCC_LAUNCHED();
     PCC_CUDA(cudaGetLastError());
-    out->q = idx->qbuf.as<float4>();
+    out->qsorted = idx->qbuf.as<float4>();
     out->order = nullptr;
-    if (sort) {
+    if (nq <= kSortMinQueries) return PCC_OK;
+    PCC_TRY(idx->qsorted.reserve((size_t)nq * sizeof(float4)));
+    PCC_TRY(idx->qorder.reserve((size_t)nq * 4));
+    if (reuse) {
+        qgather_kernel<<<blocks_for(nq, 256), 256, 0, s>>>(idx->qbuf.as<float4>(), idx->qorder.as<uint32_t>(), nq, idx->qsorted.as<float4>());
+        PCC_LAUNCHED();
+    } else {
         int bits = 1; while ((1ll << bits) <= idx->gh.n_cells && bits < 32) ++bits;
-        static const int low_env = getenv("PCC_SORT_LOW_BITS") ? atoi(getenv("PCC_SORT_LOW_BITS")) : 0;
-        const int low = std::max(0, std::min(low_env, bits - 8));
-        size_t tmp = idx->sort_tmp_bytes;
-        if (idx->sort_tmp_nq != nq || idx->sort_tmp_bits != bits) {
-            cub::DeviceRadixSort::SortPairs(nullptr, tmp, idx->qkeys.as<uint32_t>(), idx->qkeys2.as<uint32_t>(), idx->qperm.as<uint32_t>(), idx->qperm2.as<uint32_t>(), (int)nq, low, bits, s);
-            idx->sort_tmp_nq = nq; idx->sort_tmp_bits = bits; idx->sort_tmp_bytes = tmp;
-        }
-        PCC_TRY(idx->cub_tmp.reserve(tmp));
-        PCC_CUDA(cub::DeviceRadixSort::SortPairs(idx->cub_tmp.p, tmp, idx->qkeys.as<uint32_t>(), idx->qkeys2.as<uint32_t>(), idx->qperm.as<uint32_t>(), idx->qperm2.as<uint32_t>(), (int)nq, low, bits, s));
-        g_launches += 4;
-        out->order = idx->qperm2.as<uint32_t>();
-    }
+        const int top = std::min(kTopBits, bits), low = bits - top;
+        const uint32_t *keys = idx->qkeys.as<uint32_t>(), *perm = idx->qperm.as<uint32_t>();
+        if (low > 0) {
+            size_t tmp = idx->sort_tmp_bytes;
+            if (idx->sort_tmp_nq != nq || idx->sort_tmp_bits != low) {
+                cub::DeviceRadixSort::SortPairs(nullptr, tmp, idx->qkeys.as<uint32_t>(), idx->qkeys2.as<uint32_t>(), idx->qperm.as<uint32_t>(), idx->qperm2.as<uint32_t>(), (int)nq, 0, low, s);
+                idx->sort_tmp_nq = nq; idx->sort_tmp_bits = low; idx->sort_tmp_bytes = tmp;
+            }
+            PCC_TRY(idx->cub_tmp.reserve(tmp));
+            PCC_CUDA(cub::DeviceRadixSort::SortPairs(idx->cub_tmp.p, tmp, idx->qkeys.as<uint32_t>(), idx->qkeys2.as<uint32_t>(), idx->qperm.as<uint32_t>(), idx->qperm2.as<uint32_t>(), (int)nq, 0, low, s));
+            g_launches += 1 + (low + 7) / 8;
+            keys = idx->qkeys2.as<uint32_t>(); perm = idx->qperm2.as<uint32_t>();
+        }
+        const int64_t ntiles = (nq + kTopTile - 1) / kTopTile, ncounts = ntiles * kTopBins;
+        PCC_TRY(idx->qtop.reserve((size_t)ncounts * 4));
+        uint32_t *counts = idx->qtop.as<uint32_t>();
+        topdigit_count_kernel<<<(unsigned)ntiles, kTopThreads, 0, s>>>(keys, nq, low, counts, ntiles);
+        PCC_LAUNCHED();
+        size_t tmp = 0;
+        cub::DeviceScan::ExclusiveSum(nullptr, tmp, counts, counts, (int)ncounts, s);
+        PCC_TRY(idx->cub_tmp2.reserve(tmp));
+        PCC_CUDA(cub::DeviceScan::ExclusiveSum(idx->cub_tmp2.p, tmp, counts, counts, (int)ncounts, s));
+        g_launches += 2;
+        topdigit_scatter_kernel<<<(unsigned)ntiles, kTopThreads, 0, s>>>(keys, perm, nq, low, counts, ntiles, raw, stride_bytes, idx->qorder.as<uint32_t>(), idx->qsorted.as<float4>());
+        PCC_LAUNCHED();
+    }
+    PCC_CUDA(cudaGetLastError());
+    out->qsorted = idx->qsorted.as<float4>();
+    out->order = idx->qorder.as<uint32_t>();
     return PCC_OK;
 }
 
@@ -296,7 +376,7 @@
     cudaSetDevice(idx->device);
     if (idx->shadow) { pcc_index *sh = idx->shadow; idx->shadow = nullptr; pcc_destroy(sh); }
     for (int i = 0; i < 2; ++i) if (idx->pipe_stream[i]) cudaStreamDestroy(idx->pipe_stream[i]);
-    Buf *bufs[] = {&idx->pts, &idx->cell_start, &idx->occ, &idx->occ2, &idx->cstart, &idx->raw, &idx->stage4, &idx->cellrank, &idx->qbuf, &idx->qkeys, &idx->qkeys2, &idx->qperm, &idx->qperm2,
+    Buf *bufs[] = {&idx->pts, &idx->cell_start, &idx->occ, &idx->occ2, &idx->cstart, &idx->raw, &idx->stage4, &idx->cellrank, &idx->qbuf, &idx->qkeys, &idx->qkeys2, &idx->qperm, &idx->qperm2, &idx->qsorted, &idx->qorder, &idx->qtop, &idx->cub_tmp2,
                    &idx->cub_tmp, &idx->out_i, &idx->out_f, &idx->out_l, &idx->keys64, &idx->keys64b, &idx->misc, &idx->parent, &idx->inv_pos, &idx->sel_params, &idx->icp_prior, &idx->calib,
                    &idx->sift_cloud[0], &idx->sift_cloud[1], &idx->sift_val, &idx->sift_dog, &idx->sift_in, &idx->sift_nbr, &idx->sift_d2, &idx->sift_flag, &idx->sift_pos,
                    &idx->sift_row, &idx->sift_col, &idx->sift_kp};
@@ -462,6 +542,30 @@
     PCC_TRY(rebuild_occupancy(idx, s));
     if (mem == PCC_HOST) PCC_CUDA(cudaStreamSynchronize(s));
     idx->built = true;
+    return PCC_OK;
+}
+
+int pcc_query_order(pcc_index *idx, const void *q, int64_t nq, int stride_bytes, int mem, uint32_t *out_order, uint32_t *out_keys, void *stream) {
+    if (!idx) return fail(PCC_ERR_INVALID, "idx is NULL");
+    if (!q || !out_order || !out_keys) return fail(PCC_ERR_INVALID, "q / out_order / out_keys is NULL (the indexed cloud's own order is its sorted index)");
+    cudaStream_t s = (cudaStream_t)stream;
+    PCC_CUDA(cudaSetDevice(idx->device));
+    Queries qs;
+    PCC_TRY(prepare_queries(idx, q, nq, stride_bytes, mem, s, &qs));
+    if (nq == 0) return PCC_OK;
+    const uint32_t *order = qs.order;
+    if (!order) {
+        PCC_TRY(idx->qkeys.reserve((size_t)nq * 4));
+        PCC_TRY(idx->qperm2.reserve((size_t)nq * 4));
+        const BinParams b{idx->gh.ox, idx->gh.oy, idx->gh.oz, idx->gh.inv_cell, idx->gh.nx, idx->gh.ny, idx->gh.nz};
+        qkeys_identity_kernel<<<blocks_for(nq, 256), 256, 0, s>>>(qs.qsorted, nq, b, (uint32_t)idx->gh.n_cells, idx->qkeys.as<uint32_t>(), idx->qperm2.as<uint32_t>());
+        PCC_LAUNCHED();
+        PCC_CUDA(cudaGetLastError());
+        order = idx->qperm2.as<uint32_t>();
+    }
+    PCC_TRY(copy_out(out_order, order, (size_t)nq * 4, mem, s));
+    PCC_TRY(copy_out(out_keys, idx->qkeys.p, (size_t)nq * 4, mem, s));
+    PCC_CUDA(cudaStreamSynchronize(s));
     return PCC_OK;
 }
 
diff --git a/pointcloudcomparator_b200/csrc/pcc_device.cuh b/pointcloudcomparator_b200/csrc/pcc_device.cuh
--- a/pointcloudcomparator_b200/csrc/pcc_device.cuh
+++ b/pointcloudcomparator_b200/csrc/pcc_device.cuh
@@ -37,6 +37,14 @@
 __device__ __forceinline__ float grid_u(float x, float o, float inv) { return __fmul_rn(__fsub_rn(x, o), inv); }
 __device__ __forceinline__ int grid_c(float u, int n) { return (int)fminf(fmaxf(floorf(u), 0.f), (float)(n - 1)); }
 __device__ __forceinline__ bool finite3(float x, float y, float z) { return isfinite(x) && isfinite(y) && isfinite(z); }
+
+struct QueryView { const float4 *qsorted; const uint32_t *order; int64_t nq; bool self; };
+__device__ __forceinline__ int64_t query_at(const Grid &g, const QueryView &v, int64_t t, float &x, float &y, float &z) {
+    const float4 p = __ldg((v.self ? g.pts : v.qsorted) + t);
+    x = p.x; y = p.y; z = p.z;
+    if (v.self) return __float_as_int(p.w);
+    return v.order ? (int64_t)__ldg(v.order + t) : t;
+}
 
 struct QueryCell {
     float ux, uy, uz;
diff --git a/pointcloudcomparator_b200/csrc/pcc_internal.h b/pointcloudcomparator_b200/csrc/pcc_internal.h
--- a/pointcloudcomparator_b200/csrc/pcc_internal.h
+++ b/pointcloudcomparator_b200/csrc/pcc_internal.h
@@ -67,6 +67,7 @@
     bool occ_valid = false;
     pcc::Buf raw, stage4, cellrank, qbuf, qkeys, qkeys2, qperm, qperm2, cub_tmp, out_i, out_f, out_l, keys64, keys64b, misc, parent, inv_pos, sel_params, icp_prior, calib;
     pcc::Buf sift_cloud[2], sift_val, sift_dog, sift_in, sift_nbr, sift_d2, sift_flag, sift_pos, sift_row, sift_col, sift_kp;
+    pcc::Buf qsorted, qorder, qtop, cub_tmp2;
     uint64_t grid_gen = 0;
     void *comm = nullptr;
     int comm_rank = 0, comm_world = 1;
@@ -101,13 +102,13 @@
 
 namespace pcc {
 struct Queries {
-    const float4 *q = nullptr;
+    const float4 *qsorted = nullptr;
     const uint32_t *order = nullptr;
     int64_t nq = 0;
     bool self = false;
     int64_t rows = 0;
 };
-int prepare_queries(pcc_index *idx, const void *q, int64_t nq, int stride_bytes, int mem, cudaStream_t s, Queries *out);
+int prepare_queries(pcc_index *idx, const void *q, int64_t nq, int stride_bytes, int mem, cudaStream_t s, Queries *out, bool row_copy = false);
 int copy_out(void *dst, const void *src_dev, size_t bytes, int mem, cudaStream_t s);
 int rebuild_inverse(pcc_index *idx, cudaStream_t s);
 int rebuild_occupancy(pcc_index *idx, cudaStream_t s);
diff --git a/pointcloudcomparator_b200/csrc/pcc_knn.cu b/pointcloudcomparator_b200/csrc/pcc_knn.cu
--- a/pointcloudcomparator_b200/csrc/pcc_knn.cu
+++ b/pointcloudcomparator_b200/csrc/pcc_knn.cu
@@ -10,20 +10,13 @@
 
 namespace pcc {
 
-struct QueryView {
-    const float4 *q; const uint32_t *order; int64_t nq; bool self;
-};
 __device__ __forceinline__ bool load_query(const Grid &g, const QueryView &v, int64_t t, float &x, float &y, float &z, int64_t &row, bool &write_empty) {
     write_empty = false;
     if (t >= v.nq) return false;
-    if (v.self) { float4 p = __ldg(g.pts + t); x = p.x; y = p.y; z = p.z; row = __float_as_int(p.w); return true; }
-    uint32_t qi = v.order ? __ldg(v.order + t) : (uint32_t)t;
-    float4 p = __ldg(v.q + qi); x = p.x; y = p.y; z = p.z; row = qi;
+    row = query_at(g, v, t, x, y, z);
+    if (v.self) return true;
 #ifdef PCC_EXP_SEQROWS
     row = t;
-#endif
-#ifdef PCC_EXP_SEQQ
-    p = __ldg(v.q + t); x = p.x; y = p.y; z = p.z;
 #endif
     if (!finite3(x, y, z) || g.n == 0) { write_empty = true; return false; }
     return true;
@@ -740,7 +733,7 @@
 
 __global__ void fill_f32_kernel(float *p, int64_t n, float v) { int64_t i = (int64_t)blockIdx.x * blockDim.x + threadIdx.x; if (i < n) p[i] = v; }
 static inline unsigned nblocks(int64_t n, int threads) { return (unsigned)std::max<int64_t>(1, (n + threads - 1) / threads); }
-static inline QueryView view_of(const Queries &q) { return QueryView{q.q, q.order, q.nq, q.self}; }
+static inline QueryView view_of(const Queries &q) { return QueryView{q.qsorted, q.order, q.nq, q.self}; }
 static int heap_threads(int k) {
     int t = (int)((96 * 1024) / ((size_t)k * sizeof(nkey_t)));
     t = std::min(128, (t / 32) * 32);
@@ -1071,7 +1064,7 @@
     *count = 0;
     if (ns == 0) return PCC_OK;
     Queries qs;
-    PCC_TRY(prepare_queries(idx, src_inout, ns, stride_bytes, mem, s, &qs));
+    PCC_TRY(prepare_queries(idx, src_inout, ns, stride_bytes, mem, s, &qs, true));
     float4 *work = idx->qbuf.as<float4>();
     Mat34 T; int apply = 0;
     if (T_apply) { memcpy(T.m, T_apply, sizeof(T.m)); apply = 1; } else memset(&T, 0, sizeof(T));
diff --git a/pointcloudcomparator_b200/csrc/pcc_knn_thr.cuh b/pointcloudcomparator_b200/csrc/pcc_knn_thr.cuh
--- a/pointcloudcomparator_b200/csrc/pcc_knn_thr.cuh
+++ b/pointcloudcomparator_b200/csrc/pcc_knn_thr.cuh
@@ -5,9 +5,6 @@
 
 namespace pcc {
 
-#ifndef PCC_THR_QAHEAD
-#define PCC_THR_QAHEAD 0
-#endif
 #ifndef PCC_THR_EARLY
 #define PCC_THR_EARLY 16
 #endif
@@ -241,14 +238,6 @@
     constexpr uint32_t SMASK = (1u << ThrCfg<K>::slot_bits) - 1u;
     const int k = FULLK ? K : k_rt;
     float x = 0.f, y = 0.f, z = 0.f; int64_t row = 0; bool empty = false;
-#if PCC_THR_QAHEAD
-    uint32_t qi_ahead = 0xFFFFFFFFu;
-    if (!RETRY && !STAGED && v.order) {
-        constexpr int64_t AHEAD = (int64_t)PCC_THR_QAHEAD * ThrCfg<K>::threads;
-        if ((threadIdx.x & 31) == 0 && t + 2 * AHEAD < v.nq) prefetch_l2(v.order + t + 2 * AHEAD);
-        if (t + AHEAD < v.nq) qi_ahead = __ldg(v.order + t + AHEAD);
-    }
-#endif
     const bool live = load_query(g, v, t, x, y, z, row, empty);
     auto leave_dead = [&]() {
         if (t < v.nq) fix.ring_flag[t] = 0;
@@ -277,9 +266,6 @@
         for (int r = 0; r < 9; ++r) { M += re[r] - rs[r]; rowmask |= (re[r] > rs[r] ? 1u : 0u) << r; if (!STAGED && (PCC_THR_PREFETCH & 1)) prefetch_run<3, false>(g.pts, rs[r], re[r]); }
         s0 = rs[0]; e0 = re[0];
     }
-#if PCC_THR_QAHEAD
-    if (!RETRY && !STAGED && qi_ahead != 0xFFFFFFFFu) prefetch_l2(v.q + qi_ahead);
-#endif
     auto leave_wide = [&]() {
         fix.ring_flag[t] = 0;
         if (fix.stats) { atomicAdd(fix.stats + 0, 1ull); atomicAdd(fix.stats + 4, 1ull); }
diff --git a/pointcloudcomparator_b200/csrc/pcc_radius.cu b/pointcloudcomparator_b200/csrc/pcc_radius.cu
--- a/pointcloudcomparator_b200/csrc/pcc_radius.cu
+++ b/pointcloudcomparator_b200/csrc/pcc_radius.cu
@@ -7,16 +7,13 @@
 
 namespace pcc {
 
-struct QueryView { const float4 *q; const uint32_t *order; int64_t nq; bool self; };
-static inline QueryView view_of(const Queries &q) { return QueryView{q.q, q.order, q.nq, q.self}; }
+static inline QueryView view_of(const Queries &q) { return QueryView{q.qsorted, q.order, q.nq, q.self}; }
 static inline unsigned nblocks(int64_t n, int threads) { return (unsigned)std::max<int64_t>(1, (n + threads - 1) / threads); }
 
 __device__ __forceinline__ bool load_query(const Grid &g, const QueryView &v, int64_t t, float &x, float &y, float &z, int64_t &row) {
     if (t >= v.nq) return false;
-    if (v.self) { float4 p = __ldg(g.pts + t); x = p.x; y = p.y; z = p.z; row = __float_as_int(p.w); return true; }
-    uint32_t qi = v.order ? __ldg(v.order + t) : (uint32_t)t;
-    float4 p = __ldg(v.q + qi); x = p.x; y = p.y; z = p.z; row = qi;
-    return finite3(x, y, z) && g.n > 0;
+    row = query_at(g, v, t, x, y, z);
+    return v.self || (finite3(x, y, z) && g.n > 0);
 }
 
 template <class F>
@@ -284,27 +281,21 @@
                                                            const uint32_t *__restrict__ inv_pos, float vx, float vy, float vz, float4 *__restrict__ out) {
     const int64_t t = (int64_t)blockIdx.x * blockDim.x + threadIdx.x;
     if (t >= v.nq) return;
-    float x, y, z; int64_t row;
-    if (v.self) { float4 p = __ldg(g.pts + t); x = p.x; y = p.y; z = p.z; row = __float_as_int(p.w); }
-    else { uint32_t qi = v.order ? __ldg(v.order + t) : (uint32_t)t; float4 p = __ldg(v.q + qi); x = p.x; y = p.y; z = p.z; row = qi; }
+    float x, y, z;
+    const int64_t row = query_at(g, v, t, x, y, z);
     const int64_t b = offsets[row], e = offsets[row + 1];
     float a[9] = {0, 0, 0, 0, 0, 0, 0, 0, 0};
     for (int64_t j = b; j < e; ++j) { float4 p = __ldg(g.pts + __ldg(inv_pos + (uint32_t)keys[j])); accu_add(a, p.x, p.y, p.z); }
     out[row] = normal_from_accu(a, (int)min((int64_t)INT_MAX, e - b), x, y, z, vx, vy, vz);
 }
 
-__device__ __forceinline__ int64_t rows_query(const Grid &g, const QueryView &v, int64_t t, float &x, float &y, float &z) {
-    if (v.self) { float4 p = __ldg(g.pts + t); x = p.x; y = p.y; z = p.z; return __float_as_int(p.w); }
-    uint32_t qi = v.order ? __ldg(v.order + t) : (uint32_t)t; float4 p = __ldg(v.q + qi); x = p.x; y = p.y; z = p.z; return qi;
-}
-
 __global__ void __launch_bounds__(128) gradient_rows_kernel(Grid g, QueryView v, const int64_t *__restrict__ offsets, const nkey_t *__restrict__ keys,
                                                             const uint32_t *__restrict__ inv_pos, const float *__restrict__ intensity,
                                                             const float4 *__restrict__ normals, float4 *__restrict__ out) {
     const int64_t t = (int64_t)blockIdx.x * blockDim.x + threadIdx.x;
     if (t >= v.nq) return;
     float qx, qy, qz;
-    const int64_t row = rows_query(g, v, t, qx, qy, qz);
+    const int64_t row = query_at(g, v, t, qx, qy, qz);
     const int64_t b = offsets[row], e = offsets[row + 1];
     const float qnan = CUDART_NAN_F;
     if (e - b < 3) { out[row] = make_float4(qnan, qnan, qnan, 0.f); return; }
@@ -391,7 +382,7 @@
     const int64_t t = (int64_t)blockIdx.x * blockDim.x + threadIdx.x;
     if (t >= v.nq) return;
     float qx, qy, qz;
-    const int64_t row = rows_query(g, v, t, qx, qy, qz);
+    const int64_t row = query_at(g, v, t, qx, qy, qz);
     const int nb = nd * ng;
     float *o = out + row * nb;
     const int64_t b = offsets[row], e = offsets[row + 1];
@@ -445,7 +436,7 @@
     const int64_t t = (int64_t)blockIdx.x * blockDim.x + threadIdx.x;
     if (t >= v.nq) return;
     float qx, qy, qz;
-    const int64_t row = rows_query(g, v, t, qx, qy, qz);
+    const int64_t row = query_at(g, v, t, qx, qy, qz);
     const int64_t b = offsets[row], e = offsets[row + 1];
     float num[16], den[16];
 #pragma unroll
@@ -478,8 +469,8 @@
 __global__ void __launch_bounds__(128) first_within_kernel(Grid g, QueryView v, double thr, float r2_cover, int R0, int32_t *__restrict__ out) {
     const int64_t t = (int64_t)blockIdx.x * blockDim.x + threadIdx.x;
     if (t >= v.nq) return;
-    const uint32_t qi = v.order ? __ldg(v.order + t) : (uint32_t)t;
-    const float4 q = __ldg(v.q + qi);
+    float4 q;
+    const int64_t qi = query_at(g, v, t, q.x, q.y, q.z);
     int32_t best = INT_MAX;
     if (finite3(q.x, q.y, q.z) && g.n > 0) {
         const QueryCell c = locate(g, q.x, q.y, q.z);
```

Result: no change. 2.637 billion (median of 6 runs) (-0.5%).
